# tud-amr/semantic_dsp_map

Hardware: AMD Instinct MI355X
Metric: Mvoxels updated/sec (256^3 grid, 2M particles, VKITTI2 camera; whole hot-path frame) (higher is better)
Workload: dtype f32

## Files before the change

include/sdm.h:

```cpp
#ifndef SDM_H_
#define SDM_H_

#include <stddef.h>
#include <stdint.h>

#ifdef __cplusplus
extern "C" {
#endif

typedef struct sdm_map sdm_map;

typedef enum {
  SDM_OK = 0,
  SDM_ERR_INVALID_ARGUMENT = 1,
  SDM_ERR_NO_DEVICE = 2,
  SDM_ERR_HIP = 3,
  SDM_ERR_CAPACITY = 4,
  SDM_ERR_NOT_CONVERGED = 5,
  SDM_ERR_COMM = 6
} sdm_status;

typedef struct {
  int32_t x_n, y_n, z_n;
  int32_t p_n;
// ... 282 lines not shown
  uint16_t cell_max[3];
  float    wsum_max;
  uint64_t cell_sum[3];
  uint64_t cell_sq[6];
  float    box_min[3];
  float    box_max[3];
  float    centroid[3];
  uint32_t pad;
} sdm_instance;
sdm_status sdm_instances_update(sdm_map *m, uint32_t flags);
sdm_status sdm_get_instances(sdm_map *m, sdm_instance *out, int32_t cap, int32_t *n_out, float origin[3]);
sdm_status sdm_get_label_cells(sdm_map *m, uint32_t out[256]);

#define SDM_FRONTIERS_FACE_CONNECTED 0x1u
#define SDM_FRONTIERS_BYTES_PER_CELL 169
typedef struct {
  uint32_t first_cell;
  uint32_t n_cells;
  uint32_t n_unknown_faces;
  uint32_t first_index;
  uint16_t cell_min[3];
  uint16_t cell_max[3];
  uint32_t pad0;
  uint64_t cell_sum[3];
  float    box_min[3];
  float    box_max[3];
  float    centroid[3];
  uint32_t pad1;
} sdm_frontier_cluster;
sdm_status sdm_frontiers_update(sdm_map *m, uint32_t flags, int32_t min_cells, int64_t max_cells);
sdm_status sdm_get_frontier_clusters(sdm_map *m, sdm_frontier_cluster *out, int32_t cap, int32_t *n_out, float origin[3]);
sdm_status sdm_get_frontier_cells(sdm_map *m, uint32_t *cell, uint32_t *cluster, uint8_t *unknown_faces,
                                  int64_t cap, int64_t *n_out);

#define SDM_VIEW_MAX_RAYS 65536
typedef struct {
  float pos[3];
  float q[4];
  float range;
} sdm_view;
typedef struct {
  uint32_t n_unknown;
  uint32_t n_free;
  uint32_t n_occupied;
  uint32_t rays_hit;
  uint32_t rays_in_map;
  uint32_t pad;
  uint64_t ray_cells;
  uint64_t ray_unknown;
} sdm_view_gain;
sdm_status sdm_query_views(sdm_map *m, const sdm_view *views, int64_t n_views, const float *dirs, int32_t n_rays,
                           sdm_view_gain *out, sdm_segment_hit *rays_out, int32_t *ray_unknown_out, uint32_t flags);

#define SDM_REACH_FACE_CONNECTED  0x1u
#define SDM_REACH_THROUGH_UNKNOWN 0x2u
#define SDM_REACH_COST_PER_CELL   10
typedef struct {
  uint32_t n_starts_used;
  uint32_t n_traversable, n_reached, max_cost_reached;
  uint32_t rounds;
  uint32_t flags, min_d2, max_cost;
} sdm_reach_info;
typedef struct {
  uint32_t cost;
  float    metres;
  uint32_t cell;
  uint8_t  next;
  uint8_t  status;
  uint16_t pad;
} sdm_reach_result;
sdm_status sdm_reach_update(sdm_map *m, const float *start_xyz, const uint32_t *start_cells, int64_t n_starts,
                            uint32_t min_d2, uint32_t max_cost, uint32_t flags);
sdm_status sdm_get_reach(sdm_map *m, uint32_t *cost, sdm_reach_info *info, float origin[3]);
sdm_status sdm_query_reach(sdm_map *m, const float *xyz, const uint32_t *cells, int64_t n, sdm_reach_result *out, uint32_t flags);
sdm_status sdm_reach_paths(sdm_map *m, const float *xyz, const uint32_t *cells, int64_t n, int32_t max_len,
                           uint32_t *cells_out, int32_t *len_out, uint32_t flags);

sdm_status sdm_object_particle_count(sdm_map *m, int32_t track_id, int64_t *count);
sdm_status sdm_tracks_with_particles(sdm_map *m, int32_t *out, int32_t cap, int32_t *n_out);

sdm_status sdm_get_stats(sdm_map *m, sdm_stats *out, int32_t count_live);
sdm_status sdm_set_profiling(sdm_map *m, int32_t on);
sdm_status sdm_debug_force_generic_flood(sdm_map *m, int32_t on);
sdm_status sdm_get_ring_state(sdm_map *m, sdm_ring_state *out);
sdm_status sdm_set_ring_state(sdm_map *m, const sdm_ring_state *in);
sdm_status sdm_get_stamps(sdm_map *m, uint32_t *sx, uint32_t *sy, uint32_t *sz);
sdm_status sdm_set_stamps(sdm_map *m, const uint32_t *sx, const uint32_t *sy, const uint32_t *sz);
sdm_status sdm_dump_state(sdm_map *m, float *px, float *py, float *pz, float *w, uint16_t *ts,
                          uint16_t *track, uint8_t *label, uint8_t *status, uint8_t *forget,
                          uint16_t *owner);
sdm_status sdm_load_state(sdm_map *m, const float *px, const float *py, const float *pz,
                          const float *w, const uint16_t *ts, const uint16_t *track,
                          const uint8_t *label, const uint8_t *status, const uint8_t *forget,
                          const uint16_t *owner);
sdm_status sdm_get_ck_kappa(sdm_map *m, float *out);
sdm_status sdm_get_bin_counts(sdm_map *m, uint32_t *out);
sdm_status sdm_get_bins(sdm_map *m, uint32_t *out, int64_t cap, int64_t *n_out);
sdm_status sdm_get_extrinsic(sdm_map *m, float *out16);

sdm_status sdm_time_occupancy_sweep(sdm_map *m, int32_t iters, float *avg_ms);
sdm_status sdm_debug_fill_dense(sdm_map *m);
sdm_status sdm_debug_fill_dense_ex(sdm_map *m, int32_t mode);
sdm_status sdm_debug_hinted_groups(sdm_map *m, int64_t *n_out);
sdm_status sdm_debug_sweep_lists(sdm_map *m, int32_t mode);
sdm_status sdm_debug_sweep_mode(sdm_map *m, int32_t *mode_out);
sdm_status sdm_debug_alias_cap(sdm_map *m, int32_t cap);
sdm_status sdm_debug_reach_tiles(sdm_map *m, int64_t *tiles_out);
sdm_status sdm_debug_view_batch(sdm_map *m, int32_t max_views_in_flight);

sdm_status sdm_test_scan(const uint32_t *in, uint32_t *out, int64_t n);
sdm_status sdm_test_sort_pairs(const uint32_t *keys_in, const uint32_t *vals_in, uint32_t *keys_out,
                               uint32_t *vals_out, int64_t n, int32_t nbits);
#define SDM_TEST_IN_PLACE 1u
#define SDM_TEST_COUNT_ON_DEVICE 2u
#define SDM_TEST_GUARD_WORDS 64
sdm_status sdm_test_scratch_elems(int32_t sort, int64_t n, int64_t *elems);
sdm_status sdm_test_scan_seq(int32_t n_calls, const int64_t *capacity, const int64_t *count, uint32_t flags,
                             const uint32_t *in, uint32_t *out, int32_t *guard_ok, uint32_t *scratch_out);
sdm_status sdm_test_sort_pairs_seq(int32_t n_calls, const int64_t *capacity, const int64_t *count, const int32_t *nbits,
                                   uint32_t flags, const uint32_t *keys_in, const uint32_t *vals_in, uint32_t *keys_out,
                                   uint32_t *vals_out, int32_t *which, int32_t *guard_ok, uint32_t *scratch_out);

const char *sdm_last_error(void);
const char *sdm_version(void);

#ifdef __cplusplus
}
#endif
#endif
```

semantic_dsp_map_amd/binding.py:

```python
import ctypes as C
import os

import numpy as np

_HERE = os.path.dirname(os.path.abspath(__file__))
LIB_PATH = os.environ.get("SDM_LIB_PATH") or os.path.join(_HERE, "csrc", "libsdm_hip.so")

LABELED_POINT = np.dtype([("x", "<f4"), ("y", "<f4"), ("z", "<f4"), ("sigma", "<f4"),
                          ("track_id", "<u2"), ("label_id", "u1"), ("is_valid", "u1")])
OBJECT_MOVE = np.dtype([("track_id", "<i4"), ("T", "<f4", (16,))])
VOXEL_RESULT = np.dtype([("wsum", "<f4"), ("track", "<u2"), ("label", "u1"), ("occ", "i1")])
POINT = np.dtype([("x", "<f4"), ("y", "<f4"), ("z", "<f4"), ("track", "<u2"), ("label", "u1"), ("occ", "i1")])
POINT_XYZRGB = np.dtype([("x", "<f4"), ("y", "<f4"), ("z", "<f4"), ("one", "<f4"), ("b", "u1"), ("g", "u1"), ("r", "u1"), ("a", "u1"),
                         ("pad", "<u4", (3,))])
assert LABELED_POINT.itemsize == 20 and OBJECT_MOVE.itemsize == 68 and VOXEL_RESULT.itemsize == 8 and POINT.itemsize == 16
SEGMENT_HIT = np.dtype([("t", "<f4"), ("voxel", "<u4"), ("cells", "<i4"), ("track", "<u2"), ("label", "u1"), ("occ", "i1")])
BOX_RESULT = np.dtype([("n_occupied", "<i4"), ("n_free", "<i4"), ("n_unknown", "<i4"), ("first_occupied", "<u4"), ("clipped", "<i4")])
assert SEGMENT_HIT.itemsize == 16 and BOX_RESULT.itemsize == 20
QUERY_ON_DEVICE = 0x1
QUERY_UNKNOWN_BLOCKS = 0x2
DISTANCE_RESULT = np.dtype([("distance", "<f4"), ("gradient", "<f4", (3,)), ("nearest", "<f4", (3,)), ("d2", "<u4"), ("track", "<u2"),
                            ("label", "u1"), ("occ", "i1")])
assert DISTANCE_RESULT.itemsize == 36
ESDF_UNKNOWN_IS_OBSTACLE = 0x1
# ... 103 lines not shown

def load_library():
    global _lib
    if _lib is not None:
        return _lib
    if not os.path.exists(LIB_PATH):
        raise SdmError("libsdm_hip.so is not built: run `python -c 'import __graft_entry__ as g; g.build()'` "
                       "or `make -C semantic_dsp_map_amd/csrc`.  There is no CPU path.")
    L = C.CDLL(LIB_PATH)
    vp = C.c_void_p
    i32, u32, i64 = C.c_int32, C.c_uint32, C.c_int64
    sig = {
        "sdm_create": [C.POINTER(Config), C.POINTER(vp)],
        "sdm_destroy": [vp],
        "sdm_clear": [vp],
        "sdm_set_params": [vp, C.POINTER(Params)],
        "sdm_generate_noise_table": [vp, C.c_uint64, i32, C.c_float],
        "sdm_upload_noise_table": [vp, vp, i32],
        "sdm_download_noise_table": [vp, vp, i32],
        "sdm_download_pdf_table": [vp, vp, i32],
        "sdm_update": [vp, vp, vp, vp, vp, vp, i32, vp, i32, u32, i32],
        "sdm_update_raw": [vp, vp, vp, vp, vp, i32, vp, vp, vp, i32, vp, i32, u32, i32],
        "sdm_update_raw_ex": [vp, vp, vp, vp, vp, i32, vp, vp, vp, i32, vp, i32, u32, i32, vp],
        "sdm_get_labeled_cloud": [vp, vp],
        "sdm_host_alloc": [C.c_size_t, C.POINTER(vp)],
        "sdm_host_free": [vp],
        "sdm_update_begin": [vp, vp, vp, vp, vp, vp, i32, vp, i32, u32, i32, C.POINTER(vp)],
        "sdm_update_finish": [vp, vp, i32, u32, i32],
        "sdm_frame_start": [vp, vp, vp, vp, vp, vp, i32, vp, i32, u32, i32],
        "sdm_frame_moves": [vp],
        "sdm_frame_moves_pending": [vp, C.POINTER(C.c_int32)],
        "sdm_frame_predict": [vp, C.POINTER(vp)],
        "sdm_set_halo_buffers": [vp, vp, vp, vp, vp, i32],
        "sdm_comm_unique_id": [vp],
        "sdm_comm_init": [vp, vp, i32],
        "sdm_ipc_create": [vp, i32, vp],
        "sdm_ipc_connect": [vp, vp],
        "sdm_update_sharded": [vp, vp, vp, vp, vp, vp, i32, vp, i32, u32],
        "sdm_ck_chunk_elems": [vp, C.POINTER(i64)],
        "sdm_ck_reduce": [vp, vp, vp],
        "sdm_comm_timing": [vp, i32],
        "sdm_get_comm_times": [vp, vp],
        "sdm_device_alloc": [vp, C.c_size_t, C.POINTER(vp)],
        "sdm_device_free": [vp, vp],
        "sdm_device_upload": [vp, vp, vp, C.c_size_t],
        "sdm_device_download": [vp, vp, vp, C.c_size_t],
        "sdm_device_synchronize": [vp],
        "sdm_stream": [vp, C.POINTER(vp)],
        "sdm_set_stream": [vp, vp],
        "sdm_set_ck_buffer": [vp, vp],
        "sdm_synchronize": [vp],
        "sdm_get_voxels": [vp, vp],
        "sdm_get_occupied": [vp, vp, C.c_size_t, C.POINTER(C.c_size_t), i32],
        "sdm_get_occupied_rgb": [vp, vp, C.c_size_t, C.POINTER(C.c_size_t), i32],
        "sdm_get_freespace_rgb": [vp, vp, C.c_size_t, C.POINTER(C.c_size_t), i32],
        "sdm_set_colours": [vp, vp],
        "sdm_get_freespace": [vp, vp, C.c_size_t, C.POINTER(C.c_size_t), i32],
        "sdm_voxels_device_ptr": [vp, C.POINTER(vp)],
        "sdm_query_points": [vp, vp, i64, vp, vp, u32],
        "sdm_query_segments": [vp, vp, i64, vp, u32],
        "sdm_query_boxes": [vp, vp, i64, vp, u32],
        "sdm_esdf_update": [vp, u32],
        "sdm_get_esdf": [vp, vp, vp, vp],
        "sdm_query_distance": [vp, vp, i64, vp, u32],
        "sdm_instances_update": [vp, u32],
        "sdm_get_instances": [vp, vp, i32, C.POINTER(i32), vp],
        "sdm_get_label_cells": [vp, vp],
        "sdm_frontiers_update": [vp, u32, i32, i64],
        "sdm_get_frontier_clusters": [vp, vp, i32, C.POINTER(i32), vp],
        "sdm_get_frontier_cells": [vp, vp, vp, vp, i64, C.POINTER(i64)],
        "sdm_query_views": [vp, vp, i64, vp, i32, vp, vp, vp, u32],
        "sdm_debug_view_batch": [vp, i32],
        "sdm_reach_update": [vp, vp, vp, i64, u32, u32, u32],
        "sdm_get_reach": [vp, vp, vp, vp],
        "sdm_query_reach": [vp, vp, vp, i64, vp, u32],
        "sdm_reach_paths": [vp, vp, vp, i64, i32, vp, vp, u32],
        "sdm_debug_reach_tiles": [vp, C.POINTER(i64)],
        "sdm_object_particle_count": [vp, i32, C.POINTER(i64)],
        "sdm_tracks_with_particles": [vp, vp, i32, C.POINTER(i32)],
        "sdm_comm_set_options": [vp, i32, i32],
        "sdm_get_stats": [vp, C.POINTER(Stats), i32],
        "sdm_set_profiling": [vp, i32],
        "sdm_debug_force_generic_flood": [vp, i32],
        "sdm_get_ring_state": [vp, C.POINTER(RingState)],
        "sdm_set_ring_state": [vp, C.POINTER(RingState)],
        "sdm_get_stamps": [vp, vp, vp, vp],
        "sdm_set_stamps": [vp, vp, vp, vp],
        "sdm_dump_state": [vp] + [vp] * 10,
        "sdm_load_state": [vp] + [vp] * 10,
        "sdm_get_ck_kappa": [vp, vp],
        "sdm_get_bin_counts": [vp, vp],
        "sdm_get_bins": [vp, vp, i64, C.POINTER(i64)],
        "sdm_get_extrinsic": [vp, vp],
        "sdm_time_occupancy_sweep": [vp, i32, C.POINTER(C.c_float)],
        "sdm_set_issue_mode": [vp, i32],
        "sdm_bind_host_thread": [i32],
        "sdm_host_numa_node_early": [i32],
        "sdm_debug_fill_dense": [vp],
        "sdm_debug_fill_dense_ex": [vp, i32],
        "sdm_debug_hinted_groups": [vp, C.POINTER(C.c_int64)],
        "sdm_debug_sweep_lists": [vp, i32],
        "sdm_debug_sweep_mode": [vp, C.POINTER(i32)],
        "sdm_debug_alias_cap": [vp, i32],
        "sdm_test_scan": [vp, vp, i64],
        "sdm_test_sort_pairs": [vp, vp, vp, vp, i64, i32],
        "sdm_test_scratch_elems": [i32, i64, C.POINTER(i64)],
        "sdm_test_scan_seq": [i32, vp, vp, u32, vp, vp, C.POINTER(i32), vp],
        "sdm_test_sort_pairs_seq": [i32, vp, vp, vp, u32, vp, vp, vp, vp, vp, C.POINTER(i32), vp],
    }
    for name, argtypes in sig.items():
        fn = getattr(L, name)
        fn.argtypes = argtypes
        fn.restype = C.c_int
    L.sdm_last_error.restype = C.c_char_p
    L.sdm_version.restype = C.c_char_p
    global HOST_NUMA_NODE
    HOST_NUMA_NODE = L.sdm_bind_host_thread(int(os.environ.get("LOCAL_RANK", "0")))
    _lib = L
    return L


def _ptr(a):
    if a is None:
        return None
    if isinstance(a, int):
        return C.c_void_p(a)
    return a.ctypes.data_as(C.c_void_p)


def _check(L, rc, what):
    if rc != 0:
        raise SdmError("%s failed: %s (%s)" % (what, STATUS_NAMES.get(rc, rc), L.sdm_last_error().decode()))


class SdmMap:

    def __init__(self, cfg, params=None, noise_table=None, device=0, shard_rank=0, shard_count=1, max_visible=0):
        self.L = load_library()
        c = Config()
        for k, _ in Config._fields_:
            if k in cfg:
                setattr(c, k, cfg[k])
        c.device, c.shard_rank, c.shard_count, c.max_visible = device, shard_rank, shard_count, max_visible
        self.cfg = c
        h = C.c_void_p()
        _check(self.L, self.L.sdm_create(C.byref(c), C.byref(h)), "sdm_create")
        self.h = h
        self.V = 1 << (c.x_n + c.y_n + c.z_n)
        self.S = 1 << c.p_n
        self.v_count = self.V // shard_count
        self.W, self.H = c.width, c.height
        if params is not None:
            self.set_params(params)
        if noise_table is not None:
            self.upload_noise_table(noise_table)

    def close(self):
        if getattr(self, "h", None):
            self.L.sdm_destroy(self.h)
            self.h = None

    def __del__(self):
        try:
            self.close()
        except Exception:
            pass
# ... 336 lines not shown
            return None
        p = None if xyz is None else np.ascontiguousarray(xyz, dtype=np.float32).reshape(-1, 3)
        w = None if cells is None else np.ascontiguousarray(cells, dtype=np.uint32).reshape(-1)
        n = len(p) if p is not None else len(w) if w is not None else 0
        res = np.empty(n, REACH_RESULT)
        _check(self.L, self.L.sdm_query_reach(self.h, _ptr(p), _ptr(w), n, _ptr(res), 0), "sdm_query_reach")
        return res

    def reach_paths(self, xyz=None, cells=None, max_len=0, on_device=False, n=None, cells_out=None, len_out=None, fill=REACH_NO_COST):
        if on_device:
            _check(self.L, self.L.sdm_reach_paths(self.h, _ptr(int(xyz)) if xyz else None, _ptr(int(cells)) if cells else None, int(n),
                                                  int(max_len), _ptr(int(cells_out)) if cells_out else None, _ptr(int(len_out)),
                                                  QUERY_ON_DEVICE), "sdm_reach_paths")
            return None
        p = None if xyz is None else np.ascontiguousarray(xyz, dtype=np.float32).reshape(-1, 3)
        w = None if cells is None else np.ascontiguousarray(cells, dtype=np.uint32).reshape(-1)
        n = len(p) if p is not None else len(w) if w is not None else 0
        rows, lens = np.full((n, int(max_len)), fill, np.uint32), np.zeros(n, np.int32)
        _check(self.L, self.L.sdm_reach_paths(self.h, _ptr(p), _ptr(w), n, int(max_len), _ptr(rows), _ptr(lens), 0), "sdm_reach_paths")
        return rows, lens

    def reach_tiles(self):
        n = C.c_int64(0)
        _check(self.L, self.L.sdm_debug_reach_tiles(self.h, C.byref(n)), "sdm_debug_reach_tiles")
        return n.value

    def occupied(self, cap=None, zero_center=False, free=False, mark_fov=False):
        cap = cap or self.v_count
        out = np.empty(cap, POINT)
        n = C.c_size_t()
        fn = self.L.sdm_get_freespace if free else self.L.sdm_get_occupied
        _check(self.L, fn(self.h, _ptr(out), cap, C.byref(n), (1 if zero_center else 0) | (2 if mark_fov else 0)),
               "sdm_get_occupied")
        return out[:min(n.value, cap)], n.value

    def set_colours(self, label_bgr, perm, background_label=0, colour_by_label=False, jet_axis=0, evaluation_format=False):
        c = ColourConfig()
        lb = np.ascontiguousarray(label_bgr, np.uint8).reshape(256, 3)
        pm = np.ascontiguousarray(perm, np.uint8).reshape(256)
        C.memmove(c.label_bgr, lb.ctypes.data, 768)
        C.memmove(c.perm, pm.ctypes.data, 256)
        c.background_label, c.colour_by_label = int(background_label), 1 if colour_by_label else 0
        c.jet_axis, c.evaluation_format = int(jet_axis), 1 if evaluation_format else 0
        _check(self.L, self.L.sdm_set_colours(self.h, C.byref(c)), "sdm_set_colours")

    def occupied_rgb(self, cap=None, zero_center=False, free=False):
        cap = cap or self.v_count
        out = np.empty(cap, POINT_XYZRGB)
        n = C.c_size_t()
        fn = self.L.sdm_get_freespace_rgb if free else self.L.sdm_get_occupied_rgb
        _check(self.L, fn(self.h, _ptr(out), cap, C.byref(n), 1 if zero_center else 0), "sdm_get_occupied_rgb")
        return out[:min(n.value, cap)], n.value

    def object_particle_count(self, track):
        n = C.c_int64()
        _check(self.L, self.L.sdm_object_particle_count(self.h, track, C.byref(n)), "sdm_object_particle_count")
        return n.value

    def tracks_with_particles(self):
        out = np.zeros(65536, np.int32)
        n = C.c_int32(0)
        _check(self.L, self.L.sdm_tracks_with_particles(self.h, _ptr(out), out.size, C.byref(n)), "sdm_tracks_with_particles")
        return out[:n.value].copy()

    def stats_unchecked(self):
        return self.stats(check=False)

    def stats(self, count_live=False, check=True):
        s = Stats()
        rc = self.L.sdm_get_stats(self.h, C.byref(s), 1 if count_live else 0)
        if check:
            _check(self.L, rc, "sdm_get_stats")
        d = {k: getattr(s, k) for k, _ in Stats._fields_ if k not in ("stage_ms", "restamped_slabs")}
        d["stage_ms"] = list(s.stage_ms)
        d["restamped_slabs"] = list(s.restamped_slabs)
        return d

    def set_profiling(self, on=True):
        _check(self.L, self.L.sdm_set_profiling(self.h, 1 if on else 0), "sdm_set_profiling")

    def force_generic_flood(self, on=True):
        _check(self.L, self.L.sdm_debug_force_generic_flood(self.h, 1 if on else 0), "sdm_debug_force_generic_flood")

    def ring_state(self):
        r = RingState()
        _check(self.L, self.L.sdm_get_ring_state(self.h, C.byref(r)), "sdm_get_ring_state")
        return {"global_time_stamp": r.global_time_stamp, "moved_steps": list(r.moved_steps),
                "eq_steps": list(r.eq_steps), "map_center": list(r.map_center), "last_pos": list(r.last_pos),
                "birth_cursor": r.birth_cursor, "move_cursor": r.move_cursor}

    def set_ring_state(self, d):
        r = RingState()
        r.global_time_stamp = d["global_time_stamp"]
        for i in range(3):
            r.moved_steps[i] = d["moved_steps"][i]
            r.eq_steps[i] = d["eq_steps"][i]
            r.map_center[i] = d["map_center"][i]
            r.last_pos[i] = d["last_pos"][i]
        r.birth_cursor = d["birth_cursor"]
        r.move_cursor = d["move_cursor"]
        _check(self.L, self.L.sdm_set_ring_state(self.h, C.byref(r)), "sdm_set_ring_state")

    def stamps(self):
        c = self.cfg
        sx = np.empty(1 << c.x_n, np.uint32)
        sy = np.empty(1 << c.y_n, np.uint32)
        sz = np.empty(1 << c.z_n, np.uint32)
        _check(self.L, self.L.sdm_get_stamps(self.h, _ptr(sx), _ptr(sy), _ptr(sz)), "sdm_get_stamps")
        return sx, sy, sz

    def set_stamps(self, sx, sy, sz):
        sx, sy, sz = (np.ascontiguousarray(a, dtype=np.uint32) for a in (sx, sy, sz))
        _check(self.L, self.L.sdm_set_stamps(self.h, _ptr(sx), _ptr(sy), _ptr(sz)), "sdm_set_stamps")

    def dump_state(self):
        n = self.v_count * self.S
        st = {k: np.empty(n, dt) for k, dt in STATE_FIELDS}
        _check(self.L, self.L.sdm_dump_state(self.h, *[_ptr(st[k]) for k, _ in STATE_FIELDS]), "sdm_dump_state")
        return st

    def load_state(self, st):
        arrs = [np.ascontiguousarray(st[k], dtype=dt) for k, dt in STATE_FIELDS]
        _check(self.L, self.L.sdm_load_state(self.h, *[_ptr(a) for a in arrs]), "sdm_load_state")

    def ck_kappa(self):
        out = np.empty(self.W * self.H, np.float32)
        _check(self.L, self.L.sdm_get_ck_kappa(self.h, _ptr(out)), "sdm_get_ck_kappa")
        return out.reshape(self.H, self.W)

    def bin_counts(self):
        out = np.empty(self.W * self.H, np.uint32)
        _check(self.L, self.L.sdm_get_bin_counts(self.h, _ptr(out)), "sdm_get_bin_counts")
        return out.reshape(self.H, self.W)

    def bins(self):
        n = C.c_int64()
        _check(self.L, self.L.sdm_get_bins(self.h, None, 0, C.byref(n)), "sdm_get_bins")
        out = np.empty(max(n.value, 1), np.uint32)
        _check(self.L, self.L.sdm_get_bins(self.h, _ptr(out), n.value, C.byref(n)), "sdm_get_bins")
        return out[:n.value]

    def extrinsic(self):
        out = np.empty(16, np.float32)
        _check(self.L, self.L.sdm_get_extrinsic(self.h, _ptr(out)), "sdm_get_extrinsic")
        return out.reshape(4, 4)

    def fill_dense_ex(self, mode):
        _check(self.L, self.L.sdm_debug_fill_dense_ex(self.h, mode), "sdm_debug_fill_dense_ex")

    def hinted_groups(self):
        n = C.c_int64()
        _check(self.L, self.L.sdm_debug_hinted_groups(self.h, C.byref(n)), "sdm_debug_hinted_groups")
        return n.value

    def force_sweep_lists(self, mode):
        _check(self.L, self.L.sdm_debug_sweep_lists(self.h, int(mode)), "sdm_debug_sweep_lists")

    def sweep_mode(self):
        v = C.c_int32(0)
        _check(self.L, self.L.sdm_debug_sweep_mode(self.h, C.byref(v)), "sdm_debug_sweep_mode")
        return v.value

    def set_alias_cap(self, cap):
        _check(self.L, self.L.sdm_debug_alias_cap(self.h, int(cap)), "sdm_debug_alias_cap")

    def fill_dense(self):
# ... 89 lines not shown
```

semantic_dsp_map_amd/csrc/debug.hip:

```cpp
#include "sdm_map.h"

namespace {

__global__ void k_spin(unsigned long long ticks, unsigned long long *out) {
  const unsigned long long t0 = wall_clock64();
  out[0] = t0;
  while (wall_clock64() - t0 < ticks) __builtin_amdgcn_s_sleep(8);
  out[1] = wall_clock64();
}
__global__ void k_stamp(unsigned long long *out) { *out = wall_clock64(); }

}

extern "C" {

sdm_status sdm_debug_overlap(sdm_map *m, int32_t which, double out_us[2]) {
  if (!m || which < 0 || which > 2 || !out_us) return SDM_ERR_INVALID_ARGUMENT;
  HIP_TRY(hipSetDevice(m->device));
  unsigned long long *d = nullptr, h[3] = {0, 0, 0};
  DevTemps tmp;
  HIP_TRY(tmp.alloc(&d, 3));
  if (which == 2) HIP_TRY(lazy_stream(m->device, &m->s_moves));
  hipStream_t side = which == 0 ? m->s_frustum : (which == 1 ? m->s_birth : m->s_moves);
  HIP_TRY(hipStreamSynchronize(m->stream));
  HIP_TRY(hipStreamSynchronize(side));
  hipLaunchKernelGGL(k_spin, dim3(1), dim3(1), 0, m->stream, 6000ull, d);
  hipLaunchKernelGGL(k_stamp, dim3(1), dim3(1), 0, side, d + 2);
  HIP_TRY(hipStreamSynchronize(m->stream));
  HIP_TRY(hipStreamSynchronize(side));
  HIP_TRY(hipMemcpy(h, d, sizeof(h), hipMemcpyDeviceToHost));
  out_us[0] = ((double)h[2] - (double)h[0]) / 100.0;
  out_us[1] = ((double)h[1] - (double)h[0]) / 100.0;
  return SDM_OK;
}

sdm_status sdm_debug_force_generic_flood(sdm_map *m, int32_t on) {
  if (!m) return SDM_ERR_INVALID_ARGUMENT;
  m->force_generic_flood = on ? 1 : 0;
  return SDM_OK;
}

sdm_status sdm_time_occupancy_sweep(sdm_map *m, int32_t iters, float *avg_ms) {
  if (!m || !avg_ms || iters <= 0) return SDM_ERR_INVALID_ARGUMENT;
  HIP_TRY(hipSetDevice(m->device));
  hipEvent_t a, b;
  HIP_TRY(hipEventCreate(&a));
  HIP_TRY(hipEventCreate(&b));
  launch_occupancy(m->d, m->flt, m->st, m->sc.cnt, 1, m->sc.fa, m->sweep_epoch, m->stream, sweep_mode(m));
  m->sweep_rec_pending = true;
  HIP_TRY(hipStreamSynchronize(m->stream));
  SDM_TRY(sweep_mode_latch(m));
  const int mode = sweep_mode(m);
  HIP_TRY(hipEventRecord(a, m->stream));
  for (int i = 0; i < iters; ++i) launch_occupancy(m->d, m->flt, m->st, m->sc.cnt, 1, m->sc.fa, m->sweep_epoch, m->stream, mode);
  HIP_TRY(hipEventRecord(b, m->stream));
  HIP_TRY(hipEventSynchronize(b));
  m->sweep_rec_pending = true;
  float ms = 0.f;
  HIP_TRY(hipEventElapsedTime(&ms, a, b));
  *avg_ms = ms / iters;
  (void)hipEventDestroy(a);
  (void)hipEventDestroy(b);
  return SDM_OK;
}

sdm_status sdm_debug_fill_dense_ex(sdm_map *m, int32_t mode) {
  if (!m || mode < 0 || mode > 1) return SDM_ERR_INVALID_ARGUMENT;
  HIP_TRY(hipSetDevice(m->device));
  launch_fill_dense(m->d, m->st, m->global_time_stamp ? m->global_time_stamp : 1u, mode, m->stream);
  HIP_TRY(hipStreamSynchronize(m->stream));
  return SDM_OK;
}
sdm_status sdm_debug_fill_dense(sdm_map *m) { return sdm_debug_fill_dense_ex(m, 0); }
sdm_status sdm_debug_sweep_lists(sdm_map *m, int32_t mode) {
  if (!m || mode < -1 || mode > 1) return SDM_ERR_INVALID_ARGUMENT;
  m->sweep_lists_forced = mode;
  if (mode >= 0) m->sweep_lists = mode != 0;
  return SDM_OK;
}
sdm_status sdm_debug_sweep_mode(sdm_map *m, int32_t *mode_out) {
  if (!m || !mode_out) return SDM_ERR_INVALID_ARGUMENT;
  HIP_TRY(hipSetDevice(m->device));
  HIP_TRY(hipStreamSynchronize(m->stream));
  SDM_TRY(sweep_mode_latch(m));
  *mode_out = sweep_mode(m);
  return SDM_OK;
}
sdm_status sdm_debug_alias_cap(sdm_map *m, int32_t cap) {
  if (!m || cap < 1 || (uint32_t)cap > ALIAS_CAP) return SDM_ERR_INVALID_ARGUMENT;
  if (m->n_graph_frames || m->n_direct_frames) return SDM_ERR_INVALID_ARGUMENT;
  m->st.alias_cap = (uint32_t)cap;
  return SDM_OK;
}
sdm_status sdm_debug_hinted_groups(sdm_map *m, int64_t *n_out) {
  if (!m || !n_out) return SDM_ERR_INVALID_ARGUMENT;
  HIP_TRY(hipSetDevice(m->device));
  std::vector<uint8_t> h(grp_hint_bytes(m->d.v_count));
  HIP_TRY(hipMemcpyAsync(h.data(), m->st.grp_hint, h.size(), hipMemcpyDeviceToHost, m->stream));
  HIP_TRY(hipStreamSynchronize(m->stream));
  int64_t n = 0;
  for (uint8_t b : h) n += b != 0;
  *n_out = n;
  return SDM_OK;
}

#ifdef SDM_AB_TIMERS
extern "C++" {
namespace sdm {
void debug_timers(unsigned long long *out32, int reset);
void debug_timers_moves(unsigned long long *out, int reset);
}
}
sdm_status sdm_debug_timers(sdm_map *m, unsigned long long *out32, int reset) {
  HIP_TRY(hipSetDevice(m->device));
  HIP_TRY(hipDeviceSynchronize());
  sdm::debug_timers(out32, reset);
  sdm::debug_timers_moves(out32 + 6 * 8192 * 4, reset);
  return SDM_OK;
}
#endif

// ... 164 lines not shown
```

semantic_dsp_map_amd/csrc/frame.hip:

```cpp
#include <chrono>

#include "sdm_map.h"

#pragma clang fp contract(off)

void sdm::drop_graphs(sdm_map *m) {
  if (m->graph_exec) (void)hipGraphExecDestroy(m->graph_exec);
  if (m->graph) (void)hipGraphDestroy(m->graph);
  m->graph_exec = nullptr;
  m->graph = nullptr;
  m->graph_set_node = nullptr;
  for (hipGraphExec_t &g : m->piece) {
    if (g) (void)hipGraphExecDestroy(g);
    g = nullptr;
  }
}

namespace {

inline void stage_mark(sdm_map *m, int stage) {
  if (m->profiling && !m->capturing) {
    (void)hipEventRecord(m->ev[stage], m->stream);
    m->stage_ran[stage] = true;
  }
}

sdm_status frame_host_prepare(sdm_map *m, const float cam_pos[3], const float cam_q[4], const sdm_object_move *moves, int32_t n_moves,
                              const int32_t *remove_tracks, int32_t n_remove, uint32_t flags, int32_t stop_after) {
  if ((n_moves > MAX_MOVE_OBJECTS || n_remove > MAX_REMOVE_TRACKS) && m->capturing) {
    set_error("sdm_update", __FILE__, __LINE__, "object lists beyond one frame block inside a graph capture");
    return SDM_ERR_INVALID_ARGUMENT;
  }
  m->moves_all.clear();
  m->removes_all.clear();
  m->mv_batch_next = n_moves > MAX_MOVE_OBJECTS ? (size_t)MAX_MOVE_OBJECTS : 0;
  m->mv_batch_ready = false;
  if (n_moves > MAX_MOVE_OBJECTS) m->moves_all.assign(moves, moves + n_moves);
  if (n_remove > MAX_REMOVE_TRACKS) m->removes_all.assign(remove_tracks, remove_tracks + n_remove);
  m->stop_after = stop_after;
  m->frame_flags = flags;
  for (int i = 0; i < 9; ++i) m->stage_ran[i] = false;
  m->global_time_stamp += 1;
  FrameArgs &fa = m->fa;
  fa.su.n = 0;
  fa.su.value = m->global_time_stamp;
  m->restamped[0] = m->restamped[1] = m->restamped[2] = 0;
  update_ego_center(m, cam_pos);
  sync_frame_scalars(m);
  if (m->stamps_dirty) {
    m->sweep_all = true;
    fa.su.n = 0;
  }
  refresh_filter(m);
  m->forgetting_initialized = true;
  compute_extrinsic(m, cam_pos, cam_q);
  compute_frustum_box(m);
  fa.f = m->f;
  memset(&fa.ms, 0, sizeof(fa.ms));
  const int n_first = n_moves < MAX_MOVE_OBJECTS ? n_moves : MAX_MOVE_OBJECTS;
  fa.ms.n = n_first;
  for (int k = 0; k < n_first; ++k) {
    fa.ms.track[k] = (uint16_t)moves[k].track_id;
    memcpy(fa.ms.T[k], moves[k].T, 12 * sizeof(float));
  }
  fa.n_obj = n_first;
  fa.mv_batch = 0;
  if (n_moves > 0 && !stage_done(stop_after, 1)) m->mv_seq++;
  fa.mv_seq = m->mv_seq;
  fa.n_remove = n_remove < MAX_REMOVE_TRACKS ? n_remove : MAX_REMOVE_TRACKS;
  for (int k = 0; k < fa.n_remove; ++k) fa.remove[k] = (uint16_t)remove_tracks[k];
  fa.force_generic = m->force_generic_flood;
  m->n_moves = n_moves;
  m->n_remove = n_remove;
  return SDM_OK;
}

sdm_status frame_enqueue_start(sdm_map *m) {
  hipStream_t s = m->stream;
  const Dims &d = m->d;
  const int32_t stop_after = m->stop_after;
  const bool whole = d.v_count == d.V;
  stage_mark(m, 0);
  if (m->stamps_dirty) SDM_TRY(upload_stamps(m));
  m->cur_depth = m->fa.depth;
  m->cur_cloud = m->fa.cloud;
  if (m->capturing) {
    m->fb.set(d, m->st, m->sc, m->fa, true, whole);
    launch_frame_begin(m->fb, s);
    HIP_TRY(hipEventRecord(m->cap_begin, s));
    HIP_TRY(hipStreamWaitEvent(m->s_frustum, m->cap_begin, 0));
    HIP_TRY(hipStreamWaitEvent(m->s_birth, m->cap_begin, 0));
  } else {
    const bool side_chain_now = m->n_moves > 0 && (!whole || ((m->comm || m->ipc) && m->sharded_frame));
    if (!m->state_event_valid && (!m->vis_event_valid || side_chain_now)) {
      HIP_TRY(hipEventRecord(m->ev_state, s));
      m->state_event_valid = true;
    }
    HIP_TRY(hipStreamWaitEvent(m->s_frustum, m->vis_event_valid ? m->ev_vis : m->ev_state, 0));
    launch_set_frame(m->d_fa[1], m->fa, m->s_frustum);
    HIP_TRY(hipEventRecord(m->ev_fa, m->s_frustum));
    if (whole && m->mv_pending) HIP_TRY(hipMemsetAsync(m->sc.mv_tot, 0, move_total_elems() * sizeof(uint32_t), s));
    m->fb.set(d, m->st, m->sc, m->fa, false, whole);
    launch_frame_begin(m->fb, s, !stage_done(stop_after, 5) ? m->ev_begin : nullptr);
    if (whole && m->n_moves > 0) m->mv_pending = true;
  }
  stage_mark(m, 1);
  if (stage_done(stop_after, 1)) return SDM_OK;

  const bool side_chain = !m->capturing && m->n_moves > 0 && (!whole || ((m->comm || m->ipc) && m->sharded_frame));
  if (m->capturing) {
    if (!whole) launch_moves_count(d, m->st, m->sc, m->d_counts_local, s);
  } else if (side_chain) {
    HIP_TRY(lazy_stream(m->device, &m->s_moves));
    HIP_TRY(hipStreamWaitEvent(m->s_moves, m->ev_state, 0));
    if (!whole) {
      if (m->mv_pending) HIP_TRY(hipMemsetAsync(m->sc.mv_tot, 0, move_total_elems() * sizeof(uint32_t), m->s_moves));
      launch_moves_count(d, m->st, m->sc, m->counts_local_user ? m->counts_local_user : m->d_counts_local, m->s_moves, &m->fa);
      m->mv_pending = true;
    }
    if ((m->comm || m->ipc) && m->sharded_frame) {
      if (m->comm_timing) HIP_TRY(hipEventRecord(m->ev_comm[0], m->s_moves));
      SDM_TRY(exchange_counts(m, m->s_moves));
      if (m->comm_timing) {
        HIP_TRY(hipEventRecord(m->ev_comm[1], m->s_moves));
        m->comm_timed[0] = true;
      }
    }
    HIP_TRY(hipEventRecord(m->ev_counts, m->s_moves));
  }
  if (!stage_done(stop_after, 3)) {
    launch_frustum(d, m->sc, m->s_frustum);
    HIP_TRY(hipGetLastError());
    HIP_TRY(hipEventRecord(m->capturing ? m->cap_frustum : m->ev_frustum, m->s_frustum));
  } else if (!m->capturing) {
    HIP_TRY(hipStreamWaitEvent(s, m->ev_fa, 0));
  }
  if (!stage_done(stop_after, 5)) {
    if (!m->capturing) HIP_TRY(hipStreamWaitEvent(m->s_birth, m->ev_begin, 0));
    m->birth_which = launch_birth_prepare(d, m->flt, m->bo, m->st, m->sc, m->s_birth);
    HIP_TRY(hipEventRecord(m->capturing ? m->cap_birth : m->ev_birth, m->s_birth));
  }
  if (side_chain) HIP_TRY(hipStreamWaitEvent(s, m->ev_counts, 0));
  m->state_event_valid = false;
  m->vis_event_valid = false;
  return SDM_OK;
}

sdm_status check_frame_args(sdm_map *m, const float *depth, const sdm_labeled_point *cloud, const float cam_pos[3], const float cam_q[4],
                            const sdm_object_move *moves, int32_t n_moves, const int32_t *remove_tracks, int32_t n_remove) {
  if (!m || !depth || !cloud || !cam_pos || !cam_q || n_moves < 0 || n_remove < 0 || (n_moves && !moves) || (n_remove && !remove_tracks)) {
    set_error("sdm_update", __FILE__, __LINE__, "null pointer or negative count");
    return SDM_ERR_INVALID_ARGUMENT;
  }
  return SDM_OK;
}

sdm_status stage_inputs(sdm_map *m, const float *depth, const sdm_labeled_point *cloud, uint32_t flags) {
  const size_t hw = (size_t)m->d.W * m->d.H;
  if (flags & SDM_INPUT_ON_DEVICE) {
    m->fa.depth = depth;
    m->fa.cloud = cloud;
  } else {
    HIP_TRY(hipMemcpyAsync(m->d_depth, depth, hw * sizeof(float), hipMemcpyHostToDevice, m->stream));
    HIP_TRY(hipMemcpyAsync(m->d_cloud, cloud, hw * sizeof(sdm_labeled_point), hipMemcpyHostToDevice, m->stream));
    m->fa.depth = m->d_depth;
    m->fa.cloud = m->d_cloud;
  }
  return SDM_OK;
}

}

extern "C" {

sdm_status sdm_frame_start(sdm_map *m, const float *depth, const sdm_labeled_point *cloud, const float cam_pos[3],
                           const float cam_q[4], const sdm_object_move *moves, int32_t n_moves,
                           const int32_t *remove_tracks, int32_t n_remove, uint32_t flags, int32_t stop_after) {
  sdm_status rc = check_frame_args(m, depth, cloud, cam_pos, cam_q, moves, n_moves, remove_tracks, n_remove);
  if (rc != SDM_OK) return rc;
  HIP_TRY(hipSetDevice(m->device));
  if ((rc = frame_host_prepare(m, cam_pos, cam_q, moves, n_moves, remove_tracks, n_remove, flags, stop_after)) != SDM_OK) return rc;
  if ((rc = stage_inputs(m, depth, cloud, flags)) != SDM_OK) return rc;
  m->n_direct_frames++;
  return frame_enqueue_start(m);
}

sdm_status sdm_frame_moves(sdm_map *m) {
  if (!m) return SDM_ERR_INVALID_ARGUMENT;
  if (stage_done(m->stop_after, SDM_STAGE_EGO)) return SDM_OK;
  if (!m->capturing) HIP_TRY(hipSetDevice(m->device));
  const int world = m->cfg.shard_count, rank = m->cfg.shard_rank;
  const int32_t *counts_all = m->counts_all_user;
  int w = world, r = rank;
  if (!counts_all) {
    counts_all = m->counts_local_user ? m->counts_local_user : m->d_counts_local;
    w = 1;
    r = 0;
  }
  if (m->capturing || m->n_moves > 0) {
    launch_moves_transform(m->d, m->flt, m->st, m->sc, counts_all, w, r, m->stream);
    m->mv_pending = false;
    m->mv_batch_ready = false;
    const bool shard = m->d.v_count != m->d.V;
    while (m->mv_batch_next && m->mv_batch_next < m->moves_all.size()) {
      const size_t k0 = m->mv_batch_next;
      const int nb = (int)std::min<size_t>(MAX_MOVE_OBJECTS, m->moves_all.size() - k0);
      FrameArgs &fa = m->fa;
      memset(&fa.ms, 0, sizeof(fa.ms));
      fa.ms.n = nb;
      for (int k = 0; k < nb; ++k) {
        fa.ms.track[k] = (uint16_t)m->moves_all[k0 + k].track_id;
        memcpy(fa.ms.T[k], m->moves_all[k0 + k].T, 12 * sizeof(float));
      }
      fa.n_obj = nb;
      fa.mv_seq = ++m->mv_seq;
      fa.mv_batch += 1;
      m->mv_batch_next = k0 + MAX_MOVE_OBJECTS;
      launch_moves_batch(m->d, m->st, m->sc, fa, m->counts_local_user ? m->counts_local_user : m->d_counts_local, m->stream);
      if (shard) {
        m->mv_batch_ready = true;
        return SDM_OK;
      }
      launch_moves_transform(m->d, m->flt, m->st, m->sc, counts_all, w, r, m->stream);
    }
    m->mv_batch_next = 0;
  }
  return SDM_OK;
}

sdm_status sdm_frame_moves_pending(sdm_map *m, int32_t *pending) {
  if (!m || !pending) return SDM_ERR_INVALID_ARGUMENT;
  *pending = m->mv_batch_ready ? 1 : 0;
  return SDM_OK;
}

sdm_status sdm_frame_predict(sdm_map *m, const float **ck_part_dev) {
  if (!m) return SDM_ERR_INVALID_ARGUMENT;
  if (m->mv_batch_ready) {
    set_error("sdm_frame_predict", __FILE__, __LINE__, "a batch of the frame's object list is still waiting for its counts: sdm_frame_moves_pending");
    return SDM_ERR_INVALID_ARGUMENT;
  }
  const int stop_after = m->stop_after;
  if (stage_done(stop_after, SDM_STAGE_EGO)) return SDM_OK;
  if (!m->capturing) HIP_TRY(hipSetDevice(m->device));
  hipStream_t s = m->stream;
  const Dims &d = m->d;
  if (m->capturing || m->n_moves > 0)
    launch_moves_finish(d, m->flt, m->st, m->sc, m->counts_all_user ? m->cfg.shard_count : 1, m->cfg.shard_rank, s);
  stage_mark(m, 2);
  if (stage_done(stop_after, 2)) return SDM_OK;

  if (m->capturing || m->n_remove > 0) launch_remove(d, m->st, m->sc, s);
  for (size_t k0 = MAX_REMOVE_TRACKS; k0 < m->removes_all.size(); k0 += MAX_REMOVE_TRACKS) {
    FrameArgs &fa = m->fa;
    fa.n_remove = (int)std::min<size_t>(MAX_REMOVE_TRACKS, m->removes_all.size() - k0);
    for (int k = 0; k < fa.n_remove; ++k) fa.remove[k] = (uint16_t)m->removes_all[k0 + k];
    launch_set_frame(m->d_fa[0], fa, s);
    launch_remove(d, m->st, m->sc, s);
  }
  stage_mark(m, 3);
  if (stage_done(stop_after, 3)) return SDM_OK;

  HIP_TRY(hipStreamWaitEvent(s, m->capturing ? m->cap_frustum : m->ev_frustum, 0));
  float *ck_dst = m->ck_user ? m->ck_user : m->d_ck_part;
  launch_visibility(d, m->flt, m->st, m->sc, ck_dst, m->fused_ck ? 1 : 0, s, m->capturing ? nullptr : m->ev_vis);
  if (!m->capturing) m->vis_event_valid = true;
  stage_mark(m, 4);
  if (stage_done(stop_after, 4)) return SDM_OK;

  launch_ck(d, m->flt, m->st, m->sc, ck_dst, m->fused_ck ? 1 : 0, s);
  if (ck_part_dev) *ck_part_dev = ck_dst;
  return SDM_OK;
}

sdm_status sdm_update_begin(sdm_map *m, const float *depth, const sdm_labeled_point *cloud, const float cam_pos[3],
                            const float cam_q[4], const sdm_object_move *moves, int32_t n_moves,
                            const int32_t *remove_tracks, int32_t n_remove, uint32_t flags, int32_t stop_after,
                            const float **ck_part_dev) {
  sdm_status rc = sdm_frame_start(m, depth, cloud, cam_pos, cam_q, moves, n_moves, remove_tracks, n_remove, flags, stop_after);
  if (rc != SDM_OK) return rc;
  const int32_t *keep_all = m->counts_all_user;
  m->counts_all_user = nullptr;
  rc = sdm_frame_moves(m);
  while (rc == SDM_OK && m->mv_batch_ready) rc = sdm_frame_moves(m);
  if (rc == SDM_OK) rc = sdm_frame_predict(m, ck_part_dev);
  m->counts_all_user = keep_all;
  return rc;
}

sdm_status sdm_set_halo_buffers(sdm_map *m, int32_t *counts_local, const int32_t *counts_all, void *send, const void *recv_all,
                                int32_t cap_records) {
  if (!m || cap_records < 0) return SDM_ERR_INVALID_ARGUMENT;
  m->counts_local_user = counts_local;
  m->counts_all_user = counts_all;
  m->sc.halo_send = (unsigned char *)send;
  m->sc.halo_recv = (const unsigned char *)recv_all;
  m->sc.halo_cap = (uint32_t)cap_records;
  m->sc.halo_world = (uint32_t)m->cfg.shard_count;
  return SDM_OK;
}

sdm_status sdm_update_finish(sdm_map *m, const float *ck_parts_dev, int32_t n_parts, uint32_t flags, int32_t stop_after) {
  if (!m || n_parts < 1) return SDM_ERR_INVALID_ARGUMENT;
  if (stage_done(stop_after, SDM_STAGE_VISIBILITY)) return SDM_OK;
  if (!m->capturing) HIP_TRY(hipSetDevice(m->device));
  hipStream_t s = m->stream;
  const Dims &d = m->d;
  const float *own = m->ck_user ? m->ck_user : m->d_ck_part;
  const float *ck_raw = nullptr;
  if (!m->fused_ck) {
    if (!ck_parts_dev || n_parts == 1) ck_raw = ck_parts_dev ? ck_parts_dev : own;
    else launch_ck_finish(d, m->flt, m->sc, ck_parts_dev, n_parts, m->ck_part_stride, s);
  }
  m->ck_raw_last = ck_raw;
  m->ck_part_stride = 0;
  launch_weight(d, m->flt, m->st, m->sc, s, ck_raw);
  stage_mark(m, 5);
  if (stage_done(stop_after, 5)) return SDM_OK;
  HIP_TRY(hipStreamWaitEvent(s, m->capturing ? m->cap_birth : m->ev_birth, 0));
  launch_birth_replay(d, m->flt, m->st, m->sc, m->birth_which, m->global_time_stamp > 65535u, s);
  if (!m->capturing) {
    if (d.v_count != d.V || m->comm || m->ipc) {
      HIP_TRY(hipEventRecord(m->ev_state, s));
      m->state_event_valid = true;
    } else {
      m->state_event_valid = false;
    }
  }
  stage_mark(m, 6);
  if (stage_done(stop_after, 6)) return SDM_OK;
  if (!(flags & SDM_SKIP_OCCUPANCY)) {
    launch_occupancy(d, m->flt, m->st, m->sc.cnt, m->sweep_all ? 1 : 0, m->sc.fa, next_epoch(m->f.epoch), s, sweep_mode(m));
    if (m->sweep_all) m->sweep_rec_pending = true;
    m->sweep_all = false;
    if (!m->capturing) m->sweep_epoch = next_epoch(m->f.epoch);
  }
  stage_mark(m, 7);
  return SDM_OK;
}

namespace {

sdm_status issue_frame(sdm_map *m, uint32_t flags, int32_t stop_after) {
  sdm_status rc = frame_enqueue_start(m);
  if (rc == SDM_OK) rc = sdm_frame_moves(m);
  if (rc == SDM_OK) rc = sdm_frame_predict(m, nullptr);
  if (rc == SDM_OK) rc = sdm_update_finish(m, nullptr, 1, flags, stop_after);
  return rc;
}

sdm_status capture_prepare(sdm_map *m) {
  drop_graphs(m);
  HIP_TRY(hipStreamSynchronize(m->s_frustum));
  if (m->s_moves) HIP_TRY(hipStreamSynchronize(m->s_moves));
  HIP_TRY(hipStreamSynchronize(m->s_birth));
  m->sc.fa = m->d_fa[0];
  m->sc.fa_side = m->d_fa[1];
  return SDM_OK;
}

sdm_status graph_capture(sdm_map *m) {
  SDM_TRY(capture_prepare(m));
  m->capturing = true;
  hipStream_t side[3] = {m->s_frustum, m->s_birth, m->s_moves};
  if (m->graph_shape == GRAPH_CHAIN) m->s_frustum = m->s_birth = m->stream;
  hipError_t e = hipStreamBeginCapture(m->stream, hipStreamCaptureModeThreadLocal);
  sdm_status rc = SDM_OK;
  if (e == hipSuccess) {
    rc = issue_frame(m, m->frame_flags, 0);
    hipGraph_t g = nullptr;
    e = hipStreamEndCapture(m->stream, &g);
    m->graph = g;
  }
  m->s_frustum = side[0];
  m->s_birth = side[1];
  m->s_moves = side[2];
  m->capturing = false;
  if (e != hipSuccess || rc != SDM_OK || !m->graph) {
    set_error("hipStreamCapture", __FILE__, __LINE__, e != hipSuccess ? hipGetErrorString(e) : "frame enqueue failed under capture");
    (void)hipGetLastError();
    return rc != SDM_OK ? rc : SDM_ERR_HIP;
  }
  size_t n_nodes = 0;
  HIP_TRY(hipGraphGetNodes(m->graph, nullptr, &n_nodes));
  std::vector<hipGraphNode_t> nodes(n_nodes);
  HIP_TRY(hipGraphGetNodes(m->graph, nodes.data(), &n_nodes));
  for (hipGraphNode_t nd : nodes) {
    hipGraphNodeType t;
    if (hipGraphNodeGetType(nd, &t) != hipSuccess || t != hipGraphNodeTypeKernel) continue;
    hipKernelNodeParams kp;
    if (hipGraphKernelNodeGetParams(nd, &kp) == hipSuccess && kp.func == FrameBeginLaunch::kernel()) m->graph_set_node = nd;
  }
  if (!m->graph_set_node) {
    set_error("graph_capture", __FILE__, __LINE__, "frame-block node not found in the captured graph");
    return SDM_ERR_HIP;
  }
  HIP_TRY(hipGraphInstantiate(&m->graph_exec, m->graph, nullptr, nullptr, 0));
  m->graph_flt = m->flt;
  return SDM_OK;
}

sdm_status graph_launch(sdm_map *m) {
  m->fb.set(m->d, m->st, m->sc, m->fa, true, m->d.v_count == m->d.V);
  hipKernelNodeParams kp;
  memset(&kp, 0, sizeof(kp));
  kp.func = const_cast<void *>(FrameBeginLaunch::kernel());
  kp.gridDim = dim3(FrameBeginLaunch::GRID);
  kp.blockDim = dim3(FrameBeginLaunch::BLOCK);
  kp.sharedMemBytes = 0;
  kp.kernelParams = m->fb.argv;
  kp.extra = nullptr;
  const auto t0 = std::chrono::steady_clock::now();
  HIP_TRY(hipGraphExecKernelNodeSetParams(m->graph_exec, m->graph_set_node, &kp));
  const auto t1 = std::chrono::steady_clock::now();
  HIP_TRY(hipGraphLaunch(m->graph_exec, m->stream));
  if (m->host_timing) {
    m->t_setparams_us += std::chrono::duration<double, std::micro>(t1 - t0).count();
    m->t_launch_us += std::chrono::duration<double, std::micro>(std::chrono::steady_clock::now() - t1).count();
  }
  return SDM_OK;
}

sdm_status pieces_capture(sdm_map *m) {
  SDM_TRY(capture_prepare(m));
  const Dims &d = m->d;
  auto capture = [&](hipStream_t st, int which, auto &&body) -> sdm_status {
    HIP_TRY(hipStreamBeginCapture(st, hipStreamCaptureModeThreadLocal));
    body(st);
    hipGraph_t g = nullptr;
    hipError_t e = hipStreamEndCapture(st, &g);
    if (e != hipSuccess || !g) {
      set_error("hipStreamEndCapture", __FILE__, __LINE__, e != hipSuccess ? hipGetErrorString(e) : "no graph");
      (void)hipGetLastError();
      return SDM_ERR_HIP;
    }
    e = hipGraphInstantiate(&m->piece[which], g, nullptr, nullptr, 0);
    (void)hipGraphDestroy(g);
    if (e != hipSuccess) {
      set_error("hipGraphInstantiate", __FILE__, __LINE__, hipGetErrorString(e));
      return SDM_ERR_HIP;
    }
    return SDM_OK;
  };
  sdm_status rc = capture(m->s_frustum, 0, [&](hipStream_t st) { launch_frustum(d, m->sc, st); });
  if (rc == SDM_OK)
    rc = capture(m->s_birth, 1, [&](hipStream_t st) { m->birth_which = launch_birth_prepare(d, m->flt, m->bo, m->st, m->sc, st); });
  if (rc == SDM_OK)
    rc = capture(m->stream, 2, [&](hipStream_t st) {
      if (d.v_count != d.V) launch_moves_count(d, m->st, m->sc, m->d_counts_local, st);
      launch_moves_transform(d, m->flt, m->st, m->sc, m->d_counts_local, 1, 0, st);
      launch_moves_finish(d, m->flt, m->st, m->sc, 1, m->cfg.shard_rank, st);
      launch_remove(d, m->st, m->sc, st);
    });
  if (rc == SDM_OK)
    rc = capture(m->stream, 3, [&](hipStream_t st) {
      launch_visibility(d, m->flt, m->st, m->sc, m->d_ck_part, 1, st);
      launch_ck(d, m->flt, m->st, m->sc, m->d_ck_part, 1, st);
      launch_weight(d, m->flt, m->st, m->sc, st);
    });
  if (rc == SDM_OK)
    rc = capture(m->stream, 4, [&](hipStream_t st) {
      launch_birth_replay(d, m->flt, m->st, m->sc, m->birth_which, false, st);
      launch_occupancy(d, m->flt, m->st, m->sc.cnt, 0, m->sc.fa, 0, st);
    });
  m->graph_flt = m->flt;
  return rc;
}

sdm_status pieces_launch(sdm_map *m) {
  hipStream_t s = m->stream;
  const auto t0 = std::chrono::steady_clock::now();
  m->fb.set(m->d, m->st, m->sc, m->fa, true, m->d.v_count == m->d.V);
  launch_frame_begin(m->fb, s);
  HIP_TRY(hipEventRecord(m->ev_begin, s));
  HIP_TRY(hipStreamWaitEvent(m->s_frustum, m->ev_begin, 0));
  HIP_TRY(hipGraphLaunch(m->piece[0], m->s_frustum));
  HIP_TRY(hipEventRecord(m->ev_frustum, m->s_frustum));
  HIP_TRY(hipStreamWaitEvent(m->s_birth, m->ev_begin, 0));
  HIP_TRY(hipGraphLaunch(m->piece[1], m->s_birth));
  HIP_TRY(hipEventRecord(m->ev_birth, m->s_birth));
  HIP_TRY(hipGraphLaunch(m->piece[2], s));
  HIP_TRY(hipStreamWaitEvent(s, m->ev_frustum, 0));
  HIP_TRY(hipGraphLaunch(m->piece[3], s));
  HIP_TRY(hipStreamWaitEvent(s, m->ev_birth, 0));
  HIP_TRY(hipGraphLaunch(m->piece[4], s));
  if (m->host_timing) m->t_launch_us += std::chrono::duration<double, std::micro>(std::chrono::steady_clock::now() - t0).count();
  return SDM_OK;
}

}

sdm_status sdm_set_issue_mode(sdm_map *m, int32_t mode) {
  if (!m || mode < 0 || mode > 4) return SDM_ERR_INVALID_ARGUMENT;
  HIP_TRY(hipSetDevice(m->device));
  bool use;
  int shape;
  issue_mode_for(m, mode, &use, &shape);
  if (shape != m->graph_shape) {
    HIP_TRY(hipStreamSynchronize(m->stream));
    drop_graphs(m);
  }
  m->graph_mode = mode;
  m->use_graph = use;
  m->graph_shape = shape;
  return SDM_OK;
}

sdm_status sdm_update(sdm_map *m, const float *depth, const sdm_labeled_point *cloud, const float cam_pos[3],
                      const float cam_q[4], const sdm_object_move *moves, int32_t n_moves, const int32_t *remove_tracks,
                      int32_t n_remove, uint32_t flags, int32_t stop_after) {
  sdm_status rc = check_frame_args(m, depth, cloud, cam_pos, cam_q, moves, n_moves, remove_tracks, n_remove);
  if (rc != SDM_OK) return rc;
  HIP_TRY(hipSetDevice(m->device));
  m->fused_ck = true;
  const auto tp0 = std::chrono::steady_clock::now();
  rc = frame_host_prepare(m, cam_pos, cam_q, moves, n_moves, remove_tracks, n_remove, flags, stop_after);
  if (rc == SDM_OK) rc = stage_inputs(m, depth, cloud, flags);
  if (m->host_timing) m->t_prepare_us += std::chrono::duration<double, std::micro>(std::chrono::steady_clock::now() - tp0).count();
  if (rc != SDM_OK) {
    m->fused_ck = false;
    return rc;
  }
  const bool would_be_plain = stop_after == 0 && (flags & ~(uint32_t)SDM_INPUT_ON_DEVICE) == 0 && !m->profiling &&
                              m->cfg.shard_count == 1 && !m->comm && !m->ck_user && !m->counts_local_user &&
                              m->stream == m->own_stream && !m->sweep_all && !m->stamps_dirty &&
                              n_moves <= MAX_MOVE_OBJECTS && n_remove <= MAX_REMOVE_TRACKS &&
                              m->global_time_stamp <= 65535u;
  const bool plain = m->use_graph && would_be_plain;
  if (plain) {
// ... 218 lines not shown
```

semantic_dsp_map_amd/csrc/kernels.hip:

```cpp
#include <algorithm>

#include <type_traits>

#include <hip/hip_ext.h>
#include "sdm_internal.h"
#include "sdm_scratch.h"

#pragma clang fp contract(off)

namespace sdm {

namespace {

constexpr int TPB = 256;

#ifdef SDM_AB_TIMERS
}
__device__ unsigned long long g_dbg[6][8192 * 4];
namespace {
#define DBG_T() wall_clock64()
#define DBG_PUTK(k, i, v) do { if (blockIdx.x < 8192) g_dbg[k][blockIdx.x * 4 + (i)] = (unsigned long long)(v); } while (0)
#define DBG_PUT(i, v) DBG_PUTK(0, i, v)
#define DBG_LANE0(k, i) do { if (threadIdx.x == 0 && threadIdx.y == 0) DBG_PUTK(k, i, DBG_T()); } while (0)
#else
// ... 2280 lines not shown
        const uint16_t ptrack = (uint16_t)(tf[u] & 0xffffu);
        const float ff = flt.forget[(tf[u] >> 16) & 7];
        right[u] = 0;
#pragma unroll
        for (int rd = 0; rd < ROUNDS; ++rd) {
          float t = 0.f;
          const uint16_t otrack = (uint16_t)(ot[u][rd] & 0xffffu);
          if ((ot[u][rd] >> 16) && !(flt.independent && otrack != ptrack)) {
            float gk = query_pdf_r<F>(pdf, pv[u].x, o[u][rd].x, sigma[u], rsig[u]) *
                       query_pdf_r<F>(pdf, pv[u].y, o[u][rd].y, sigma[u], rsig[u]) *
                       query_pdf_r<F>(pdf, pv[u].z, o[u][rd].z, sigma[u], rsig[u]);
            if (!flt.independent) {
              if (ptrack != otrack) {
                gk *= flt.id_transition;
              } else {
                if (gk > SDM_MIN_RIGHT_PDF) right[u] = 1;
              }
              gk *= ff;
            }
            t = gk / o[u][rd].w;
          }
          term[wv][u][rd * 64 + lane] = t;
        }
      }
    };
    if (all_fast) terms(std::true_type{}); else terms(std::false_type{});
    unsigned long long rb[U];
#pragma unroll
    for (int u = 0; u < U; ++u) rb[u] = __ballot(right[u]);
    wave_lds_sync();
    const int lu = lane / A7_ROWS, lr = lane % A7_ROWS;
    if (lu < U && lr < side) {
      float acc = 0.f;
      for (int c = 0; c < side; ++c) acc += term[wv][lu][lr * side + c];
      rowsum[wv][lu][lr] = acc;
    }
    wave_lds_sync();
    if (lu < U && lr == 0 && k0 + lu < n) {
      float a = 0.f;
      for (int m = 0; m < side; ++m) a += rowsum[wv][lu][m];
      uint32_t my_bi = bi[0], my_tf = tf[0];
      float my_w = pv[0].w;
      bool right_id = rb[0] != 0ull;
#pragma unroll
      for (int u = 1; u < U; ++u)
        if (lu == u) my_bi = bi[u], my_tf = tf[u], my_w = pv[u].w, right_id = rb[u] != 0ull;
      const size_t li = (size_t)my_bi - slot_base;
      const uint32_t fc = (my_tf >> 16) & 0xffu;
      const SlotRef sr = slot_ref_li(st, d.p_n, li);
      sr.set_w(my_w * (a * flt.p_detect + 1.f - flt.p_detect));
      sr.set_status(ST_UPDATED);
      st.vflag[li >> d.p_n] = VF_DIRTY;
      mark_tile(st, li >> d.p_n, f.epoch);
      sr.set_ts((uint16_t)f.gts);
      if (!flt.independent) {
        uint32_t nf = right_id ? 0u : (fc < 5u ? fc + 1u : fc);
        if (nf != fc) st.forget[li] = (uint8_t)nf;
      }
    }
    wave_lds_sync();
  }
  DBG_LANE0(4, 1);
}

__device__ __forceinline__ void birth_seq_to_pixel(const BirthOrder &bo, int q, int &i, int &j) {
  int p = 0;
#pragma unroll
  for (int k = 1; k < 9; ++k)
    if (q >= bo.off[k]) p = k;
  int r = q - bo.off[p];
  int cols = bo.cols[p];
  i = p / 3 + 3 * (r / cols);
  j = p % 3 + 3 * (r % cols);
}

__global__ __launch_bounds__(TPB) void k_birth_flags(Dims d, BirthOrder bo, Scratch sc) {
  int q = blockIdx.x * blockDim.x + threadIdx.x;
  if (q >= d.W * d.H) return;
  int i, j;
  birth_seq_to_pixel(bo, q, i, j);
  sc.b_valid[q] = as_global(sc.fa->cloud)[i * d.W + j].is_valid ? 1u : 0u;
}

__global__ __launch_bounds__(TPB) void k_birth_candidates(Dims d, Filter flt, BirthOrder bo, State st, Scratch sc) {
  const Frame f = sc.fa->f;
  uint32_t b = blockIdx.x * blockDim.x + threadIdx.x;
  uint32_t total = (uint32_t)(d.W * d.H) * (uint32_t)flt.nb;
  if (b >= total) return;
  int q = (int)(b / (uint32_t)flt.nb), n = (int)(b % (uint32_t)flt.nb);
  int i, j;
  birth_seq_to_pixel(bo, q, i, j);
  const sdm_labeled_point pt = load_point(sc.fa->cloud, (size_t)(i * d.W + j));
  uint32_t key = d.V;
  float x = pt.x, y = pt.y, z = pt.z;
  if (pt.is_valid) {
    if (flt.use_rng) {
      long long draw = (long long)sc.cur->birth_cursor + 3ll * ((long long)flt.nb * sc.b_rank[q] + n);
      float nx = pt.sigma * st.noise[(draw + 1) % flt.noise_n];
      float ny = pt.sigma * st.noise[(draw + 2) % flt.noise_n];
      float nz = pt.sigma * st.noise[(draw + 3) % flt.noise_n];
      x = pt.x + nx;
      y = pt.y + ny;
      z = pt.z + nz;
    }
    uint32_t rx, ry, rz;
    uint32_t v = global_pos_to_voxel(d, f, x, y, z, rx, ry, rz);
    if (v != INVALID_INDEX && rz >= d.rz_begin && rz < d.rz_begin + d.rz_count) key = v;
  }
  sc.bkey_a[b] = key;
  sc.bval_a[b] = b;
  sc.bpos[b] = make_float4(x, y, z, __uint_as_float((uint32_t)pt.track_id | ((uint32_t)pt.label_id << 16)));
}

__global__ void k_birth_cursor(Dims d, Filter flt, Scratch sc) {
  if (threadIdx.x != 0 || blockIdx.x != 0) return;
  int last = d.W * d.H - 1;
  uint32_t n_valid = sc.b_rank[last] + sc.b_valid[last];
  sc.cnt->n_valid_px = n_valid;
  sc.cnt->n_birth_attempts = n_valid * (uint32_t)flt.nb;
  if (flt.use_rng) {
    long long c = (long long)sc.cur->birth_cursor + 3ll * flt.nb * (long long)n_valid;
    sc.cur->birth_cursor = (int32_t)(c % flt.noise_n);
  }
}

__device__ __forceinline__ float resample_next_threshold(float run, float thr, float wpp) {
  if (!(run > thr)) return thr;
  if (wpp == 1.f) return ceilf(run);
  while (run > thr) thr += wpp;
  return thr;
}

template <int S>
__device__ __forceinline__ bool resample_voxel(const Dims &d, State &st, size_t base, uint8_t (&stv)[S], uint16_t (&own)[S],
                                               uint32_t n_alias, bool touched, uint32_t fbits, float (&wv)[S], const uint16_t (&trk)[S]) {
  float weight_sum = 0.f;
  uint32_t updated = 0;
#pragma unroll
  for (int i = 1; i < S; ++i)
    if (stv[i] == ST_UPDATED) {
      weight_sum += wv[i];
      ++updated;
    }
  const uint32_t trigger = S >> 1;
  if (updated <= trigger) return false;
  if (weight_sum < 0.01f) {
#pragma unroll
    for (int i = 1; i < S; ++i)
      if (stv[i] == ST_UPDATED) {
        stv[i] = ST_INVALID;
        owner_erase_local(st, base + i, trk[i], own[i], n_alias, touched, fbits, i);
      }
    return true;
  }
  float wpp = weight_sum / (float)trigger;
  if (wpp > 1.f) wpp = 1.f;
  float run = 0.f, thr = wpp;
#pragma unroll
  for (int i = 1; i < S; ++i)
    if (stv[i] == ST_UPDATED) {
      run += wv[i];
      if (run < thr) {
        stv[i] = ST_INVALID;
        owner_erase_local(st, base + i, trk[i], own[i], n_alias, touched, fbits, i);
      } else {
        wv[i] = wpp;
        thr += wpp;
        thr = resample_next_threshold(run, thr, wpp);
      }
    }
  return true;
}

template <int S>
__device__ __forceinline__ bool resample_voxel_seq(const Dims &d, State &st, size_t base, uint8_t (&stv)[S]) {
  float weight_sum = 0.f;
  uint32_t updated = 0;
  unsigned char *const rec = st.rec + base / S * rec_bytes(S);
  float wv[S];
  {
    uint16_t t1[S], t2[S];
    uint8_t l1[S], s1[S];
    rec_load<S>(rec, wv, t1, t2, l1, s1);
  }
#pragma unroll
  for (int i = 1; i < S; ++i)
    if (stv[i] == ST_UPDATED) {
      weight_sum += wv[i];
      ++updated;
    }
  const uint32_t trigger = S >> 1;
  if (updated <= trigger) return false;
  if (weight_sum < 0.01f) {
#pragma unroll
// ... 47 lines not shown
      ok[j] = u < total && skey[u] == v;
      vs[j] = ok[j] ? sval[u] : 0u;
    }
#pragma unroll
    for (int j = 0; j < 8; ++j)
      if (ok[j]) bps[j] = sc.bpos[vs[j]];
#pragma unroll
    for (int j = 0; j < 8; ++j) {
      if (done) break;
      if (!ok[j]) {
        done = true;
        break;
      }
      const float4 bp = bps[j];
      const uint32_t tl = __float_as_uint(bp.w);
      const uint16_t track = (uint16_t)(tl & 0xffffu);
      const uint8_t label = (uint8_t)((tl >> 16) & 0xffu);
      bool changed = false;
#pragma unroll
      for (int attempt = 0; attempt < 2; ++attempt) {
        int slot = -1;
#pragma unroll
        for (int i = S - 1; i >= 1; --i)
          if (stv[i] == ST_INVALID || (uint32_t)tsv[i] < smax) slot = i;
        if (slot > 0) {
          st.pos4[base + slot] = make_float4(bp.x, bp.y, bp.z, 0.f);
          st.forget[base + slot] = 0;
          const SlotRef sr{rec, S - 1, (uint32_t)slot - 1u};
          sr.set_w(SDM_OCC_INIT_WEIGHT);
          sr.set_ts((uint16_t)f.gts);
          sr.set_track(track);
          sr.set_label(label);
          sr.set_status(ST_REGULAR_BORN);
          if ((int)track <= d.max_movable) {
            if (!owner_insert(st, base + slot, track)) sc.cnt->overflow = 1;
            flag_owner_chunk(st, base + slot);
          }
#pragma unroll
          for (int i = 1; i < S; ++i)
            if (i == slot) {
              stv[i] = ST_REGULAR_BORN;
              tsv[i] = (uint16_t)f.gts;
            }
          changed = true;
          ++n_success;
          break;
        }
        if (!flt.consider_depth_noise) break;
        if (attempt == 1 || resampled || checked) break;
        if (resample_voxel_seq<S>(d, st, base, stv)) {
          resampled = true;
          changed = true;
          n_resamp++;
        } else {
          checked = true;
          break;
        }
      }
      if (!flt.consider_depth_noise && !resampled && !checked) {
        if (resample_voxel_seq<S>(d, st, base, stv)) {
          resampled = true;
          changed = true;
          n_resamp++;
        } else {
          checked = true;
        }
      }
      if (!changed && (resampled || checked)) done = true;
    }
  }
  n_success_out = n_success;
  n_resamp_out = n_resamp;
}

template <int S, bool LITERAL>
__global__ __launch_bounds__(TPB) void k_birth_replay(Dims d, Filter flt, State st, Scratch sc,
                                                      const uint32_t *__restrict__ skey, const uint32_t *__restrict__ sval,
                                                      uint32_t total) {
  const Frame f = sc.fa->f;
  uint32_t t = blockIdx.x * blockDim.x + threadIdx.x;
#ifndef SDM_TIMERS_BIRTH
  if (threadIdx.x == 0) DBG_PUT(0, DBG_T());
#endif
  __shared__ uint32_t heads[TPB], head_key[TPB];
  __shared__ uint32_t n_heads;
  if (threadIdx.x == 0) n_heads = 0;
  __syncthreads();
  if (t < total) {
    const uint32_t key = skey[t];
    const uint32_t prev = t > 0 ? skey[t - 1] : 0xffffffffu;
    if (key < d.V && prev != key) {
      const uint32_t q = atomicAdd(&n_heads, 1u);
      heads[q] = t;
      head_key[q] = key;
    }
  }
  __syncthreads();
  if (threadIdx.x >= n_heads) return;
#ifndef SDM_TIMERS_BIRTH
  if (threadIdx.x == 0) DBG_PUT(1, DBG_T());
#endif
  t = heads[threadIdx.x];
  const uint32_t v = head_key[threadIdx.x];
  constexpr int LMAX = 2 * (S - 1) + 1;
  uint32_t kb[LMAX], sv[LMAX];
  kb[0] = v;
#pragma unroll
  for (int j = 1; j < LMAX; ++j) kb[j] = t + j < total ? skey[t + j] : 0xffffffffu;
  if constexpr (!LITERAL) {
#pragma unroll
    for (int j = 0; j < LMAX; ++j) sv[j] = t + j < total ? sval[t + j] : 0u;
  }
  uint32_t rx, ry, rz;
  voxel_to_ring(d, v, rx, ry, rz);
  const uint32_t smax = stamp_max(st, rx, ry, rz);
  if constexpr (LITERAL) {
    uint32_t ns = 0, nr = 0;
    birth_replay_sequential<S>(d, f, flt, st, sc, skey, sval, total, t, v, smax, ns, nr);
    if (ns || nr) {
      st.vflag[v - d.v_begin] = VF_DIRTY;
      mark_tile(st, v - d.v_begin, f.epoch);
    }
    if (ns) atomicAdd(&sc.cnt->shard[blockIdx.x & (VIS_SHARDS - 1)].birth, ns);
    if (nr) atomicAdd(&sc.cnt->shard[blockIdx.x & (VIS_SHARDS - 1)].resample, nr);
    return;
  } else {
  const size_t base = (size_t)(v - d.v_begin) * S;
  uint8_t stv[S];
  uint16_t tsv[S];
  unsigned char *const rec = rec_ptr(st, S, v - d.v_begin);
  float wv0[S];
  uint16_t trk0[S];
  uint8_t lab0[S], fg[S];
  rec_load<S>(rec, wv0, tsv, trk0, lab0, stv);
  __builtin_memcpy(fg, st.forget + base, S);
  uint16_t own[S];
  load_vec<(2 * S < 16 ? 2 * S : 16)>(own, st.owner + base);
  const uint32_t n_alias = st.alias[0];
  bool alias_touched = false;
  uint32_t fbits = n_alias ? alias_filter_bits<S>(st, base) : 0u;
  uint32_t L = 0;
  {
    bool run = true;
#pragma unroll
    for (int j = 0; j < LMAX; ++j) {
      run = run && kb[j] == v;
      L += run ? 1u : 0u;
    }
  }
#ifdef SDM_TIMERS_BIRTH
  if (threadIdx.x == 0) DBG_PUT(0, DBG_T() + (stv[1] == 0xEE ? 1 : 0) + (own[1] == 0xEEEE ? 1 : 0) + (wv0[1] == 1234.5f ? 1 : 0) + (trk0[1] == 0xEEEE ? 1 : 0) + (kb[LMAX - 1] == 0xEEEEEEEEu ? 1 : 0) + (sv[LMAX - 1] == 0xEEEEEEEEu ? 1 : 0));
#endif
  const bool noise_flavour = flt.consider_depth_noise != 0;
  uint32_t vac0 = 0;
#pragma unroll
  for (int i = 1; i < S; ++i)
    if (stv[i] == ST_INVALID || (uint32_t)tsv[i] < smax) vac0 |= 1u << i;
  const uint32_t V0 = (uint32_t)__popc(vac0);
  const uint32_t nA = noise_flavour ? (L < V0 ? L : V0) : ((L >= 1 && V0 >= 1) ? 1u : 0u);
  int cand[S];
#pragma unroll
  for (int i = 1; i < S; ++i) {
    const uint32_t rank = (uint32_t)__popc(vac0 & ((1u << i) - 1u));
    const bool take = ((vac0 >> i) & 1u) && rank < nA;
    cand[i] = take ? (int)rank : -1;
    if (take) {
      stv[i] = ST_REGULAR_BORN;
      tsv[i] = (uint16_t)f.gts;
    }
  }
  const bool try_resample = noise_flavour ? L > V0 : L >= 1;
  uint32_t n_resamp = 0;
  if (try_resample && resample_voxel<S>(d, st, base, stv, own, n_alias, alias_touched, fbits, wv0, trk0)) n_resamp = 1;
  uint32_t nB = 0;
  if (try_resample) {
    const uint32_t consumed = noise_flavour ? V0 : 1u;
    uint32_t vac1 = 0;
#pragma unroll
    for (int i = 1; i < S; ++i)
      if (stv[i] == ST_INVALID || (uint32_t)tsv[i] < smax) vac1 |= 1u << i;
    const uint32_t V1 = (uint32_t)__popc(vac1), left = L - consumed;
    nB = left < V1 ? left : V1;
#pragma unroll
    for (int i = 1; i < S; ++i) {
      const uint32_t rank = (uint32_t)__popc(vac1 & ((1u << i) - 1u));
      if (((vac1 >> i) & 1u) && rank < nB) cand[i] = (int)(consumed + rank);
    }
  }
  const uint32_t n_success = nA + nB;
  bool any_owner = false;
#ifdef SDM_TIMERS_BIRTH
  if (threadIdx.x == 0) DBG_PUT(1, DBG_T() + (n_success == 77u ? 1 : 0) + (n_resamp == 77u ? 1 : 0) + (stv[S - 1] == 0xEE ? 1 : 0));
#endif
  uint32_t cidx[S];
  float4 bps[S];
#pragma unroll
  for (int i = 1; i < S; ++i) {
    cidx[i] = 0;
    if (cand[i] >= 0) {
#pragma unroll
      for (int j = 0; j < LMAX; ++j) cidx[i] = cand[i] == j ? sv[j] : cidx[i];
    }
  }
#pragma unroll
  for (int i = 1; i < S; ++i) bps[i] = sc.bpos[cidx[i]];
  __builtin_amdgcn_sched_barrier(0);
#ifdef SDM_TIMERS_BIRTH
  if (threadIdx.x == 0) DBG_PUT(2, DBG_T() + (bps[1].x == 1234.5f ? 1 : 0) + (bps[S - 1].x == 1234.5f ? 1 : 0));
#endif
#pragma unroll
  for (int i = 1; i < S; ++i) {
    if (cand[i] < 0) continue;
    const float4 bp = bps[i];
    const uint32_t tl = __float_as_uint(bp.w);
    const uint16_t track = (uint16_t)(tl & 0xffffu);
    const uint8_t label = (uint8_t)((tl >> 16) & 0xffu);
    st.pos4[base + i] = make_float4(bp.x, bp.y, bp.z, 0.f);
    fg[i] = 0;
    wv0[i] = SDM_OCC_INIT_WEIGHT;
    tsv[i] = (uint16_t)f.gts;
    trk0[i] = track;
    lab0[i] = label;
    stv[i] = ST_REGULAR_BORN;
    if ((int)track <= d.max_movable) {
      if (!owner_insert_local(st, base + i, track, own[i], n_alias, alias_touched, fbits, i)) sc.cnt->overflow = 1;
      any_owner = true;
    }
  }
  if (n_success || n_resamp) {
    rec_store_all<S>(rec, wv0, tsv, trk0, lab0, stv);
    __builtin_memcpy(st.owner + base, own, 2 * S);
    if (n_success) __builtin_memcpy(st.forget + base, fg, S);
    if (any_owner) flag_owner_chunk(st, base + 1);
  }
// ... 477 lines not shown
    } else {
      SDM_DISPATCH_S(k_occupancy_scan, sgrid, s, d, flt.occ_threshold, st, cnt, st.occ_need, grid.x, remark);
    }
    SDM_DISPATCH_S(k_occupancy_dense, grid, s, d, flt.occ_threshold, st, cnt, st.occ_need, remark, grid.x);
  } else {
    const uint32_t n_tiles = grid.x;
    const uint32_t seg = n_tiles <= TPB * OCC_SEG_MAX ? ((n_tiles + TPB - 1) / TPB + 15u) / 16u * 16u : 0u;
    if (seg) grid = dim3(std::min<uint32_t>(OCC_GRID, n_tiles));
    SDM_DISPATCH_S(k_occupancy, grid, s, d, flt.occ_threshold, st, cnt, fa, n_tiles, seg);
  }
}


void launch_set_frame(FrameArgs *fa_dev, const FrameArgs &fa, hipStream_t s) {
  hipLaunchKernelGGL(k_set_frame, dim3(1), dim3(TPB), 0, s, fa_dev, fa);
}
const void *set_frame_kernel() { return reinterpret_cast<const void *>(k_set_frame); }

void launch_frustum(const Dims &d, const Scratch &sc, hipStream_t s) {
  static bool lds_attr_set = false;
  if (!lds_attr_set) {
    (void)hipFuncSetAttribute(reinterpret_cast<const void *>(k_flood2d), hipFuncAttributeMaxDynamicSharedMemorySize, 152 * 1024);
    lds_attr_set = true;
  }
  const size_t max_words = (size_t)(d.NY + 1) * (d.NZ + 1) * sc.wpl;
  const unsigned g_mask = (unsigned)std::min<size_t>(blocks_for(max_words * 64), 4096);
  const unsigned g_line = (unsigned)std::min<size_t>(blocks_for((size_t)sc.wy * (d.NZ + 1) * 64), 256);
  hipLaunchKernelGGL(k_vertex_mask, dim3(g_mask), dim3(TPB), 0, s, d, sc.fa_side, sc.vmask, sc.wpl, sc.cnt);
  hipLaunchKernelGGL(k_line_info, dim3(g_line), dim3(TPB), 0, s, d, sc.fa_side, sc.vmask, sc.wpl, sc.wy, sc.line_ne, sc.line_ey, sc.line_ez,
                     sc.cnt);
  hipLaunchKernelGGL(k_flood2d, dim3(1), dim3(TPB), (size_t)(d.NZ + 1) * sc.wy * 8 * 4, s, d, sc.fa_side, sc.vmask, sc.wpl, sc.wy, sc.line_ey,
                     sc.line_ez, sc.line_reach, sc.cnt);
  hipLaunchKernelGGL(k_flood_generic, dim3(1), dim3(1024), 0, s, d, sc.fa_side, sc.vmask, sc.reach, sc.wpl, sc.cnt);
}

void launch_visibility(const Dims &d, const Filter &flt, const State &st, const Scratch &sc, float *ck_out, int finish, hipStream_t s,
                       hipEvent_t vis_done) {
  {
    const size_t max_words = (size_t)((d.NX + 63) / 64 + 1) * d.NY * d.NZ;
    dim3 grid((unsigned)std::min<size_t>(blocks_for(max_words, VIS_WORDS), 2048));
    if (vis_done) {
      switch (d.p_n) {
        case 1: hipExtLaunchKernelGGL(k_visibility<2>, grid, dim3(TPB), 0, s, nullptr, vis_done, 0, d, st, sc); break;
        case 2: hipExtLaunchKernelGGL(k_visibility<4>, grid, dim3(TPB), 0, s, nullptr, vis_done, 0, d, st, sc); break;
        case 3: hipExtLaunchKernelGGL(k_visibility<8>, grid, dim3(TPB), 0, s, nullptr, vis_done, 0, d, st, sc); break;
        default: hipExtLaunchKernelGGL(k_visibility<16>, grid, dim3(TPB), 0, s, nullptr, vis_done, 0, d, st, sc); break;
      }
    } else {
      SDM_DISPATCH_S(k_visibility, grid, s, d, st, sc);
    }
  }
  if (d.W <= 2 * BR_TPB) hipLaunchKernelGGL(k_bin_rows<2>, dim3((unsigned)d.H), dim3(BR_TPB), 0, s, d, st, sc);
  else if (d.W <= 4 * BR_TPB) hipLaunchKernelGGL(k_bin_rows<4>, dim3((unsigned)d.H), dim3(BR_TPB), 0, s, d, st, sc);
  else hipLaunchKernelGGL(k_bin_rows<8>, dim3((unsigned)d.H), dim3(BR_TPB), 0, s, d, st, sc);
  hipLaunchKernelGGL(k_ck_classify, dim3(blocks_for((size_t)d.W * d.H)), dim3(TPB), 0, s, d, flt, sc, ck_out, finish);
}

void launch_ck(const Dims &d, const Filter &flt, const State &st, const Scratch &sc, float *ck_out, int finish, hipStream_t s) {
  hipLaunchKernelGGL(k_ck, dim3(CK_HEAVY_BLOCKS + blocks_for((size_t)d.W * d.H, A7_ROWS * A7_ITEMS)), dim3(A7_ROWS, A7_ITEMS), 0, s, d, flt, st, sc,
                     ck_out, finish);
}
void launch_ck_finish(const Dims &d, const Filter &flt, const Scratch &sc, const float *parts, int n_parts, size_t part_stride, hipStream_t s) {
  hipLaunchKernelGGL(k_ck_finish, dim3(blocks_for((size_t)d.W * d.H)), dim3(TPB), 0, s, d, flt, sc, parts, n_parts,
                     part_stride ? part_stride : (size_t)d.W * d.H);
}
void launch_ck_reduce_chunk(const float *stage, const float *own_part, float *full, uint32_t chunk, int world, int rank, hipStream_t s) {
  hipLaunchKernelGGL(k_ck_reduce_chunk, dim3((chunk + TPB - 1) / TPB), dim3(TPB), 0, s, stage, own_part, full, chunk, world, rank);
}
void launch_weight(const Dims &d, const Filter &flt, const State &st, const Scratch &sc, hipStream_t s, const float *ck_raw) {
  const int side = 2 * d.window_half + 1;
#define SDM_WEIGHT(UU, RR)                                                                                              \
  if (ck_raw) hipLaunchKernelGGL((k_weight<UU, RR, true>), dim3(WT_GRID), dim3(64 * WT_WAVES), 0, s, d, flt, st, sc, ck_raw); \
  else hipLaunchKernelGGL((k_weight<UU, RR, false>), dim3(WT_GRID), dim3(64 * WT_WAVES), 0, s, d, flt, st, sc, ck_raw);
  if (side * side <= 64) {
    SDM_WEIGHT(4, 1)
  } else if (side * side <= 128) {
    SDM_WEIGHT(4, 2)
  } else {
    SDM_WEIGHT(2, 4)
  }
#undef SDM_WEIGHT
}

int launch_birth_prepare(const Dims &d, const Filter &flt, const BirthOrder &bo, const State &st,
                         const Scratch &sc, hipStream_t s) {
  const size_t hw = (size_t)d.W * d.H;
  const size_t total = hw * flt.nb;
  if (flt.use_rng) {
    hipLaunchKernelGGL(k_birth_flags, dim3(blocks_for(hw)), dim3(TPB), 0, s, d, bo, sc);
    exclusive_scan_u32(sc.b_valid, sc.b_rank, hw, sc.scan_scratch_b, s);
  }
  hipLaunchKernelGGL(k_birth_candidates, dim3(blocks_for(total)), dim3(TPB), 0, s, d, flt, bo, st, sc);
  if (flt.use_rng) hipLaunchKernelGGL(k_birth_cursor, dim3(1), dim3(64), 0, s, d, flt, sc);
  int nbits = d.x_n + d.y_n + d.z_n + 1;
  return radix_sort_pairs(sc.bkey_a, sc.bval_a, sc.bkey_b, sc.bval_b, total, nbits, sc.sort_scratch, s);
}

void launch_birth_replay(const Dims &d, const Filter &flt, const State &st, const Scratch &sc, int which, bool literal,
                         hipStream_t s) {
  const size_t total = (size_t)d.W * d.H * flt.nb;
  const uint32_t *skey = which ? sc.bkey_b : sc.bkey_a;
  const uint32_t *sval = which ? sc.bval_b : sc.bval_a;
  dim3 grid(blocks_for(total));
#define SDM_BIRTH(SS)                                                                                                  \
  if (literal) hipLaunchKernelGGL((k_birth_replay<SS, true>), grid, dim3(TPB), 0, s, d, flt, st, sc, skey, sval, (uint32_t)total); \
  else hipLaunchKernelGGL((k_birth_replay<SS, false>), grid, dim3(TPB), 0, s, d, flt, st, sc, skey, sval, (uint32_t)total);
  switch (d.p_n) {
    case 1: SDM_BIRTH(2) break;
    case 2: SDM_BIRTH(4) break;
    case 3: SDM_BIRTH(8) break;
    default: SDM_BIRTH(16) break;
  }
#undef SDM_BIRTH
}

void launch_labeled_cloud(const Dims &d, const CloudArgsHost &h, const float *depth, const uint8_t *static_mask,
                          const uint16_t *label_to_inst, const uint8_t *obj_masks, const double *bbox,
                          sdm_labeled_point *cloud, hipStream_t s) {
  CloudArgs a;
  static_assert(sizeof(CloudArgs) == sizeof(CloudArgsHost), "CloudArgs layout");
  __builtin_memcpy(&a, &h, sizeof(a));
  hipLaunchKernelGGL(k_labeled_cloud, dim3(blocks_for((size_t)d.W * d.H)), dim3(TPB), 0, s, d, a, depth, static_mask, label_to_inst,
                     obj_masks, bbox, cloud);
}

void launch_manual_resize(const Dims &d, const void *src, void *dst, int src_w, int src_h, float scale, int elem_bytes,
                          hipStream_t s) {
  const float scale_inv = 1.f / scale;
  dim3 grid(blocks_for((size_t)d.W * d.H));
  if (elem_bytes == 4)
    hipLaunchKernelGGL(k_manual_resize<float>, grid, dim3(TPB), 0, s, (const float *)src, (float *)dst, src_w, src_h, d.W, d.H, scale_inv);
  else
    hipLaunchKernelGGL(k_manual_resize<uint8_t>, grid, dim3(TPB), 0, s, (const uint8_t *)src, (uint8_t *)dst, src_w, src_h, d.W, d.H,
                       scale_inv);
}

__global__ __launch_bounds__(TPB) void k_rec_pack(Dims d, State st, const float *__restrict__ w, const uint16_t *__restrict__ ts,
                                                  const uint16_t *__restrict__ track, const uint8_t *__restrict__ label,
                                                  const uint8_t *__restrict__ status, size_t n) {
  size_t li = (size_t)blockIdx.x * blockDim.x + threadIdx.x;
  if (li >= n) return;
  if ((li & (d.S - 1)) == 0) {
    st.vts[li >> d.p_n] = ts[li];
    return;
  }
  const SlotRef sr = slot_ref_li(st, d.p_n, li);
  sr.set_status(status[li]);
  sr.set_w(w[li]);
  sr.set_ts(ts[li]);
  sr.set_track(track[li]);
  sr.set_label(label[li]);
}
__global__ __launch_bounds__(TPB) void k_rec_unpack(Dims d, State st, float *__restrict__ w, uint16_t *__restrict__ ts,
                                                    uint16_t *__restrict__ track, uint8_t *__restrict__ label,
                                                    uint8_t *__restrict__ status, size_t n) {
  size_t li = (size_t)blockIdx.x * blockDim.x + threadIdx.x;
  if (li >= n) return;
  if ((li & (d.S - 1)) == 0) {
    status[li] = ST_TIMEPTC;
    w[li] = 0.f;
    ts[li] = st.vts[li >> d.p_n];
    track[li] = 0;
    label[li] = 0;
    return;
  }
  const SlotRef sr = slot_ref_li(st, d.p_n, li);
  status[li] = sr.status();
  w[li] = sr.w();
  ts[li] = sr.ts();
  track[li] = sr.track();
  label[li] = sr.label();
}

void launch_rec_pack(const Dims &d, const State &st, const float *w, const uint16_t *ts, const uint16_t *track,
                     const uint8_t *label, const uint8_t *status, hipStream_t s) {
  const size_t n = (size_t)d.v_count * d.S;
  hipLaunchKernelGGL(k_rec_pack, dim3(blocks_for(n)), dim3(TPB), 0, s, d, st, w, ts, track, label, status, n);
}
void launch_rec_unpack(const Dims &d, const State &st, float *w, uint16_t *ts, uint16_t *track, uint8_t *label, uint8_t *status,
                       hipStream_t s) {
  const size_t n = (size_t)d.v_count * d.S;
  hipLaunchKernelGGL(k_rec_unpack, dim3(blocks_for(n)), dim3(TPB), 0, s, d, st, w, ts, track, label, status, n);
}

__global__ __launch_bounds__(TPB) void k_fill_dense(Dims d, State st, uint32_t stamp, int mode) {
  size_t li = (size_t)blockIdx.x * blockDim.x + threadIdx.x;
  const size_t n = (size_t)d.v_count * d.S;
  if (li >= n) return;
  const uint32_t i = (uint32_t)(li & (d.S - 1));
// ... 88 lines not shown
```

semantic_dsp_map_amd/csrc/lifecycle.hip:

```cpp
#include <rocrand/rocrand.h>

#include <chrono>
#include <cmath>
#include <cstdlib>
#include <mutex>

#include "sdm_map.h"

#pragma clang fp contract(off)

namespace {

thread_local std::string g_last_error;

__attribute__((constructor(101))) void sdm_runtime_defaults() {
  setenv("HIP_FORCE_DEV_KERNARG", "1", 0);
}

constexpr double GRAPH_PIECES_US = 110.0, GRAPH_CHAIN_US = 170.0;
constexpr int LAUNCHES_PER_FRAME = 50;

__global__ void k_noop() {}

}

namespace sdm {

void set_error(const char *what, const char *file, int line, const char *detail) {
  char buf[512];
  snprintf(buf, sizeof(buf), "%s (%s:%d): %s", what, file, line, detail ? detail : "");
  g_last_error = buf;
}

sdm_status map_alloc(sdm_map *m, void **p, size_t bytes, bool pinned) {
  *p = nullptr;
  HIP_TRY(pinned ? hipHostMalloc(p, bytes, hipHostMallocDefault) : hipMalloc(p, bytes));
  (pinned ? m->pinned : m->allocs).push_back(*p);
  return SDM_OK;
}
void map_release(sdm_map *m, void **p) {
  for (auto *list : {&m->allocs, &m->pinned}) {
    const auto at = std::find(list->begin(), list->end(), *p);
    if (!*p || at == list->end()) continue;
    list->erase(at);
    (void)(list == &m->pinned ? hipHostFree(*p) : hipFree(*p));
  }
  *p = nullptr;
}
sdm_status new_event(sdm_map *m, hipEvent_t *e, unsigned flags) {
  HIP_TRY(hipEventCreateWithFlags(e, flags));
  m->events.push_back(*e);
  return SDM_OK;
}

void issue_mode_for(const sdm_map *m, int mode, bool *use_graph, int *shape) {
  *use_graph = mode == 2 ? m->enqueue_us > GRAPH_PIECES_US : mode != 0;
  *shape = mode == 1 ? GRAPH_BRANCHED
           : mode == 3 ? GRAPH_CHAIN
           : mode == 2 ? (m->enqueue_us > GRAPH_CHAIN_US ? GRAPH_CHAIN : GRAPH_PIECES)
                       : GRAPH_PIECES;
}

static hipError_t new_stream(int, hipStream_t *s) { return hipStreamCreateWithFlags(s, hipStreamNonBlocking); }
static void retire_stream(int, hipStream_t s) {
  if (!s) return;
  (void)hipStreamSynchronize(s);
  (void)hipStreamDestroy(s);
}
hipError_t lazy_stream(int device, hipStream_t *s) {
  if (*s) return hipSuccess;
  return new_stream(device, s);
}

static void build_pdf_table(std::vector<float> &pdf) {
  pdf.resize(PDF_NUM);
  const float pi_2 = 1.5707964f;
  for (int i = 0; i < PDF_NUM; ++i) {
    float value = (float)(i - PDF_NUM / 2) * 0.001f;
    pdf[i] = (1.f / (sqrtf(2.f * pi_2))) * expf(-powf(value, 2) / (2));
  }
}

void refresh_filter(sdm_map *m) {
  Filter &flt = m->flt;
  const sdm_params &p = m->prm;
  if (!m->forgetting_initialized) {
    for (int i = 0; i < 5; ++i) m->forgetting_function[i] = (float)pow(2.5, -i / p.forgetting_rate);
  }
  for (int c = 0; c < 8; ++c)
    flt.forget[c] = (c < p.max_forget_count && c < 5) ? m->forgetting_function[c] : 0.f;
  flt.p_detect = p.detection_probability;
  flt.noise_number = p.noise_number;
  flt.occ_threshold = p.occupancy_threshold;
  flt.id_transition = p.id_transition_probability;
  flt.independent = p.if_use_independent_filter ? 1 : 0;
  flt.consider_depth_noise = p.if_consider_depth_noise ? 1 : 0;
  flt.nb = p.if_consider_depth_noise ? std::max(p.nb_ptc_num_per_point, 0) : 1;
  flt.use_rng = (p.if_consider_depth_noise && p.nb_ptc_num_per_point != 1) ? 1 : 0;
  flt.noise_n = m->noise_n;
}

static void build_birth_order(sdm_map *m) {
  const int W = m->d.W, H = m->d.H;
  int off = 0;
  for (int p = 0; p < 9; ++p) {
    int rs = p / 3, cs = p % 3;
    int rows = rs < H ? (H - rs + 2) / 3 : 0;
    int cols = cs < W ? (W - cs + 2) / 3 : 0;
    m->bo.off[p] = off;
    m->bo.cols[p] = cols > 0 ? cols : 1;
    off += rows * cols;
  }
  m->bo.off[9] = off;
}

static sdm_status ensure_birth_buffers(sdm_map *m) {
  const size_t hw = (size_t)m->d.W * m->d.H;
  const int nb = std::max(m->flt.nb, 1);
  if (nb <= m->nb_alloc) return SDM_OK;
  const size_t need = hw * nb;
  Scratch &sc = m->sc;
  void **const old[6] = {(void **)&sc.bkey_a, (void **)&sc.bval_a, (void **)&sc.bkey_b, (void **)&sc.bval_b, (void **)&sc.bpos, (void **)&sc.sort_scratch};
  const size_t bytes[6] = {need * 4, need * 4, need * 4, need * 4, need * sizeof(*sc.bpos), sort_scratch_elems(need) * 4};
  void *fresh[6] = {};
  sdm_status rc = SDM_OK;
  HIP_TRY(hipStreamSynchronize(m->stream));
  for (int i = 0; i < 6 && rc == SDM_OK; ++i) rc = map_alloc(m, &fresh[i], bytes[i], false);
  for (int i = 0; i < 6; ++i) {
    map_release(m, rc == SDM_OK ? old[i] : &fresh[i]);
    if (rc == SDM_OK) *old[i] = fresh[i];
  }
  SDM_TRY(rc);
  HIP_TRY(hipMemsetAsync(sc.sort_scratch, 0, sort_scratch_elems(need) * 4, m->stream));
  HIP_TRY(hipStreamSynchronize(m->stream));
  m->nb_alloc = nb;
  m->sort_cap = need;
  return SDM_OK;
}

static void update_ring_index_params(sdm_map *m) {
  const Dims &d = m->d;
  int steps[3];
  for (int a = 0; a < 3; ++a) steps[a] = static_cast<int>(m->ego_center[a] * d.recip);
  for (int a = 0; a < 3; ++a) m->map_center[a] = static_cast<float>(steps[a]) * d.voxel_size;
  const uint32_t N[3] = {d.NX, d.NY, d.NZ};
  std::vector<uint32_t> *st[3] = {&m->stamps_x, &m->stamps_y, &m->stamps_z};
  for (int a = 0; a < 3; ++a) {
    const int new_moved = steps[a] - m->moved_steps[a];
    const int n = (int)N[a];
    auto stamp = [&](uint32_t idx) {
      (*st[a])[idx] = m->global_time_stamp;
      m->restamped[a]++;
      StampUpdates &su = m->fa.su;
      if (su.n < MAX_STAMP_UPDATES) su.entry[su.n++] = (uint16_t)((a << 12) | idx);
      else m->stamps_dirty = true;
    };
    if (new_moved > 0) {
      for (int i = 0; i < new_moved; ++i) stamp(axis_correct(i + m->eq_steps[a], N[a]));
    } else if (new_moved < 0) {
      for (int i = 0; i < -new_moved; ++i) stamp(axis_correct(n - 1 - i + m->eq_steps[a], N[a]));
    }
  }
  for (int a = 0; a < 3; ++a) {
    m->moved_steps[a] = steps[a];
    const int n = (int)N[a];
    const int o = steps[a];
    m->eq_steps[a] = o > 0 ? o % n : (o < 0 ? -(-o % n) : 0);
  }
}

void update_ego_center(sdm_map *m, const float pos[3]) {
  const Dims &d = m->d;
  const float mx = (1 << (d.x_n - 2)) * d.voxel_size;
  const float my = (1 << (d.y_n - 2)) * d.voxel_size;
  const float mz = (1 << (d.z_n - 2)) * d.voxel_size;
  const float max_once = std::min(std::min(mx, my), mz);
  float mv[3] = {pos[0] - m->last_pos[0], pos[1] - m->last_pos[1], pos[2] - m->last_pos[2]};
  const float sq = (mv[0] * mv[0] + mv[1] * mv[1]) + mv[2] * mv[2];
  float dist = sqrtf(sq);
  float unit[3] = {mv[0], mv[1], mv[2]};
  if (sq > 0.f)
    for (int a = 0; a < 3; ++a) unit[a] = mv[a] / dist;
  float new_pos[3] = {m->last_pos[0], m->last_pos[1], m->last_pos[2]};
  while (dist > max_once) {
    for (int a = 0; a < 3; ++a) new_pos[a] = new_pos[a] + unit[a] * max_once;
    for (int a = 0; a < 3; ++a) m->ego_center[a] = new_pos[a];
    update_ring_index_params(m);
    for (int a = 0; a < 3; ++a) mv[a] = pos[a] - new_pos[a];
    dist = sqrtf((mv[0] * mv[0] + mv[1] * mv[1]) + mv[2] * mv[2]);
  }
  for (int a = 0; a < 3; ++a) m->ego_center[a] = pos[a];
  update_ring_index_params(m);
  for (int a = 0; a < 3; ++a) m->last_pos[a] = pos[a];
}

void compute_extrinsic(sdm_map *m, const float pos[3], const float q[4]) {
  const float w = q[0], x = q[1], y = q[2], z = q[3];
  const float tx = 2.f * x, ty = 2.f * y, tz = 2.f * z;
  const float twx = tx * w, twy = ty * w, twz = tz * w;
  const float txx = tx * x, txy = ty * x, txz = tz * x;
  const float tyy = ty * y, tyz = tz * y, tzz = tz * z;
  float *R = m->cam_R;
  R[0] = 1.f - (tyy + tzz);
  R[1] = txy - twz;
  R[2] = txz + twy;
  R[3] = txy + twz;
  R[4] = 1.f - (txx + tzz);
  R[5] = tyz - twx;
  R[6] = txz - twy;
  R[7] = tyz + twx;
  R[8] = 1.f - (txx + tyy);
  for (int a = 0; a < 3; ++a) m->cam_p[a] = pos[a];
  float *E = m->f.E;
  for (int r = 0; r < 3; ++r) {
    const float a = R[0 * 3 + r], b = R[1 * 3 + r], c = R[2 * 3 + r];
    E[r * 4 + 0] = a;
// ... 108 lines not shown
  }
  if (c.overflow && c.n_moved > m->sc.cap_move) {
    char buf[160];
    snprintf(buf, sizeof(buf), "moved-copy list overflowed: %u particles of moving objects in one frame, more than %u", c.n_moved,
             m->sc.cap_move);
    set_error("capacity", __FILE__, __LINE__, buf);
    return SDM_ERR_CAPACITY;
  }
  if (c.overflow) {
    set_error("capacity", __FILE__, __LINE__, "visible-particle or move list overflowed: more visible particles than sdm_config.max_visible, more in ONE image row than "
              "max(2 max_visible / height, 2 width slots) - raise max_visible -, or more than 2^20 in one pixel's bin");
    return SDM_ERR_CAPACITY;
  }
  if (c.vis_flood_rounds >= 256 && !c.vis_flood_complex) {
    set_error("flood", __FILE__, __LINE__, "frustum flood fill did not converge");
    return SDM_ERR_NOT_CONVERGED;
  }
  return SDM_OK;
}

}

extern "C" {

const char *sdm_last_error(void) { return g_last_error.c_str(); }
const char *sdm_version(void) { return "libsdm_hip 0.1 (gfx950)"; }

static sdm_status map_init(sdm_map *m, const sdm_config *cfg, int shard_count) {
  m->cfg = *cfg;
  m->cfg.shard_count = shard_count;
  m->device = cfg->device;
  Dims &d = m->d;
  d.x_n = cfg->x_n;
  d.y_n = cfg->y_n;
  d.z_n = cfg->z_n;
  d.p_n = cfg->p_n;
  d.NX = 1u << d.x_n;
  d.NY = 1u << d.y_n;
  d.NZ = 1u << d.z_n;
  d.S = 1u << d.p_n;
  d.V = d.NX * d.NY * d.NZ;
  d.rz_count = d.NZ / shard_count;
  d.rz_begin = d.rz_count * cfg->shard_rank;
  d.v_count = d.V / shard_count;
  d.v_begin = d.v_count * cfg->shard_rank;
  d.voxel_size = cfg->voxel_size;
  d.recip = 1.f / cfg->voxel_size;
  d.pmax[0] = (d.NX >> 1) * cfg->voxel_size;
  d.pmax[1] = (d.NY >> 1) * cfg->voxel_size;
  d.pmax[2] = (d.NZ >> 1) * cfg->voxel_size;
  for (int a = 0; a < 3; ++a) d.pmin[a] = -d.pmax[a];
  d.W = cfg->width;
  d.H = cfg->height;
  d.fx = cfg->fx;
  d.fy = cfg->fy;
  d.cx = cfg->cx;
  d.cy = cfg->cy;
  d.dmin = cfg->depth_min;
  d.dmax = cfg->depth_max;
  d.tanx = (float)tan(atan2(cfg->width / 2.0, (double)cfg->fx));
  d.tany = (float)tan(atan2(cfg->height / 2.0, (double)cfg->fy));
  d.occl_coeff = 0.1f + 1.f;
  d.window_half = cfg->window_half;
  d.max_movable = cfg->max_movable_track;
  m->stamps_x.assign(d.NX, 0);
  m->stamps_y.assign(d.NY, 0);
  m->stamps_z.assign(d.NZ, 0);
  m->prm.detection_probability = 0.95f;
  m->prm.noise_number = 0.1f;
  m->prm.nb_ptc_num_per_point = 3;
  m->prm.occupancy_threshold = 0.2f;
  m->prm.max_obersevation_lost_time = 5;
  m->prm.forgetting_rate = 1.0f;
  m->prm.max_forget_count = 5;
  m->prm.match_score_threshold = 0.3f;
  m->prm.id_transition_probability = 0.1f;
  m->prm.if_consider_depth_noise = 0;
  m->prm.if_use_independent_filter = 0;
  m->prm.depth_noise_first_order = 0.f;
  m->prm.depth_noise_zero_order = 0.1f;

  for (hipStream_t *s : {&m->own_stream, &m->s_frustum, &m->s_birth}) HIP_TRY(new_stream(cfg->device, s));
  m->stream = m->own_stream;
  for (hipEvent_t *e : {&m->ev_state, &m->ev_counts, &m->ev_begin, &m->ev_frustum, &m->ev_birth, &m->ev_fa, &m->ev_vis, &m->cap_begin,
                        &m->cap_frustum, &m->cap_birth, &m->ev_copy, &m->raw[0].ev_free, &m->raw[1].ev_free})
    SDM_TRY(new_event(m, e, hipEventDisableTiming));
  const size_t n_slots = (size_t)d.v_count * d.S;
  const size_t hw = (size_t)d.W * d.H;
#define A(ptr, n) SDM_TRY(alloc_tracked(m, &(ptr), (n)))
  A(m->st.pos4, n_slots);
  A(m->st.forget, n_slots);
  HIP_TRY(hipMemsetAsync(m->st.forget, 0, n_slots, m->stream));
  A(m->st.rec, rec_array_bytes(d.v_count, d.S));
  const size_t v_groups = ((size_t)d.v_count + 511) / 512 * 512;
  A(m->st.vts, v_groups + 64);
  A(m->st.vflag, v_groups + 64);
  m->st.tile_stride = (uint32_t)tile_mark_bytes(d);
  A(m->st.tile_dirty, 2 * (size_t)m->st.tile_stride);
  A(m->st.occ_need, ((size_t)d.v_count + 63) / 64 + 32);
  A(m->st.occ_list, occ_list_tiles(d.v_count) * OCC_LIST_CAP);
  A(m->st.occ_list_n, occ_list_tiles(d.v_count) + 64);
  m->st.occ_unit_cap = (uint32_t)((occ_list_tiles(d.v_count) + OCC_LIST_SHARDS - 1) / OCC_LIST_SHARDS * (OCC_LIST_CAP / OCC_LIST_UNIT));
  A(m->st.occ_unit, (size_t)OCC_LIST_SHARDS * m->st.occ_unit_cap);
  A(m->st.occ_shard, OCC_LIST_SHARDS + 1);
  HIP_TRY(hipMemsetAsync(m->st.occ_shard, 0, (OCC_LIST_SHARDS + 1) * sizeof(State::OccListShard), m->stream));
  A(m->st.grp_hint, grp_hint_bytes(d.v_count));
  HIP_TRY(hipMemsetAsync(m->st.grp_hint, 0, grp_hint_bytes(d.v_count), m->stream));
  A(m->st.owner, n_slots);
  A(m->st.owner_flag, owner_flag_bytes(n_slots));
  A(m->st.owner_flag2, owner_flag2_bytes(n_slots));
  A(m->st.alias, 2 + 2 * ALIAS_CAP);
  m->st.alias_cap = ALIAS_CAP;
  HIP_TRY(hipMemsetAsync(m->st.alias, 0, 8, m->stream));
  A(m->st.alias_filter, ALIAS_FILTER_WORDS);
  HIP_TRY(hipMemsetAsync(m->st.alias_filter, 0, ALIAS_FILTER_WORDS * 4, m->stream));
  A(m->st.res, d.v_count);
  A(m->st.stamps_x, d.NX);
  A(m->st.stamps_y, d.NY);
  A(m->st.stamps_z, d.NZ);
  A(m->st.pdf, PDF_NUM);
  m->noise_n = 1000000;
  A(m->st.noise, m->noise_n);
  HIP_TRY(hipMemsetAsync(m->st.noise, 0, (size_t)m->noise_n * 4, m->stream));
  {
    std::vector<float> pdf;
    build_pdf_table(pdf);
    HIP_TRY(hipMemcpyAsync(m->st.pdf, pdf.data(), PDF_NUM * 4, hipMemcpyHostToDevice, m->stream));
    HIP_TRY(hipStreamSynchronize(m->stream));
  }
  Scratch &sc = m->sc;
  sc.wpl = (int)((d.NX + 1 + 63) / 64);
  const size_t n_words = (size_t)(d.NZ + 1) * (d.NY + 1) * sc.wpl;
  A(sc.vmask, n_words);
  A(sc.reach, n_words);
  sc.wy = (int)((d.NY + 1 + 63) / 64);
  const size_t n_line_words = (size_t)(d.NZ + 1) * sc.wy;
  A(sc.line_ne, n_line_words);
  A(sc.line_ey, n_line_words);
  A(sc.line_ez, n_line_words);
  A(sc.line_reach, n_line_words);
  A(m->d_depth, hw);
  A(m->d_cloud, hw);
  A(sc.bin_count, hw + 1 + (size_t)d.H * ROW_SUBS * ROW_CNT_STRIDE);
  A(sc.row_win, hw);
  sc.row_cnt = sc.bin_count + hw + 1;
  A(sc.bin_start, (size_t)d.H * (d.W + 1));
  size_t cap_vis = cfg->max_visible > 0 ? (size_t)cfg->max_visible
                                        : std::min<size_t>(n_slots + (size_t)VIS_SHARDS * 256 * d.S, (size_t)16 << 20);
  cap_vis = (cap_vis + VIS_SHARDS - 1) / VIS_SHARDS * VIS_SHARDS;
  cap_vis = std::min<size_t>(cap_vis, 0xffffff00u);
  sc.cap_vis = (uint32_t)cap_vis;
  {
    const size_t row_total = std::min<size_t>(cap_vis, std::max<size_t>(2 * cap_vis / (size_t)d.H, (size_t)2 * d.W * d.S));
    sc.row_cap = (uint32_t)std::max<size_t>(64, (row_total + row_total / 4) / ROW_SUBS + 64);
  }
  A(sc.row_list, (size_t)d.H * ROW_SUBS * sc.row_cap);
  A(sc.bin_idx, cap_vis);
  A(sc.vpix, cap_vis);
  A(sc.vp4, cap_vis);
  A(sc.vtf, cap_vis);
  A(sc.pix4, hw);
  A(sc.pixt, hw);
  A(sc.ck_kappa, hw);
  sc.cap_heavy = (uint32_t)(((hw + 255) / 256 + VIS_SHARDS - 1) / VIS_SHARDS * 256);
  A(sc.ck_heavy, (size_t)sc.cap_heavy * VIS_SHARDS);
  A(sc.ck_class, hw);
  m->ck_chunk = (uint32_t)(((hw + shard_count - 1) / shard_count + 63) / 64 * 64);
// ... 83 lines not shown
    static double best_seen = 0.0;
    double best = burst[0];
    {
      std::lock_guard<std::mutex> g(best_mu);
      if (best_seen == 0.0 || best < best_seen) best_seen = best;
      best = best_seen;
    }
    m->enqueue_us = best / 16.0 * LAUNCHES_PER_FRAME;
    issue_mode_for(m, m->graph_mode, &m->use_graph, &m->graph_shape);
  }
  return SDM_OK;
}

sdm_status sdm_create(const sdm_config *cfg, sdm_map **out) {
  if (!cfg || !out) return SDM_ERR_INVALID_ARGUMENT;
  *out = nullptr;
  if (cfg->x_n + cfg->y_n + cfg->z_n + cfg->p_n > 31 || cfg->x_n < 2 || cfg->y_n < 2 || cfg->z_n < 2 || cfg->p_n < 1 ||
      cfg->p_n > 4 || cfg->x_n > 9 || cfg->y_n > 9 || cfg->z_n > 9 || cfg->width <= 0 || cfg->height <= 0 || !(cfg->voxel_size > 0.f) ||
      cfg->window_half < 0 || cfg->window_half > 7) {
    set_error("sdm_create", __FILE__, __LINE__, "invalid configuration");
    return SDM_ERR_INVALID_ARGUMENT;
  }
  int shard_count = cfg->shard_count > 0 ? cfg->shard_count : 1;
  if (cfg->shard_rank < 0 || cfg->shard_rank >= shard_count || ((1u << cfg->z_n) % (uint32_t)shard_count) != 0) {
    set_error("sdm_create", __FILE__, __LINE__, "invalid shard rank/count (count must divide the z axis)");
    return SDM_ERR_INVALID_ARGUMENT;
  }
  if (cfg->width >= (1 << ROW_COL_BITS)) {
    set_error("sdm_create", __FILE__, __LINE__, "image width above 4095 (the row kernel of the pixel bins holds one image row in LDS)");
    return SDM_ERR_INVALID_ARGUMENT;
  }
  int ndev = 0;
  if (hipGetDeviceCount(&ndev) != hipSuccess || ndev <= 0 || cfg->device < 0 || cfg->device >= ndev) {
    set_error("sdm_create", __FILE__, __LINE__, "no HIP device / bad device ordinal: libsdm_hip has no CPU path");
    return SDM_ERR_NO_DEVICE;
  }
  HIP_TRY(hipSetDevice(cfg->device));
  {
    const char *e = getenv("SDM_NUMA_BIND");
    if (!(e && e[0] == '0')) (void)bind_host_thread_to(cfg->device);
  }
  sdm_map *m = new sdm_map();
  const sdm_status rc = map_init(m, cfg, shard_count);
  if (rc == SDM_OK) *out = m;
  else (void)sdm_destroy(m);
  return rc;
}

sdm_status sdm_destroy(sdm_map *m) {
  if (!m) return SDM_ERR_INVALID_ARGUMENT;
  if (m->host_timing) {
    const double ng = m->n_graph_frames ? (double)m->n_graph_frames : 1.0, nd = m->n_direct_frames ? (double)m->n_direct_frames : 1.0;
    fprintf(stderr, "sdm host timing: prepare+inputs %.1f us/frame; graph frames %llu: set-params %.1f us, hipGraphLaunch %.1f us; direct frames %llu: %.1f us\n",
            m->t_prepare_us / (ng + nd - ((m->n_graph_frames && m->n_direct_frames) ? 0.0 : 1.0)), (unsigned long long)m->n_graph_frames,
            m->t_setparams_us / ng, m->t_launch_us / ng, (unsigned long long)m->n_direct_frames, m->t_direct_us / nd);
  }
  (void)hipSetDevice(m->device);
  for (hipStream_t st : {m->stream, m->s_frustum, m->s_birth, m->s_moves, m->s_copy})
    if (st) (void)hipStreamSynchronize(st);
  exchange_teardown(m);
  drop_graphs(m);
  for (hipEvent_t e : m->events) (void)hipEventDestroy(e);
  for (void *p : m->allocs) (void)hipFree(p);
  for (void *p : m->pinned) (void)hipHostFree(p);
  retire_stream(m->device, m->s_copy);
  retire_stream(m->device, m->s_moves);
  retire_stream(m->device, m->own_stream);
  retire_stream(m->device, m->s_frustum);
  retire_stream(m->device, m->s_birth);
  delete m;
  return SDM_OK;
}

sdm_status sdm_clear(sdm_map *m) {
  if (!m) return SDM_ERR_INVALID_ARGUMENT;
  HIP_TRY(hipSetDevice(m->device));
  m->state_event_valid = false;
  m->vis_event_valid = false;
  m->sweep_all = true;
  m->sweep_skip_scan = false;
  m->sweep_rec_pending = false;
  host_initialize(m);
  launch_clear(m->d, m->st, m->stream, false);
  return upload_stamps(m);
}

sdm_status sdm_set_params(sdm_map *m, const sdm_params *p) {
  if (!m || !p) return SDM_ERR_INVALID_ARGUMENT;
  if (p->nb_ptc_num_per_point < 0 || p->nb_ptc_num_per_point > 64) return SDM_ERR_INVALID_ARGUMENT;
  HIP_TRY(hipSetDevice(m->device));
  const sdm_params before = m->prm;
  m->prm = *p;
  m->sweep_all = true;
  refresh_filter(m);
  const sdm_status rc = ensure_birth_buffers(m);
  if (rc != SDM_OK) {
    m->prm = before;
    refresh_filter(m);
  }
  return rc;
}

sdm_status sdm_generate_noise_table(sdm_map *m, uint64_t seed, int32_t n, float stddev) {
  if (!m || n <= 0 || n > m->noise_n || (n & 1)) return SDM_ERR_INVALID_ARGUMENT;
  HIP_TRY(hipSetDevice(m->device));
  rocrand_generator gen;
  if (rocrand_create_generator(&gen, ROCRAND_RNG_PSEUDO_PHILOX4_32_10) != ROCRAND_STATUS_SUCCESS) {
    set_error("rocrand_create_generator", __FILE__, __LINE__, "failed");
    return SDM_ERR_HIP;
  }
  rocrand_status rs = rocrand_set_seed(gen, seed);
  if (rs == ROCRAND_STATUS_SUCCESS) rs = rocrand_set_stream(gen, m->stream);
  if (rs == ROCRAND_STATUS_SUCCESS) rs = rocrand_generate_normal(gen, m->st.noise, (size_t)n, 0.0f, stddev);
  (void)hipStreamSynchronize(m->stream);
  rocrand_destroy_generator(gen);
  if (rs != ROCRAND_STATUS_SUCCESS) {
    set_error("rocrand_generate_normal", __FILE__, __LINE__, "failed");
    return SDM_ERR_HIP;
  }
  m->flt.noise_n = n;
  return SDM_OK;
}

sdm_status sdm_upload_noise_table(sdm_map *m, const float *table, int32_t n) {
  if (!m || !table || n <= 0 || n > m->noise_n) return SDM_ERR_INVALID_ARGUMENT;
  HIP_TRY(hipSetDevice(m->device));
  HIP_TRY(hipMemcpyAsync(m->st.noise, table, (size_t)n * 4, hipMemcpyHostToDevice, m->stream));
  HIP_TRY(hipStreamSynchronize(m->stream));
  m->flt.noise_n = n;
  return SDM_OK;
}

sdm_status sdm_download_noise_table(sdm_map *m, float *table, int32_t n) {
  if (!m || !table || n <= 0 || n > m->noise_n) return SDM_ERR_INVALID_ARGUMENT;
  HIP_TRY(hipSetDevice(m->device));
  HIP_TRY(hipMemcpyAsync(table, m->st.noise, (size_t)n * 4, hipMemcpyDeviceToHost, m->stream));
  HIP_TRY(hipStreamSynchronize(m->stream));
  return SDM_OK;
}

sdm_status sdm_download_pdf_table(sdm_map *m, float *table, int32_t n) {
  if (!m || !table || n <= 0 || n > PDF_NUM) return SDM_ERR_INVALID_ARGUMENT;
  HIP_TRY(hipSetDevice(m->device));
  HIP_TRY(hipMemcpyAsync(table, m->st.pdf, (size_t)n * 4, hipMemcpyDeviceToHost, m->stream));
  HIP_TRY(hipStreamSynchronize(m->stream));
  return SDM_OK;
}

}
```

semantic_dsp_map_amd/csrc/moves.hip:

```cpp
#include <hip/hip_ext.h>
#include "sdm_internal.h"
#include "sdm_scratch.h"

#pragma clang fp contract(off)

namespace sdm {

#ifdef SDM_AB_TIMERS
__device__ unsigned long long g_dbg_m[4][4096 * 4];
void debug_timers_moves(unsigned long long *out, int reset) {
  (void)hipMemcpyFromSymbol(out, HIP_SYMBOL(g_dbg_m), sizeof(g_dbg_m));
  if (reset) {
    static unsigned long long z[4][4096 * 4];
    (void)hipMemcpyToSymbol(HIP_SYMBOL(g_dbg_m), z, sizeof(z));
  }
}
#define DBGM(k, i, v) do { if (blockIdx.x < 4096 && threadIdx.x == 0) g_dbg_m[k][blockIdx.x * 4 + (i)] = (unsigned long long)(v); } while (0)
#define DBGM_T() wall_clock64()
#define DBGM_MAX(i, v) atomicMax(&g_dbg_m[1][2048 * 4 + (i)], (unsigned long long)(v))
#define DBGM_ADD(i, v) atomicAdd(&g_dbg_m[1][2048 * 4 + (i)], (unsigned long long)(v))
#else
#define DBGM(k, i, v)
#define DBGM_T() 0ull
#define DBGM_MAX(i, v)
// ... 1022 lines not shown

void launch_tracks_with_particles(const Dims &d, const State &st, uint32_t *bitmap, hipStream_t s) {
  const size_t n_slots = (size_t)d.v_count * d.S;
  hipMemsetAsync(bitmap, 0, 2048 * sizeof(uint32_t), s);
  const size_t n_chunks = (n_slots + OWNER_CHUNK - 1) / OWNER_CHUNK;
  hipLaunchKernelGGL(k_tracks_with_particles, dim3((unsigned)((n_chunks + OWNER_GROUP - 1) / OWNER_GROUP)), dim3(TPB), 0, s, st, n_slots, bitmap);
}

size_t move_blocks(const Dims &d) { return ((size_t)d.v_count * d.S + MV_CHUNK - 1) / MV_CHUNK; }
size_t move_count_elems() { return (size_t)MAX_MOVE_OBJECTS * MV_LIST_CAP + 1; }
size_t move_member_elems(size_t n_slots) {
  const size_t n_chunks = (n_slots + MV_CHUNK - 1) / MV_CHUNK;
  return std::min<size_t>(MV_LIST_CAP, std::max<size_t>(n_chunks, 1024)) * MV_CHUNK;
}
size_t move_total_elems() { return (size_t)2 * MAX_MOVE_OBJECTS * MV_TOT_STRIDE; }

static MembersArgs members_args(const Dims &d, const Scratch &sc) {
  MembersArgs ma;
  ma.mv_cnt = sc.mv_cnt;
  ma.mv_list = sc.mv_list;
  ma.mv_nlist = sc.mv_nlist;
  ma.mv_nmem = sc.mv_nmem;
  ma.mv_mem = sc.mv_mem;
  ma.mv_tot = sc.mv_tot;
  ma.cur = sc.cur;
  ma.n_flags = (uint32_t)move_blocks(d);
  ma.n_slots = (size_t)d.v_count * d.S;
  return ma;
}
void launch_moves_count(const Dims &d, const State &st, const Scratch &sc, int32_t *counts_local, hipStream_t s, const FrameArgs *by_value) {
  const FrameArgs *fa = by_value ? sc.fa_moves : sc.fa_side;
  const MembersArgs ma = members_args(d, sc);
  if (by_value)
    hipLaunchKernelGGL(k_move_members_v, dim3(MV_GRID), dim3(TPB), 0, s, st, ma, *by_value, const_cast<FrameArgs *>(sc.fa_moves));
  else
    hipLaunchKernelGGL(k_move_members, dim3(MV_GRID), dim3(TPB), 0, s, st, ma, fa);
  if (d.v_count != d.V) hipLaunchKernelGGL(k_move_local_counts, dim3(1), dim3(HALO_OBJ), 0, s, counts_local, sc, fa, 1);
}

void launch_moves_batch(const Dims &d, const State &st, const Scratch &sc, const FrameArgs &fa_batch, int32_t *counts_local, hipStream_t s) {
  const MembersArgs ma = members_args(d, sc);
  hipLaunchKernelGGL(k_move_members_v, dim3(MV_GRID), dim3(TPB), 0, s, st, ma, fa_batch, const_cast<FrameArgs *>(sc.fa));
  if (d.v_count != d.V) hipLaunchKernelGGL(k_move_local_counts, dim3(1), dim3(HALO_OBJ), 0, s, counts_local, sc, sc.fa, 0);
}

void FrameBeginLaunch::set(const Dims &d_, const State &st_, const Scratch &sc, const FrameArgs &fa_, bool with_side, bool with_members_) {
  cnt = sc.cnt;
  bin_count = sc.bin_count;
  n_bins = (uint32_t)(d_.W * d_.H + 1 + d_.H * (int)(ROW_SUBS * ROW_CNT_STRIDE));
  st = st_;
  fa = fa_;
  dst_main = const_cast<FrameArgs *>(sc.fa);
  dst_side = with_side ? const_cast<FrameArgs *>(sc.fa_side) : nullptr;
  d = d_;
  slab_max = d_.NY * d_.NZ;
  if (d_.NX * d_.NZ > slab_max) slab_max = d_.NX * d_.NZ;
  if (d_.NX * d_.NY > slab_max) slab_max = d_.NX * d_.NY;
  ma = members_args(d_, sc);
  with_members = with_members_ ? 1 : 0;
  argv[0] = &cnt;
  argv[1] = &bin_count;
  argv[2] = &n_bins;
  argv[3] = &st;
  argv[4] = &fa;
  argv[5] = &dst_main;
  argv[6] = &dst_side;
  argv[7] = &d;
  argv[8] = &slab_max;
  argv[9] = &ma;
  argv[10] = &with_members;
}
const void *FrameBeginLaunch::kernel() { return reinterpret_cast<const void *>(k_frame_begin); }

void launch_frame_begin(FrameBeginLaunch &a, hipStream_t s, hipEvent_t done) {
  if (done) (void)hipExtLaunchKernel(FrameBeginLaunch::kernel(), dim3(FrameBeginLaunch::GRID), dim3(FrameBeginLaunch::BLOCK), a.argv, 0, s, nullptr, done, 0);
  else (void)hipLaunchKernel(FrameBeginLaunch::kernel(), dim3(FrameBeginLaunch::GRID), dim3(FrameBeginLaunch::BLOCK), a.argv, 0, s);
}

void launch_moves_transform(const Dims &d, const Filter &flt, const State &st, const Scratch &sc, const int32_t *counts_all, int world,
                            int rank, hipStream_t s) {
  hipLaunchKernelGGL(k_move_apply, dim3(1024), dim3(TPB), 0, s, d, flt, st, sc, d.v_count != d.V ? counts_all : nullptr, world, rank);
}

void launch_moves_finish(const Dims &d, const Filter &flt, const State &st, const Scratch &sc, int world, int rank, hipStream_t s) {
  if (world > 1 && sc.halo_recv) hipLaunchKernelGGL(k_move_import, dim3(64, world), dim3(TPB), 0, s, d, sc, world, rank);
  dim3 grid(RP_GRID);
  switch (d.p_n) {
    case 1: hipLaunchKernelGGL(k_move_replay<2>, grid, dim3(RP_TPB), 0, s, d, flt, st, sc); break;
    case 2: hipLaunchKernelGGL(k_move_replay<4>, grid, dim3(RP_TPB), 0, s, d, flt, st, sc); break;
    case 3: hipLaunchKernelGGL(k_move_replay<8>, grid, dim3(RP_TPB), 0, s, d, flt, st, sc); break;
    default: hipLaunchKernelGGL(k_move_replay<16>, grid, dim3(RP_TPB), 0, s, d, flt, st, sc); break;
  }
}

void launch_remove(const Dims &d, const State &st, const Scratch &sc, hipStream_t s) {
  const size_t n_slots = (size_t)d.v_count * d.S;
  const size_t n_chunks = (n_slots + OWNER_CHUNK - 1) / OWNER_CHUNK;
  hipLaunchKernelGGL(k_remove, dim3((unsigned)(n_chunks < 1024 ? n_chunks : 1024)), dim3(TPB), 0, s, st, n_slots, sc.fa, d.p_n);
}

}
```

semantic_dsp_map_amd/csrc/readback.hip:

```cpp
#include <cmath>

#include "sdm_map.h"

extern "C" {

sdm_status sdm_get_labeled_cloud(sdm_map *m, sdm_labeled_point *out) {
  if (!m || !out) return SDM_ERR_INVALID_ARGUMENT;
  HIP_TRY(hipSetDevice(m->device));
  HIP_TRY(hipMemcpyAsync(out, m->cur_cloud, (size_t)m->d.W * m->d.H * sizeof(sdm_labeled_point), hipMemcpyDeviceToHost, m->stream));
  HIP_TRY(hipStreamSynchronize(m->stream));
  return SDM_OK;
}

sdm_status sdm_device_alloc(sdm_map *m, size_t bytes, void **out) {
  if (!m || !out) return SDM_ERR_INVALID_ARGUMENT;
  HIP_TRY(hipSetDevice(m->device));
  HIP_TRY(hipMalloc(out, bytes ? bytes : 1));
  return SDM_OK;
}
sdm_status sdm_device_free(sdm_map *m, void *p) {
  if (!m) return SDM_ERR_INVALID_ARGUMENT;
  HIP_TRY(hipSetDevice(m->device));
  HIP_TRY(hipFree(p));
  return SDM_OK;
// ... 254 lines not shown
  if (!m || !sx || !sy || !sz) return SDM_ERR_INVALID_ARGUMENT;
  memcpy(sx, m->stamps_x.data(), m->d.NX * 4);
  memcpy(sy, m->stamps_y.data(), m->d.NY * 4);
  memcpy(sz, m->stamps_z.data(), m->d.NZ * 4);
  return SDM_OK;
}
sdm_status sdm_set_stamps(sdm_map *m, const uint32_t *sx, const uint32_t *sy, const uint32_t *sz) {
  if (m) m->sweep_all = true;
  if (!m || !sx || !sy || !sz) return SDM_ERR_INVALID_ARGUMENT;
  HIP_TRY(hipSetDevice(m->device));
  memcpy(m->stamps_x.data(), sx, m->d.NX * 4);
  memcpy(m->stamps_y.data(), sy, m->d.NY * 4);
  memcpy(m->stamps_z.data(), sz, m->d.NZ * 4);
  SDM_TRY(upload_stamps(m));
  HIP_TRY(hipStreamSynchronize(m->stream));
  return SDM_OK;
}

sdm_status sdm_dump_state(sdm_map *m, float *px, float *py, float *pz, float *w, uint16_t *ts, uint16_t *track,
                          uint8_t *label, uint8_t *status, uint8_t *forget, uint16_t *owner) {
  if (!m) return SDM_ERR_INVALID_ARGUMENT;
  HIP_TRY(hipSetDevice(m->device));
  hipStream_t s = m->stream;
  const size_t n = (size_t)m->d.v_count * m->d.S;
  if (px || py || pz || forget) {
    DevTemps tmp;
    float *tx, *ty, *tz;
    uint8_t *tf;
    HIP_TRY(tmp.alloc(&tx, n));
    HIP_TRY(tmp.alloc(&ty, n));
    HIP_TRY(tmp.alloc(&tz, n));
    HIP_TRY(tmp.alloc(&tf, n));
    launch_unpack_pos4(m->st.pos4, m->st.forget, tx, ty, tz, tf, n, s);
    if (px) HIP_TRY(hipMemcpyAsync(px, tx, n * 4, hipMemcpyDeviceToHost, s));
    if (py) HIP_TRY(hipMemcpyAsync(py, ty, n * 4, hipMemcpyDeviceToHost, s));
    if (pz) HIP_TRY(hipMemcpyAsync(pz, tz, n * 4, hipMemcpyDeviceToHost, s));
    if (forget) HIP_TRY(hipMemcpyAsync(forget, tf, n, hipMemcpyDeviceToHost, s));
    HIP_TRY(hipStreamSynchronize(s));
  }
  if (w || ts || track || label || status) {
    DevTemps tmp;
    float *tw;
    uint16_t *tts, *ttr;
    uint8_t *tl, *tst;
    HIP_TRY(tmp.alloc(&tw, n));
    HIP_TRY(tmp.alloc(&tts, n));
    HIP_TRY(tmp.alloc(&ttr, n));
    HIP_TRY(tmp.alloc(&tl, n));
    HIP_TRY(tmp.alloc(&tst, n));
    launch_rec_unpack(m->d, m->st, tw, tts, ttr, tl, tst, s);
    if (status) HIP_TRY(hipMemcpyAsync(status, tst, n, hipMemcpyDeviceToHost, s));
    if (w) HIP_TRY(hipMemcpyAsync(w, tw, n * 4, hipMemcpyDeviceToHost, s));
    if (ts) HIP_TRY(hipMemcpyAsync(ts, tts, n * 2, hipMemcpyDeviceToHost, s));
    if (track) HIP_TRY(hipMemcpyAsync(track, ttr, n * 2, hipMemcpyDeviceToHost, s));
    if (label) HIP_TRY(hipMemcpyAsync(label, tl, n, hipMemcpyDeviceToHost, s));
    HIP_TRY(hipStreamSynchronize(s));
  }
  if (owner) HIP_TRY(hipMemcpyAsync(owner, m->st.owner, n * 2, hipMemcpyDeviceToHost, s));
  HIP_TRY(hipStreamSynchronize(s));
  if (owner) {
    std::vector<uint32_t> al(2 + 2 * ALIAS_CAP);
    HIP_TRY(hipMemcpyAsync(al.data(), m->st.alias, al.size() * 4, hipMemcpyDeviceToHost, m->stream));
    HIP_TRY(hipStreamSynchronize(m->stream));
    const uint32_t na = std::min<uint32_t>(al[0], m->st.alias_cap);
    for (uint32_t k = 0; k < na; ++k) {
      const uint32_t idx = al[2 + 2 * k], trk = al[3 + 2 * k];
      if (trk == OWNER_NONE || idx >= n) continue;
      if (owner[idx] == OWNER_NONE || owner[idx] < trk) owner[idx] = (uint16_t)trk;
    }
  }
  return SDM_OK;
}

sdm_status sdm_load_state(sdm_map *m, const float *px, const float *py, const float *pz, const float *w,
                          const uint16_t *ts, const uint16_t *track, const uint8_t *label, const uint8_t *status,
                          const uint8_t *forget, const uint16_t *owner) {
  if (!m || !px || !py || !pz || !w || !ts || !track || !label || !status || !forget) return SDM_ERR_INVALID_ARGUMENT;
  m->sweep_all = true;
  m->state_event_valid = false;
  HIP_TRY(hipSetDevice(m->device));
  hipStream_t s = m->stream;
  const size_t n = (size_t)m->d.v_count * m->d.S;
  HIP_TRY(hipMemsetAsync(m->st.grp_hint, 0, grp_hint_bytes(m->d.v_count), s));
  m->sweep_skip_scan = false;
  m->sweep_rec_pending = false;
  DevTemps tmp;
  float *tx, *ty, *tz;
  uint8_t *tf;
  HIP_TRY(tmp.alloc(&tx, n));
  HIP_TRY(tmp.alloc(&ty, n));
  HIP_TRY(tmp.alloc(&tz, n));
  HIP_TRY(tmp.alloc(&tf, n));
  HIP_TRY(hipMemcpyAsync(tx, px, n * 4, hipMemcpyHostToDevice, s));
  HIP_TRY(hipMemcpyAsync(ty, py, n * 4, hipMemcpyHostToDevice, s));
  HIP_TRY(hipMemcpyAsync(tz, pz, n * 4, hipMemcpyHostToDevice, s));
  HIP_TRY(hipMemcpyAsync(tf, forget, n, hipMemcpyHostToDevice, s));
  launch_pack_pos4(m->st.pos4, m->st.forget, tx, ty, tz, tf, n, s);
  {
    float *tw;
    uint16_t *tts, *ttr;
    uint8_t *tl, *tst;
    HIP_TRY(tmp.alloc(&tw, n));
    HIP_TRY(tmp.alloc(&tts, n));
    HIP_TRY(tmp.alloc(&ttr, n));
    HIP_TRY(tmp.alloc(&tl, n));
    HIP_TRY(tmp.alloc(&tst, n));
    HIP_TRY(hipMemcpyAsync(tst, status, n, hipMemcpyHostToDevice, s));
    HIP_TRY(hipMemcpyAsync(tw, w, n * 4, hipMemcpyHostToDevice, s));
    HIP_TRY(hipMemcpyAsync(tts, ts, n * 2, hipMemcpyHostToDevice, s));
    HIP_TRY(hipMemcpyAsync(ttr, track, n * 2, hipMemcpyHostToDevice, s));
    HIP_TRY(hipMemcpyAsync(tl, label, n, hipMemcpyHostToDevice, s));
    launch_rec_pack(m->d, m->st, tw, tts, ttr, tl, tst, s);
    HIP_TRY(hipStreamSynchronize(s));
  }
  if (owner) HIP_TRY(hipMemcpyAsync(m->st.owner, owner, n * 2, hipMemcpyHostToDevice, s));
  else HIP_TRY(hipMemsetAsync(m->st.owner, 0xFF, n * 2, s));
  launch_owner_flags(m->d, m->st, s);
  HIP_TRY(hipMemsetAsync(m->st.alias, 0, 8, s));
  HIP_TRY(hipMemsetAsync(m->st.alias_filter, 0, ALIAS_FILTER_WORDS * 4, s));
  launch_vflag_from_records(m->d, m->st, s);
  HIP_TRY(hipStreamSynchronize(s));
  return SDM_OK;
}

sdm_status sdm_get_ck_kappa(sdm_map *m, float *out) {
  if (!m || !out) return SDM_ERR_INVALID_ARGUMENT;
  HIP_TRY(hipSetDevice(m->device));
  if (m->ck_raw_last) launch_ck_finish(m->d, m->flt, m->sc, m->ck_raw_last, 1, 0, m->stream);
  HIP_TRY(hipMemcpyAsync(out, m->sc.ck_kappa, (size_t)m->d.W * m->d.H * 4, hipMemcpyDeviceToHost, m->stream));
  HIP_TRY(hipStreamSynchronize(m->stream));
  return SDM_OK;
}
sdm_status sdm_get_bin_counts(sdm_map *m, uint32_t *out) {
  if (!m || !out) return SDM_ERR_INVALID_ARGUMENT;
  HIP_TRY(hipSetDevice(m->device));
  HIP_TRY(hipMemcpyAsync(out, m->sc.bin_count, (size_t)m->d.W * m->d.H * 4, hipMemcpyDeviceToHost, m->stream));
  HIP_TRY(hipStreamSynchronize(m->stream));
  return SDM_OK;
}
sdm_status sdm_get_bins(sdm_map *m, uint32_t *out, int64_t cap, int64_t *n_out) {
  if (!m || !n_out) return SDM_ERR_INVALID_ARGUMENT;
  HIP_TRY(hipSetDevice(m->device));
  Counters c;
  HIP_TRY(hipMemcpyAsync(&c, m->sc.cnt, sizeof(c), hipMemcpyDeviceToHost, m->stream));
  HIP_TRY(hipStreamSynchronize(m->stream));
  *n_out = c.n_vis;
  const int64_t n_vis = std::min<int64_t>(c.n_vis, m->sc.cap_vis);
  if (n_vis > 0 && out && cap > 0) {
    const int W = m->d.W, H = m->d.H;
    std::vector<uint32_t> idx((size_t)n_vis), bs((size_t)H * (W + 1));
    HIP_TRY(hipMemcpyAsync(idx.data(), m->sc.bin_idx, idx.size() * 4, hipMemcpyDeviceToHost, m->stream));
    HIP_TRY(hipMemcpyAsync(bs.data(), m->sc.bin_start, bs.size() * 4, hipMemcpyDeviceToHost, m->stream));
    HIP_TRY(hipStreamSynchronize(m->stream));
    int64_t at = 0;
    for (int r = 0; r < H && at < cap; ++r) {
      const uint32_t a = bs[(size_t)r * (W + 1)], b = bs[(size_t)r * (W + 1) + W];
      for (uint32_t k = a; k < b && at < cap && k < (uint32_t)n_vis; ++k) out[at++] = idx[k];
    }
  }
  return SDM_OK;
}
sdm_status sdm_get_extrinsic(sdm_map *m, float *out16) {
  if (!m || !out16) return SDM_ERR_INVALID_ARGUMENT;
  memcpy(out16, m->f.E, 64);
  return SDM_OK;
}
// ... 13 lines not shown
```

semantic_dsp_map_amd/csrc/sdm_internal.h:

```cpp
#pragma once
#include <hip/hip_runtime.h>
#include <stdint.h>

#include "../../include/sdm.h"

#pragma clang fp contract(off)

namespace sdm {

constexpr uint32_t INVALID_INDEX = 0xffffffffu;
constexpr uint16_t OWNER_NONE = 0xFFFF;
constexpr int PDF_NUM = 20000;
#define SDM_OCC_INIT_WEIGHT 0.05f
#define SDM_MIN_RIGHT_PDF 0.1f

enum : uint8_t { ST_INVALID = 0, ST_UPDATED = 1, ST_REGULAR_BORN = 2, ST_GUESSED_BORN = 3, ST_COPIED = 4, ST_TIMEPTC = 5 };

struct Dims {
  int x_n, y_n, z_n, p_n;
  uint32_t NX, NY, NZ, S;
  uint32_t V;
  uint32_t v_begin;
  uint32_t v_count;
  uint32_t rz_begin, rz_count;
  float voxel_size, recip;
  float pmin[3], pmax[3];
  int W, H;
  float fx, fy, cx, cy;
  float dmin, dmax;
  float tanx, tany;
  float occl_coeff;
  int window_half;
  int max_movable;
};

struct Frame {
  int eq[3];
  float center[3];
  uint32_t gts;
  uint32_t epoch;
  float E[16];
  int bb0[3], bb1[3];
  int start_v[3];
  int start_ok;
};

struct Filter {
  float p_detect, noise_number, occ_threshold, id_transition;
  float forget[8];
  int independent;
  int consider_depth_noise;
  int nb;
  int use_rng;
  int noise_n;
};

struct Counters {
  uint32_t n_vis;
  uint32_t n_birth_success;
  uint32_t n_birth_attempts;
  uint32_t n_resampled;
  uint32_t n_moved;
  uint32_t n_move_reinserted;
  uint32_t n_frustum_voxels;
  uint32_t n_occupied;
  uint32_t n_free;
  uint32_t overflow;
  uint32_t n_valid_px;
  uint32_t n_halo_dropped;
  uint32_t vis_flood_complex, vis_flood_rounds, vis_start_in_frustum;
  uint32_t n_moved_b[2];
  uint32_t pad[2];
  struct alignas(128) ShardLine {
    uint32_t vis;
    uint32_t fv;
    uint32_t heavy;
    uint32_t birth;
    uint32_t resample;
    uint32_t sweep;
    uint32_t sweep_tiles;
    uint32_t heavy_ticket;
    uint32_t pad[24];
  };
  ShardLine shard[64];
  uint32_t flood_complex;
  uint32_t flood_rounds;
  uint32_t start_in_frustum;
  uint32_t flood_pad[29];
};
static_assert(sizeof(Counters::ShardLine) == 128, "one cache line per shard");
constexpr uint32_t VIS_SHARDS = 64;
constexpr uint32_t ROW_SUBS = 8;
constexpr int ROW_COL_BITS = 12, ROW_PIB_BITS = 32 - ROW_COL_BITS;
constexpr uint32_t ROW_CNT_STRIDE = 32;
constexpr uint32_t OWNER_CHUNK = 4096;
constexpr uint32_t OWNER_GROUP = 64;
__host__ __device__ constexpr size_t owner_flag_bytes(size_t n_slots) {
  return ((n_slots + OWNER_CHUNK - 1) / OWNER_CHUNK + OWNER_GROUP - 1) / OWNER_GROUP * OWNER_GROUP;
}
__host__ __device__ constexpr size_t owner_flag2_bytes(size_t n_slots) { return (owner_flag_bytes(n_slots) / OWNER_GROUP + 4095) / 4096 * 4096; }
constexpr int MAX_STAMP_UPDATES = 96;
struct StampUpdates {
  int n;
  uint32_t value;
  uint16_t entry[MAX_STAMP_UPDATES];
};
struct Cursors {
  int32_t birth_cursor;
  int32_t move_cursor;
  uint32_t move_list_overflow;
};

constexpr size_t REC_BYTES_PER_SLOT = 10;
__host__ __device__ constexpr uint32_t rec_bytes(uint32_t S) { return (uint32_t)REC_BYTES_PER_SLOT * (S - 1u); }
__host__ __device__ constexpr size_t rec_array_bytes(size_t v_count, uint32_t S) { return (v_count + 64) * rec_bytes(S) + 64; }
typedef float rec_f32 __attribute__((aligned(2)));
typedef uint32_t rec_v4u __attribute__((ext_vector_type(4), aligned(2)));
typedef uint32_t rec_v2u __attribute__((ext_vector_type(2), aligned(2)));

struct SlotRef {
  unsigned char *r;
  uint32_t L, k;
  __host__ __device__ __forceinline__ float w() const { return *reinterpret_cast<const rec_f32 *>(r + 4u * k); }
  __host__ __device__ __forceinline__ uint16_t ts() const { return *reinterpret_cast<const uint16_t *>(r + 4u * L + 2u * k); }
  __host__ __device__ __forceinline__ uint16_t track() const { return *reinterpret_cast<const uint16_t *>(r + 6u * L + 2u * k); }
  __host__ __device__ __forceinline__ uint8_t label() const { return r[8u * L + k]; }
  __host__ __device__ __forceinline__ uint8_t status() const { return r[9u * L + k]; }
  __host__ __device__ __forceinline__ void set_w(float v) const { *reinterpret_cast<rec_f32 *>(r + 4u * k) = v; }
  __host__ __device__ __forceinline__ void set_ts(uint16_t v) const { *reinterpret_cast<uint16_t *>(r + 4u * L + 2u * k) = v; }
  __host__ __device__ __forceinline__ void set_track(uint16_t v) const { *reinterpret_cast<uint16_t *>(r + 6u * L + 2u * k) = v; }
  __host__ __device__ __forceinline__ void set_label(uint8_t v) const { r[8u * L + k] = v; }
  __host__ __device__ __forceinline__ void set_status(uint8_t v) const { r[9u * L + k] = v; }
};

struct State {
  float4 *pos4 = nullptr;
  uint8_t *forget = nullptr;
  unsigned char *rec = nullptr;
  uint16_t *vts = nullptr;
  uint8_t *vflag = nullptr;
  uint8_t *tile_dirty = nullptr;
  uint32_t tile_stride = 0;
  unsigned long long *occ_need = nullptr;
  uint16_t *occ_list = nullptr;
  uint32_t *occ_list_n = nullptr;
  uint2 *occ_unit = nullptr;
  uint32_t occ_unit_cap = 0;
  struct alignas(128) OccListShard {
    unsigned long long word;
    uint32_t aux[30];
  };
  OccListShard *occ_shard = nullptr;
  uint8_t *grp_hint = nullptr;
  uint16_t *owner = nullptr;
  uint8_t *owner_flag = nullptr;
  uint8_t *owner_flag2 = nullptr;
  uint32_t *alias = nullptr;
  uint32_t alias_cap = 0;
  uint32_t *alias_filter = nullptr;
  sdm_voxel_result *res = nullptr;
  uint32_t *stamps_x = nullptr, *stamps_y = nullptr, *stamps_z = nullptr;
  float *pdf = nullptr;
  float *noise = nullptr;
};

// ... 335 lines not shown
```

semantic_dsp_map_amd/csrc/sdm_map.h:

```cpp
#pragma once
#include <algorithm>
#include <cstdio>
#include <cstring>
#include <functional>
#include <string>
#include <vector>

#include "sdm_internal.h"
#include "sdm_scratch.h"

typedef struct ncclComm *ncclComm_t;

namespace sdm {
void set_error(const char *what, const char *file, int line, const char *detail);
}

#define HIP_TRY(expr)                                                        \
  do {                                                                       \
    hipError_t e_ = (expr);                                                  \
    if (e_ != hipSuccess) {                                                  \
      sdm::set_error(#expr, __FILE__, __LINE__, hipGetErrorString(e_));      \
      return SDM_ERR_HIP;                                                    \
    }                                                                        \
  } while (0)
#define NCCL_TRY(expr)                                                       \
  do {                                                                       \
    ncclResult_t r_ = (expr);                                                \
    if (r_ != ncclSuccess) {                                                 \
      sdm::set_error(#expr, __FILE__, __LINE__, ncclGetErrorString(r_));     \
      return SDM_ERR_COMM;                                                   \
    }                                                                        \
  } while (0)
#define SDM_TRY(expr) do { const sdm_status rc_ = (expr); if (rc_ != SDM_OK) return rc_; } while (0)

using namespace sdm;

struct Derived {
  Frame f{};
  uint32_t flags = 0;
  bool valid = false;
  void built(const Frame &from, uint32_t with) { f = from, flags = with, valid = true; }
};
struct QueryStage {
  unsigned char *d = nullptr, *h = nullptr;
  size_t bytes = 0;
};
struct EsdfLayer : Derived {
  uint32_t *site = nullptr, *snap = nullptr;
};
struct InstLayer : Derived {
  unsigned char *acc = nullptr;
  sdm_instance *out = nullptr;
  uint32_t *meta = nullptr;
};
struct FrontLayer : Derived {
  unsigned char *bits = nullptr, *cells = nullptr;
  uint32_t *meta = nullptr, *scan = nullptr;
  size_t alloc = 0;
  int64_t cap = 0;
};
struct ViewPool {
  uint32_t *pool = nullptr;
  uint32_t masks = 0;
  int32_t batch = 0;
  bool clear_rewalk = false;
};
struct ReachLayer : Derived {
  uint32_t *cost = nullptr, *trav = nullptr, *act = nullptr, *list = nullptr;
  uint32_t *meta = nullptr, *h_meta = nullptr;
  uint32_t min_d2 = 0, max_cost = 0;
};

struct sdm_map {
  sdm_config cfg{};
  sdm_params prm{};
  Dims d{};
  Frame f{};
  Filter flt{};
  BirthOrder bo{};
  State st{};
  Scratch sc{};
  hipStream_t stream = nullptr;
  hipStream_t own_stream = nullptr;
  hipStream_t s_frustum = nullptr, s_birth = nullptr, s_moves = nullptr;
  hipEvent_t ev_state = nullptr, ev_counts = nullptr;
  hipEvent_t ev_vis = nullptr;
  bool vis_event_valid = false;
  bool mv_pending = false;
  bool state_event_valid = false;
  hipEvent_t ev_begin = nullptr, ev_frustum = nullptr, ev_birth = nullptr;
  int birth_which = 0;
  float *ck_user = nullptr;
  bool fused_ck = false;
  const float *ck_raw_last = nullptr;
  int32_t stop_after = 0;
  uint32_t frame_flags = 0;
  int n_moves = 0, n_remove = 0;
  std::vector<sdm_object_move> moves_all;
  std::vector<int32_t> removes_all;
  size_t mv_batch_next = 0;
  bool mv_batch_ready = false;
  uint32_t mv_seq = 0;
  uint32_t *d_track_bits = nullptr;
  int32_t *d_counts_local = nullptr;
  ncclComm_t comm = nullptr;
  bool ipc = false;
  unsigned char *ipc_arena = nullptr;
  void *ipc_peer[16] = {};
  uint32_t ipc_seq[4] = {0, 0, 0, 0};
  size_t ipc_off_counts = 0, ipc_off_halo = 0, ipc_off_stage = 0, ipc_off_full = 0, ipc_bytes = 0;
  int ipc_fine_grained = 0;
  float *d_ck_full_local = nullptr;
  int32_t *d_counts_all_local = nullptr;
  uint32_t *d_ipc_sync = nullptr;
  int32_t *d_counts_all = nullptr;
  unsigned char *d_halo_send = nullptr, *d_halo_recv = nullptr;
  float *d_ck_stage = nullptr, *d_ck_full = nullptr;
  uint32_t halo_cap_own = 0;
  size_t ck_part_stride = 0;
  int ck_exchange = 0;
  float *d_ck_all = nullptr;
  int comm_timeout_ms = 30000;
  uint32_t ck_chunk = 0;
  hipEvent_t ev_comm[8]{};
  bool comm_timing = false, comm_timed[4]{};
  bool sharded_frame = false;
  int32_t *counts_local_user = nullptr;
  const int32_t *counts_all_user = nullptr;
  int device = 0;

  std::vector<uint32_t> stamps_x, stamps_y, stamps_z;
  int moved_steps[3]{}, eq_steps[3]{};
  float map_center[3]{}, ego_center[3]{}, last_pos[3]{};
  uint32_t global_time_stamp = 0;
  float forgetting_function[5]{};
  bool forgetting_initialized = false;
  float cam_R[9]{}, cam_p[3]{};
  FrameArgs fa{};
  FrameArgs *d_fa[3]{};
  FrameBeginLaunch fb{};
  hipEvent_t ev_fa = nullptr;
  const float *cur_depth = nullptr;
  const sdm_labeled_point *cur_cloud = nullptr;
  int graph_mode = 2;
  bool use_graph = false;
  int graph_shape = 0;
  hipGraphExec_t piece[5] = {};
  double enqueue_us = 0.0;
  double t_prepare_us = 0, t_setparams_us = 0, t_launch_us = 0, t_direct_us = 0;
  bool host_timing = false;
  bool capturing = false;
  hipGraph_t graph = nullptr;
  hipGraphExec_t graph_exec = nullptr;
  hipGraphNode_t graph_set_node = nullptr;
  Filter graph_flt{};
  hipEvent_t cap_begin = nullptr, cap_frustum = nullptr, cap_birth = nullptr;
  uint64_t n_graph_frames = 0, n_direct_frames = 0;
  int restamped[3]{};
  bool stamps_dirty = true;
  bool sweep_all = true;
  bool sweep_lists = true;
  bool sweep_skip_scan = false;
  bool sweep_skip_allowed = true;
  bool sweep_rec_pending = false;
  int sweep_lists_forced = -1;
  uint32_t sweep_epoch = 1;

  float *d_depth = nullptr;
  sdm_labeled_point *d_cloud = nullptr;
  float *d_ck_part = nullptr;
  struct RawInputs {
    float *depth = nullptr;
    uint8_t *static_mask = nullptr, *obj_masks = nullptr;
    uint16_t *label_to_inst = nullptr;
    uint16_t label_host[256];
    bool label_valid = false;
    double *bbox = nullptr;
    size_t obj_masks_cap = 0;
    hipEvent_t ev_free = nullptr;
  } raw[2];
  int raw_next = 0;
  hipStream_t s_copy = nullptr;
  hipEvent_t ev_copy = nullptr;
  unsigned char *d_src_stage = nullptr;
  size_t src_stage_bytes = 0;
  unsigned long long *d_u64 = nullptr;
  EmitScratch emit;
  unsigned char *h_emit = nullptr;
  size_t h_emit_bytes = 0;
  uint32_t *h_track_bits = nullptr;
  size_t emit_guess = 1024;
  sdm_point *d_points = nullptr;
  size_t points_cap = 0;
  QueryStage stage;
  EsdfLayer esdf;
  InstLayer inst;
  FrontLayer front;
  ViewPool views;
  ReachLayer reach;
  sdm_point_xyzrgb *d_points_rgb = nullptr;
  size_t points_rgb_cap = 0;
  ColourTables *d_colours = nullptr;
  bool colours_set = false;
  int nb_alloc = 0;
  size_t sort_cap = 0;
  int noise_n = 0;
  int force_generic_flood = 0;

  bool profiling = false;
  hipEvent_t ev[9]{};
  bool stage_ran[9]{};
  std::vector<void *> allocs, pinned;
  std::vector<hipEvent_t> events;
};

namespace sdm {

sdm_status map_alloc(sdm_map *m, void **p, size_t bytes, bool pinned);
void map_release(sdm_map *m, void **p);
sdm_status new_event(sdm_map *m, hipEvent_t *e, unsigned flags);
template <typename T>
sdm_status alloc_tracked(sdm_map *m, T **p, size_t n, bool pinned = false) {
  return map_alloc(m, (void **)p, std::max<size_t>(n, 1) * sizeof(T), pinned);
}
template <typename T>
void release(sdm_map *m, T **p) {
  map_release(m, (void **)p);
}
template <typename T>
sdm_status regrow(sdm_map *m, T **p, size_t *cap, size_t n, hipStream_t quiet = nullptr, bool pinned = false) {
  if (quiet) HIP_TRY(hipStreamSynchronize(quiet));
  *cap = 0;
  release(m, p);
  SDM_TRY(alloc_tracked(m, p, n, pinned));
  *cap = n;
  return SDM_OK;
}
struct DevTemps {
  std::vector<void *> v;
  template <typename T>
  hipError_t alloc(T **p, size_t n) {
    const hipError_t e = hipMalloc((void **)p, std::max<size_t>(n, 1) * sizeof(T));
    if (e == hipSuccess) v.push_back((void *)*p);
    return e;
  }
  ~DevTemps() { for (void *p : v) (void)hipFree(p); }
};

inline bool stage_done(int32_t stop_after, int stage) { return stop_after != 0 && stop_after <= stage; }
enum { GRAPH_PIECES = 0, GRAPH_BRANCHED = 1, GRAPH_CHAIN = 2 };
void issue_mode_for(const sdm_map *m, int mode, bool *use_graph, int *shape);
hipError_t lazy_stream(int device, hipStream_t *s);
void refresh_filter(sdm_map *m);
void update_ego_center(sdm_map *m, const float pos[3]);
void compute_extrinsic(sdm_map *m, const float pos[3], const float q[4]);
void compute_frustum_box(sdm_map *m);
void sync_frame_scalars(sdm_map *m);
sdm_status upload_stamps(sdm_map *m);
int sweep_mode(const sdm_map *m);
sdm_status sweep_mode_latch(sdm_map *m);
sdm_status check_counters(sdm_map *m, Counters *out);
int bind_host_thread_to(int device);
void drop_graphs(sdm_map *m);
sdm_status exchange_counts(sdm_map *m, hipStream_t s);
sdm_status exchange_check(sdm_map *m);
sdm_status exchange_wait(sdm_map *m);
void exchange_teardown(sdm_map *m);
sdm_status query_check(sdm_map *m, const void *in, int64_t n, const void *out, uint32_t flags, uint32_t allowed, const char *what);
struct LayerName {
  const char *the_layer, *build, *update;
  bool plural;
};
sdm_status layer_check(sdm_map *m, const char *what, const Derived *need, const LayerName &name);
void layer_origin(const sdm_map *m, const Derived &l, float origin[3]);
struct StageCol {
  enum Kind { IN, OUT, OUT_RAW } kind;
  void *host;
  size_t elem;
};
using StageLaunch = std::function<sdm_status(const unsigned char *pre, unsigned char *const *col, size_t count)>;
using StageCopyOut = std::function<void(const unsigned char *const *col, size_t off, size_t count)>;
sdm_status run_staged(sdm_map *m, size_t n, size_t chunk, const void *pre, size_t pre_bytes, const std::vector<StageCol> &cols,
                      const StageLaunch &launch, const StageCopyOut &copy_out = nullptr);
using QueryLaunch = std::function<void(const void *, void *, void *, uint32_t, hipStream_t)>;
sdm_status run_query(sdm_map *m, const void *in_v, size_t in_elem, void *out_v, size_t out_elem, void *out2_v, size_t out2_elem, int64_t n,
                     uint32_t flags, const QueryLaunch &launch);

}
```

semantic_dsp_map_amd/csrc/sdm_scratch.h:

```cpp
#pragma once
#include "sdm_internal.h"

namespace sdm {

struct BirthOrder {
  int off[10];
  int cols[9];
};

struct MoveCopy {
  float x, y, z;
  uint32_t forget_bits;
  float w;
  uint16_t ts, track, owner;
  uint8_t label, status;
  uint32_t voxel;
};
static_assert(sizeof(MoveCopy) == 32, "MoveCopy layout");

constexpr int MAX_MOVE_OBJECTS = 48;
constexpr int MAX_REMOVE_TRACKS = 128;
constexpr int HALO_OBJ = 64;
constexpr int HALO_RECORD_BYTES = 36;
constexpr int HALO_HEADER_BYTES = 16;
__host__ __device__ constexpr size_t halo_segment_bytes(uint32_t cap) { return HALO_HEADER_BYTES + (size_t)cap * HALO_RECORD_BYTES; }
struct MoveSet {
  int n;
  float T[MAX_MOVE_OBJECTS][12];
  uint16_t track[MAX_MOVE_OBJECTS];
};

struct FrameArgs {
  Frame f;
  StampUpdates su;
  MoveSet ms;
  int n_obj;
  int n_remove;
  uint32_t mv_seq;
  uint32_t mv_batch;
  int force_generic;
  const float *depth;
  const sdm_labeled_point *cloud;
  uint16_t remove[MAX_REMOVE_TRACKS];
};
static_assert(sizeof(FrameArgs) <= 3400, "FrameArgs travels as a kernel argument (4 KB limit, with the launch's other arguments)");

constexpr int MV_ROW = 16;
constexpr int MV_DIRECT = MV_ROW - 2;
constexpr uint32_t MV_FIRST = 0x100u;
struct Scratch {
  const FrameArgs *fa = nullptr;
  const FrameArgs *fa_side = nullptr;
  const FrameArgs *fa_moves = nullptr;
  uint64_t *vmask = nullptr, *reach = nullptr;
  int wpl = 0;
  uint64_t *line_ne = nullptr, *line_ey = nullptr, *line_ez = nullptr, *line_reach = nullptr;
  int wy = 0;
  uint32_t *bin_count = nullptr, *bin_start = nullptr;
  uint32_t *row_cnt = nullptr;
  uint8_t *row_win = nullptr;
  uint2 *row_list = nullptr;
  uint32_t row_cap = 0;
  uint32_t cap_vis = 0;
  uint32_t *bin_idx = nullptr, *vpix = nullptr;
  float4 *vp4 = nullptr;
  uint32_t *vtf = nullptr;
  float4 *pix4 = nullptr;
  uint32_t *pixt = nullptr;
  float *ck_kappa = nullptr;
  uint8_t *ck_class = nullptr;
  uint32_t *ck_heavy = nullptr;
  uint32_t cap_heavy = 0;
  uint32_t *b_valid = nullptr, *b_rank = nullptr;
  uint32_t *bkey_a = nullptr, *bval_a = nullptr, *bkey_b = nullptr, *bval_b = nullptr;
  float4 *bpos = nullptr;
  uint32_t *mv_cnt = nullptr;
  uint32_t *mv_list = nullptr, *mv_nlist = nullptr;
  uint32_t *mv_nmem = nullptr, *mv_mem = nullptr, *mv_tot = nullptr;
  MoveCopy *mv_copy = nullptr;
  uint32_t cap_move = 0;
  unsigned char *halo_send = nullptr;
  const unsigned char *halo_recv = nullptr;
  uint32_t halo_cap = 0;
  uint32_t halo_world = 1;
  uint8_t *track_to_obj = nullptr;
  uint32_t *scan_scratch = nullptr, *sort_scratch = nullptr;
  uint32_t *scan_scratch_b = nullptr;
  uint32_t *mv_row = nullptr, *mv_next = nullptr;
  Counters *cnt = nullptr;
  Cursors *cur = nullptr;
};

constexpr int MAX_CLOUD_OBJECTS = 64;
struct CloudArgsHost {
  double R[9], t[3];
  double ifx, icx, ify, icy;
  double dmin, dmax;
  float sigma0, sigma1;
  int consider_depth_noise, consider_instance, n_objects, has_static;
  int sky_instance, has_bbox;
  int track[MAX_CLOUD_OBJECTS], label[MAX_CLOUD_OBJECTS];
};
void launch_labeled_cloud(const Dims &d, const CloudArgsHost &h, const float *depth, const uint8_t *static_mask,
                          const uint16_t *label_to_inst, const uint8_t *obj_masks, const double *bbox,
                          sdm_labeled_point *cloud, hipStream_t s);
void launch_manual_resize(const Dims &d, const void *src, void *dst, int src_w, int src_h, float scale, int elem_bytes,
                          hipStream_t s);

void launch_set_frame(FrameArgs *fa_dev, const FrameArgs &fa, hipStream_t s);
const void *set_frame_kernel();
struct MembersArgs {
  uint32_t *mv_cnt, *mv_list, *mv_nlist, *mv_nmem, *mv_mem, *mv_tot;
  Cursors *cur;
  uint32_t n_flags;
  size_t n_slots;
};
struct FrameBeginLaunch {
#ifndef SDM_FB_GRID
#define SDM_FB_GRID 1024
#endif
  static constexpr unsigned GRID = SDM_FB_GRID, BLOCK = 256;
  Counters *cnt;
  uint32_t *bin_count;
  uint32_t n_bins;
  State st;
  FrameArgs fa;
  FrameArgs *dst_main, *dst_side;
  Dims d;
  uint32_t slab_max;
  MembersArgs ma;
  int with_members;
  void *argv[11];
  void set(const Dims &d, const State &st, const Scratch &sc, const FrameArgs &fa, bool with_side, bool with_members);
  static const void *kernel();
};
void launch_frame_begin(FrameBeginLaunch &a, hipStream_t s, hipEvent_t done = nullptr);
void launch_moves_batch(const Dims &d, const State &st, const Scratch &sc, const FrameArgs &fa_batch, int32_t *counts_local, hipStream_t s);
constexpr int OCC_LISTS = 1, OCC_SKIP_SCAN = 2;
void launch_occupancy(const Dims &d, const Filter &flt, const State &st, Counters *cnt, int all_dirty, const FrameArgs *fa, uint32_t remark,
                      hipStream_t s, int mode = 0);
size_t tile_mark_bytes(const Dims &d);
void launch_frustum(const Dims &d, const Scratch &sc, hipStream_t s);
void launch_visibility(const Dims &d, const Filter &flt, const State &st, const Scratch &sc, float *ck_out, int finish, hipStream_t s,
                       hipEvent_t vis_done = nullptr);
void launch_ck(const Dims &d, const Filter &flt, const State &st, const Scratch &sc, float *ck_out, int finish, hipStream_t s);
void launch_ck_finish(const Dims &d, const Filter &flt, const Scratch &sc, const float *parts, int n_parts, size_t part_stride, hipStream_t s);
void launch_ck_reduce_chunk(const float *stage, const float *own_part, float *full, uint32_t chunk, int world, int rank, hipStream_t s);
void launch_weight(const Dims &d, const Filter &flt, const State &st, const Scratch &sc, hipStream_t s, const float *ck_raw = nullptr);
int launch_birth_prepare(const Dims &d, const Filter &flt, const BirthOrder &bo, const State &st,
                         const Scratch &sc, hipStream_t s);
void launch_birth_replay(const Dims &d, const Filter &flt, const State &st, const Scratch &sc, int which, bool literal,
                         hipStream_t s);
void launch_count_live(const Dims &d, const State &st, unsigned long long *out, hipStream_t s);
void launch_count_owner(const Dims &d, const State &st, uint16_t track, unsigned long long *out, hipStream_t s);
void launch_pack_pos4(float4 *pos4, uint8_t *forget_plane, const float *px, const float *py, const float *pz, const uint8_t *forget, size_t n,
                      hipStream_t s);
void launch_unpack_pos4(const float4 *pos4, const uint8_t *forget_plane, float *px, float *py, float *pz, uint8_t *forget, size_t n, hipStream_t s);
void launch_rec_pack(const Dims &d, const State &st, const float *w, const uint16_t *ts, const uint16_t *track,
                     const uint8_t *label, const uint8_t *status, hipStream_t s);
void launch_rec_unpack(const Dims &d, const State &st, float *w, uint16_t *ts, uint16_t *track, uint8_t *label, uint8_t *status,
                       hipStream_t s);
void launch_fill_dense(const Dims &d, const State &st, uint32_t stamp, int mode, hipStream_t s);
void launch_vflag_from_records(const Dims &d, const State &st, hipStream_t s);
struct ColourTables {
  sdm_colour_config cfg;
  int32_t sdiv[256], hdiv180[256];
};
struct EmitScratch {
  uint8_t *mask = nullptr;
  uint32_t *blk_cnt = nullptr;
  uint32_t *total = nullptr;
};
size_t emit_mask_bytes(const Dims &d);
size_t emit_block_elems(const Dims &d);
void launch_emit_count(const Dims &d, const State &st, const EmitScratch &e, int want_free, hipStream_t s);
void launch_emit_points_rgb(const Dims &d, const Frame &f, const State &st, const ColourTables *ct, const EmitScratch &e,
                            sdm_point_xyzrgb *out, uint32_t cap, int want_free, const float sub[3], hipStream_t s);
void launch_emit_points(const Dims &d, const Frame &f, const State &st, const EmitScratch &e, sdm_point *out, uint32_t cap, int want_free,
                        const float sub[3], int mark_fov, hipStream_t s);

size_t move_blocks(const Dims &d);
size_t move_count_elems();
size_t move_member_elems(size_t n_slots);
size_t move_total_elems();
void launch_tracks_with_particles(const Dims &d, const State &st, uint32_t *bitmap, hipStream_t s);
void launch_owner_flags(const Dims &d, const State &st, hipStream_t s);
void launch_moves_count(const Dims &d, const State &st, const Scratch &sc, int32_t *counts_local, hipStream_t s,
                        const FrameArgs *by_value = nullptr);
void launch_moves_transform(const Dims &d, const Filter &flt, const State &st, const Scratch &sc, const int32_t *counts_all, int world,
                            int rank, hipStream_t s);
void launch_moves_finish(const Dims &d, const Filter &flt, const State &st, const Scratch &sc, int world, int rank, hipStream_t s);
void launch_remove(const Dims &d, const State &st, const Scratch &sc, hipStream_t s);

}
```

Before: 95860.

## Replace birth radix sort with wavefront-aggregated hash table selecting earliest candidates per voxel

In the common non-literal case, birth preparation no longer sorts all candidate keys. A new select kernel groups candidates by voxel within each wavefront using ballots and has one leader claim a slot in an open-addressed hash table. It keeps the K smallest candidate indices per voxel with atomicMin insertion and records claimed buckets in per-shard head lists. Birth replay then iterates those heads, reads and resets each bucket, and never scans the sorted arrays. The change also adds configurable points for starting birth preparation, including after move replay or visibility, plus debug knobs for table size and hash mask. The cost is extra scratch memory, atomic contention, and table reset bookkeeping.

```diff
diff --git a/include/sdm.h b/include/sdm.h
--- a/include/sdm.h
+++ b/include/sdm.h
@@ -388,6 +388,7 @@
 sdm_status sdm_get_stats(sdm_map *m, sdm_stats *out, int32_t count_live);
 sdm_status sdm_set_profiling(sdm_map *m, int32_t on);
 sdm_status sdm_debug_force_generic_flood(sdm_map *m, int32_t on);
+sdm_status sdm_debug_birth_table(sdm_map *m, int32_t min_size, uint32_t hash_mask);
 sdm_status sdm_get_ring_state(sdm_map *m, sdm_ring_state *out);
 sdm_status sdm_set_ring_state(sdm_map *m, const sdm_ring_state *in);
 sdm_status sdm_get_stamps(sdm_map *m, uint32_t *sx, uint32_t *sy, uint32_t *sz);
diff --git a/semantic_dsp_map_amd/binding.py b/semantic_dsp_map_amd/binding.py
--- a/semantic_dsp_map_amd/binding.py
+++ b/semantic_dsp_map_amd/binding.py
@@ -209,6 +209,7 @@
         "sdm_get_stats": [vp, C.POINTER(Stats), i32],
         "sdm_set_profiling": [vp, i32],
         "sdm_debug_force_generic_flood": [vp, i32],
+        "sdm_debug_birth_table": [vp, i32, C.c_uint32],
         "sdm_get_ring_state": [vp, C.POINTER(RingState)],
         "sdm_set_ring_state": [vp, C.POINTER(RingState)],
         "sdm_get_stamps": [vp, vp, vp, vp],
@@ -711,6 +712,9 @@
     def force_generic_flood(self, on=True):
         _check(self.L, self.L.sdm_debug_force_generic_flood(self.h, 1 if on else 0), "sdm_debug_force_generic_flood")
 
+    def debug_birth_table(self, min_size=False, hash_mask=0xffffffff):
+        _check(self.L, self.L.sdm_debug_birth_table(self.h, 1 if min_size else 0, hash_mask), "sdm_debug_birth_table")
+
     def ring_state(self):
         r = RingState()
         _check(self.L, self.L.sdm_get_ring_state(self.h, C.byref(r)), "sdm_get_ring_state")
diff --git a/semantic_dsp_map_amd/csrc/debug.hip b/semantic_dsp_map_amd/csrc/debug.hip
--- a/semantic_dsp_map_amd/csrc/debug.hip
+++ b/semantic_dsp_map_amd/csrc/debug.hip
@@ -37,6 +37,14 @@
 sdm_status sdm_debug_force_generic_flood(sdm_map *m, int32_t on) {
   if (!m) return SDM_ERR_INVALID_ARGUMENT;
   m->force_generic_flood = on ? 1 : 0;
+  return SDM_OK;
+}
+
+sdm_status sdm_debug_birth_table(sdm_map *m, int32_t min_size, uint32_t hash_mask) {
+  if (!m) return SDM_ERR_INVALID_ARGUMENT;
+  if (m->n_graph_frames || m->n_direct_frames) return SDM_ERR_INVALID_ARGUMENT;
+  m->sc.bt_min = min_size ? 1u : 0u;
+  m->sc.bt_hash_mask = hash_mask;
   return SDM_OK;
 }
 
diff --git a/semantic_dsp_map_amd/csrc/frame.hip b/semantic_dsp_map_amd/csrc/frame.hip
--- a/semantic_dsp_map_amd/csrc/frame.hip
+++ b/semantic_dsp_map_amd/csrc/frame.hip
@@ -72,6 +72,23 @@
   fa.force_generic = m->force_generic_flood;
   m->n_moves = n_moves;
   m->n_remove = n_remove;
+  return SDM_OK;
+}
+
+#ifndef SDM_BIRTH_START
+#define SDM_BIRTH_START 0
+#endif
+int birth_start(const sdm_map *m) {
+  if (m->capturing) return 0;
+  if (SDM_BIRTH_START == 1) return m->n_moves > 0 ? 1 : 0;
+  return SDM_BIRTH_START;
+}
+
+sdm_status enqueue_birth_prepare(sdm_map *m, hipEvent_t behind) {
+  if (!m->capturing) HIP_TRY(hipStreamWaitEvent(m->s_birth, behind, 0));
+  m->birth_literal = !m->capturing && m->global_time_stamp > 65535u;
+  m->birth_which = launch_birth_prepare(m->d, m->flt, m->bo, m->st, m->sc, m->birth_literal, m->s_birth);
+  HIP_TRY(hipEventRecord(m->capturing ? m->cap_birth : m->ev_birth, m->s_birth));
   return SDM_OK;
 }
 
@@ -101,7 +118,7 @@
     HIP_TRY(hipEventRecord(m->ev_fa, m->s_frustum));
     if (whole && m->mv_pending) HIP_TRY(hipMemsetAsync(m->sc.mv_tot, 0, move_total_elems() * sizeof(uint32_t), s));
     m->fb.set(d, m->st, m->sc, m->fa, false, whole);
-    launch_frame_begin(m->fb, s, !stage_done(stop_after, 5) ? m->ev_begin : nullptr);
+    launch_frame_begin(m->fb, s, !stage_done(stop_after, 5) && birth_start(m) == 0 ? m->ev_begin : nullptr);
     if (whole && m->n_moves > 0) m->mv_pending = true;
   }
   stage_mark(m, 1);
@@ -135,11 +152,7 @@
   } else if (!m->capturing) {
     HIP_TRY(hipStreamWaitEvent(s, m->ev_fa, 0));
   }
-  if (!stage_done(stop_after, 5)) {
-    if (!m->capturing) HIP_TRY(hipStreamWaitEvent(m->s_birth, m->ev_begin, 0));
-    m->birth_which = launch_birth_prepare(d, m->flt, m->bo, m->st, m->sc, m->s_birth);
-    HIP_TRY(hipEventRecord(m->capturing ? m->cap_birth : m->ev_birth, m->s_birth));
-  }
+  if (!stage_done(stop_after, 5) && birth_start(m) == 0) SDM_TRY(enqueue_birth_prepare(m, m->ev_begin));
   if (side_chain) HIP_TRY(hipStreamWaitEvent(s, m->ev_counts, 0));
   m->state_event_valid = false;
   m->vis_event_valid = false;
@@ -246,7 +259,9 @@
   hipStream_t s = m->stream;
   const Dims &d = m->d;
   if (m->capturing || m->n_moves > 0)
-    launch_moves_finish(d, m->flt, m->st, m->sc, m->counts_all_user ? m->cfg.shard_count : 1, m->cfg.shard_rank, s);
+    launch_moves_finish(d, m->flt, m->st, m->sc, m->counts_all_user ? m->cfg.shard_count : 1, m->cfg.shard_rank, s,
+                        !stage_done(stop_after, 5) && birth_start(m) == 1 ? m->ev_moved : nullptr);
+  if (!stage_done(stop_after, 5) && birth_start(m) == 1) SDM_TRY(enqueue_birth_prepare(m, m->ev_moved));
   stage_mark(m, 2);
   if (stage_done(stop_after, 2)) return SDM_OK;
 
@@ -265,6 +280,7 @@
   float *ck_dst = m->ck_user ? m->ck_user : m->d_ck_part;
   launch_visibility(d, m->flt, m->st, m->sc, ck_dst, m->fused_ck ? 1 : 0, s, m->capturing ? nullptr : m->ev_vis);
   if (!m->capturing) m->vis_event_valid = true;
+  if (!stage_done(stop_after, 5) && birth_start(m) == 2) SDM_TRY(enqueue_birth_prepare(m, m->ev_vis));
   stage_mark(m, 4);
   if (stage_done(stop_after, 4)) return SDM_OK;
 
@@ -318,7 +334,7 @@
   stage_mark(m, 5);
   if (stage_done(stop_after, 5)) return SDM_OK;
   HIP_TRY(hipStreamWaitEvent(s, m->capturing ? m->cap_birth : m->ev_birth, 0));
-  launch_birth_replay(d, m->flt, m->st, m->sc, m->birth_which, m->global_time_stamp > 65535u, s);
+  launch_birth_replay(d, m->flt, m->st, m->sc, m->birth_which, m->birth_literal, s);
   if (!m->capturing) {
     if (d.v_count != d.V || m->comm || m->ipc) {
       HIP_TRY(hipEventRecord(m->ev_state, s));
@@ -444,7 +460,7 @@
   };
   sdm_status rc = capture(m->s_frustum, 0, [&](hipStream_t st) { launch_frustum(d, m->sc, st); });
   if (rc == SDM_OK)
-    rc = capture(m->s_birth, 1, [&](hipStream_t st) { m->birth_which = launch_birth_prepare(d, m->flt, m->bo, m->st, m->sc, st); });
+    rc = capture(m->s_birth, 1, [&](hipStream_t st) { m->birth_which = launch_birth_prepare(d, m->flt, m->bo, m->st, m->sc, false, st); });
   if (rc == SDM_OK)
     rc = capture(m->stream, 2, [&](hipStream_t st) {
       if (d.v_count != d.V) launch_moves_count(d, m->st, m->sc, m->d_counts_local, st);
diff --git a/semantic_dsp_map_amd/csrc/kernels.hip b/semantic_dsp_map_amd/csrc/kernels.hip
--- a/semantic_dsp_map_amd/csrc/kernels.hip
+++ b/semantic_dsp_map_amd/csrc/kernels.hip
@@ -2386,11 +2386,8 @@
   sc.b_valid[q] = as_global(sc.fa->cloud)[i * d.W + j].is_valid ? 1u : 0u;
 }
 
-__global__ __launch_bounds__(TPB) void k_birth_candidates(Dims d, Filter flt, BirthOrder bo, State st, Scratch sc) {
-  const Frame f = sc.fa->f;
-  uint32_t b = blockIdx.x * blockDim.x + threadIdx.x;
-  uint32_t total = (uint32_t)(d.W * d.H) * (uint32_t)flt.nb;
-  if (b >= total) return;
+__device__ __forceinline__ uint32_t birth_candidate(const Dims &d, const Frame &f, const Filter &flt, const BirthOrder &bo, const State &st,
+                                                    const Scratch &sc, uint32_t b) {
   int q = (int)(b / (uint32_t)flt.nb), n = (int)(b % (uint32_t)flt.nb);
   int i, j;
   birth_seq_to_pixel(bo, q, i, j);
@@ -2411,9 +2408,90 @@
     uint32_t v = global_pos_to_voxel(d, f, x, y, z, rx, ry, rz);
     if (v != INVALID_INDEX && rz >= d.rz_begin && rz < d.rz_begin + d.rz_count) key = v;
   }
-  sc.bkey_a[b] = key;
+  sc.bpos[b] = make_float4(x, y, z, __uint_as_float((uint32_t)pt.track_id | ((uint32_t)pt.label_id << 16)));
+  return key;
+}
+
+__global__ __launch_bounds__(TPB) void k_birth_candidates(Dims d, Filter flt, BirthOrder bo, State st, Scratch sc) {
+  const Frame f = sc.fa->f;
+  uint32_t b = blockIdx.x * blockDim.x + threadIdx.x;
+  uint32_t total = (uint32_t)(d.W * d.H) * (uint32_t)flt.nb;
+  if (b >= total) return;
+  sc.bkey_a[b] = birth_candidate(d, f, flt, bo, st, sc, b);
   sc.bval_a[b] = b;
-  sc.bpos[b] = make_float4(x, y, z, __uint_as_float((uint32_t)pt.track_id | ((uint32_t)pt.label_id << 16)));
+}
+
+constexpr uint32_t BT_IDLE = 0xffffffffu;
+__device__ __forceinline__ uint32_t bt_load(const uint32_t *p) { return __hip_atomic_load(p, __ATOMIC_RELAXED, __HIP_MEMORY_SCOPE_AGENT); }
+__host__ __device__ constexpr uint32_t birth_head_cap(size_t candidates) {
+  return (uint32_t)(((candidates + TPB - 1) / TPB + VIS_SHARDS - 1) / VIS_SHARDS) * TPB;
+}
+
+template <int S>
+__global__ __launch_bounds__(TPB) void k_birth_select(Dims d, Filter flt, BirthOrder bo, State st, Scratch sc, uint32_t n_buckets) {
+  constexpr int K = 2 * (S - 1) + 1, BW = 2 * S;
+  const Frame f = sc.fa->f;
+  const uint32_t b = blockIdx.x * blockDim.x + threadIdx.x;
+  const uint32_t total = (uint32_t)(d.W * d.H) * (uint32_t)flt.nb;
+  uint32_t key = d.V;
+  if (b < total) key = birth_candidate(d, f, flt, bo, st, sc, b);
+  const bool has = key < d.V;
+  uint64_t peers = __ballot(has);
+  if (peers == 0ull) return;
+  const int nbits = d.x_n + d.y_n + d.z_n;
+  for (int bit = 0; bit < nbits; ++bit) {
+    const bool one = (key >> bit) & 1u;
+    const uint64_t m = __ballot(one);
+    peers &= one ? m : ~m;
+  }
+  const uint32_t lane = threadIdx.x & 63u;
+  const uint64_t lt_mask = (lane == 0) ? 0ull : (~0ull >> (64 - lane));
+  const uint32_t rank = (uint32_t)__popcll(peers & lt_mask);
+  uint32_t bucket = BT_IDLE, tail = BT_IDLE;
+  bool claimed = false;
+  if (has && rank == 0u) {
+    const uint32_t h = (key * 0x9E3779B1u) & sc.bt_hash_mask;
+    uint32_t idx = (uint32_t)(((uint64_t)h * n_buckets) >> 32);
+    for (uint32_t n = 0; n < n_buckets; ++n) {
+      uint32_t *const kp = sc.btab + (size_t)idx * BW;
+      uint32_t k = bt_load(kp);
+      if (k == BT_IDLE) {
+        k = atomicCAS(kp, BT_IDLE, key);
+        if (k == BT_IDLE) {
+          claimed = true;
+          k = key;
+        }
+      }
+      if (k == key) {
+        bucket = idx;
+        if (!claimed) tail = bt_load(kp + K);
+        break;
+      }
+      idx = idx + 1u == n_buckets ? 0u : idx + 1u;
+    }
+    if (bucket == BT_IDLE) sc.cnt->overflow = 1;
+  }
+  const uint64_t cm = __ballot(claimed);
+  if (cm != 0ull) {
+    const int first = __ffsll((unsigned long long)cm) - 1;
+    const uint32_t shard = blockIdx.x & (VIS_SHARDS - 1);
+    uint32_t base = 0;
+    if ((int)lane == first) base = atomicAdd(&sc.cnt->shard[shard].bheads, (uint32_t)__popcll(cm));
+    base = (uint32_t)__shfl((int)base, first, 64);
+    if (claimed) sc.bheads[(size_t)shard * birth_head_cap(total) + base + (uint32_t)__popcll(cm & lt_mask)] = bucket;
+  }
+  const int src = has ? __ffsll((unsigned long long)peers) - 1 : (int)lane;
+  bucket = (uint32_t)__shfl((int)bucket, src, 64);
+  tail = (uint32_t)__shfl((int)tail, src, 64);
+  if (!has || rank >= (uint32_t)K || bucket == BT_IDLE || tail < b) return;
+  uint32_t *const row = sc.btab + (size_t)bucket * BW + 1;
+  uint32_t x = b;
+  for (int i = (int)rank; i < K; ++i) {
+    if (i > (int)rank && bt_load(row + K - 1) < x) break;
+    const uint32_t old = atomicMin(row + i, x);
+    x = old > x ? old : x;
+    if (x == BT_IDLE) break;
+  }
 }
 
 __global__ void k_birth_cursor(Dims d, Filter flt, Scratch sc) {
@@ -2627,39 +2705,27 @@
 #ifndef SDM_TIMERS_BIRTH
   if (threadIdx.x == 0) DBG_PUT(0, DBG_T());
 #endif
-  __shared__ uint32_t heads[TPB], head_key[TPB];
-  __shared__ uint32_t n_heads;
-  if (threadIdx.x == 0) n_heads = 0;
-  __syncthreads();
-  if (t < total) {
-    const uint32_t key = skey[t];
-    const uint32_t prev = t > 0 ? skey[t - 1] : 0xffffffffu;
-    if (key < d.V && prev != key) {
-      const uint32_t q = atomicAdd(&n_heads, 1u);
-      heads[q] = t;
-      head_key[q] = key;
-    }
-  }
-  __syncthreads();
-  if (threadIdx.x >= n_heads) return;
-#ifndef SDM_TIMERS_BIRTH
-  if (threadIdx.x == 0) DBG_PUT(1, DBG_T());
-#endif
-  t = heads[threadIdx.x];
-  const uint32_t v = head_key[threadIdx.x];
-  constexpr int LMAX = 2 * (S - 1) + 1;
-  uint32_t kb[LMAX], sv[LMAX];
-  kb[0] = v;
-#pragma unroll
-  for (int j = 1; j < LMAX; ++j) kb[j] = t + j < total ? skey[t + j] : 0xffffffffu;
-  if constexpr (!LITERAL) {
-#pragma unroll
-    for (int j = 0; j < LMAX; ++j) sv[j] = t + j < total ? sval[t + j] : 0u;
-  }
-  uint32_t rx, ry, rz;
-  voxel_to_ring(d, v, rx, ry, rz);
-  const uint32_t smax = stamp_max(st, rx, ry, rz);
   if constexpr (LITERAL) {
+    __shared__ uint32_t heads[TPB], head_key[TPB];
+    __shared__ uint32_t n_heads;
+    if (threadIdx.x == 0) n_heads = 0;
+    __syncthreads();
+    if (t < total) {
+      const uint32_t key = skey[t];
+      const uint32_t prev = t > 0 ? skey[t - 1] : 0xffffffffu;
+      if (key < d.V && prev != key) {
+        const uint32_t q = atomicAdd(&n_heads, 1u);
+        heads[q] = t;
+        head_key[q] = key;
+      }
+    }
+    __syncthreads();
+    if (threadIdx.x >= n_heads) return;
+    t = heads[threadIdx.x];
+    const uint32_t v = head_key[threadIdx.x];
+    uint32_t rx, ry, rz;
+    voxel_to_ring(d, v, rx, ry, rz);
+    const uint32_t smax = stamp_max(st, rx, ry, rz);
     uint32_t ns = 0, nr = 0;
     birth_replay_sequential<S>(d, f, flt, st, sc, skey, sval, total, t, v, smax, ns, nr);
     if (ns || nr) {
@@ -2670,6 +2736,30 @@
     if (nr) atomicAdd(&sc.cnt->shard[blockIdx.x & (VIS_SHARDS - 1)].resample, nr);
     return;
   } else {
+  constexpr int LMAX = 2 * (S - 1) + 1;
+  const uint32_t shard = t / total, place = t - shard * total;
+  if (place >= sc.cnt->shard[shard].bheads) return;
+#ifndef SDM_TIMERS_BIRTH
+  if (threadIdx.x == 0) DBG_PUT(1, DBG_T());
+#endif
+  uint32_t *const bucket = sc.btab + (size_t)sc.bheads[(size_t)shard * total + place] * (2 * S);
+  uint32_t bw[2 * S], sv[LMAX];
+  load_vec<(8 * S < 16 ? 8 * S : 16)>(bw, bucket);
+  {
+    v4u idle = {BT_IDLE, BT_IDLE, BT_IDLE, BT_IDLE};
+#pragma unroll
+    for (int j = 0; j < 2 * S / 4; ++j) reinterpret_cast<v4u *>(bucket)[j] = idle;
+  }
+  const uint32_t v = bw[0];
+  uint32_t L = 0;
+#pragma unroll
+  for (int j = 0; j < LMAX; ++j) {
+    sv[j] = bw[1 + j];
+    L += sv[j] != BT_IDLE ? 1u : 0u;
+  }
+  uint32_t rx, ry, rz;
+  voxel_to_ring(d, v, rx, ry, rz);
+  const uint32_t smax = stamp_max(st, rx, ry, rz);
   const size_t base = (size_t)(v - d.v_begin) * S;
   uint8_t stv[S];
   uint16_t tsv[S];
@@ -2684,17 +2774,8 @@
   const uint32_t n_alias = st.alias[0];
   bool alias_touched = false;
   uint32_t fbits = n_alias ? alias_filter_bits<S>(st, base) : 0u;
-  uint32_t L = 0;
-  {
-    bool run = true;
-#pragma unroll
-    for (int j = 0; j < LMAX; ++j) {
-      run = run && kb[j] == v;
-      L += run ? 1u : 0u;
-    }
-  }
 #ifdef SDM_TIMERS_BIRTH
-  if (threadIdx.x == 0) DBG_PUT(0, DBG_T() + (stv[1] == 0xEE ? 1 : 0) + (own[1] == 0xEEEE ? 1 : 0) + (wv0[1] == 1234.5f ? 1 : 0) + (trk0[1] == 0xEEEE ? 1 : 0) + (kb[LMAX - 1] == 0xEEEEEEEEu ? 1 : 0) + (sv[LMAX - 1] == 0xEEEEEEEEu ? 1 : 0));
+  if (threadIdx.x == 0) DBG_PUT(0, DBG_T() + (stv[1] == 0xEE ? 1 : 0) + (own[1] == 0xEEEE ? 1 : 0) + (wv0[1] == 1234.5f ? 1 : 0) + (trk0[1] == 0xEEEE ? 1 : 0) + (sv[LMAX - 1] == 0xEEEEEEEEu ? 1 : 0));
 #endif
   const bool noise_flavour = flt.consider_depth_noise != 0;
   uint32_t vac0 = 0;
@@ -3338,14 +3419,25 @@
 #undef SDM_WEIGHT
 }
 
+size_t birth_table_words(const Dims &d, size_t candidates) { return 2 * candidates * (2 * (size_t)d.S); }
+size_t birth_head_words(size_t candidates) { return (size_t)VIS_SHARDS * birth_head_cap(candidates); }
+
 int launch_birth_prepare(const Dims &d, const Filter &flt, const BirthOrder &bo, const State &st,
-                         const Scratch &sc, hipStream_t s) {
+                         const Scratch &sc, bool literal, hipStream_t s) {
   const size_t hw = (size_t)d.W * d.H;
   const size_t total = hw * flt.nb;
   if (flt.use_rng) {
     hipLaunchKernelGGL(k_birth_flags, dim3(blocks_for(hw)), dim3(TPB), 0, s, d, bo, sc);
     exclusive_scan_u32(sc.b_valid, sc.b_rank, hw, sc.scan_scratch_b, s);
   }
+  if (!literal) {
+    if (total) {
+      const uint32_t n_buckets = (uint32_t)(sc.bt_min ? total : 2 * total);
+      SDM_DISPATCH_S(k_birth_select, dim3(blocks_for(total)), s, d, flt, bo, st, sc, n_buckets);
+    }
+    if (flt.use_rng) hipLaunchKernelGGL(k_birth_cursor, dim3(1), dim3(64), 0, s, d, flt, sc);
+    return 0;
+  }
   hipLaunchKernelGGL(k_birth_candidates, dim3(blocks_for(total)), dim3(TPB), 0, s, d, flt, bo, st, sc);
   if (flt.use_rng) hipLaunchKernelGGL(k_birth_cursor, dim3(1), dim3(64), 0, s, d, flt, sc);
   int nbits = d.x_n + d.y_n + d.z_n + 1;
@@ -3357,10 +3449,12 @@
   const size_t total = (size_t)d.W * d.H * flt.nb;
   const uint32_t *skey = which ? sc.bkey_b : sc.bkey_a;
   const uint32_t *sval = which ? sc.bval_b : sc.bval_a;
-  dim3 grid(blocks_for(total));
+  const uint32_t cap = birth_head_cap(total);
+  dim3 grid(literal ? blocks_for(total) : VIS_SHARDS * (cap / TPB));
+  if (grid.x == 0) return;
 #define SDM_BIRTH(SS)                                                                                                  \
   if (literal) hipLaunchKernelGGL((k_birth_replay<SS, true>), grid, dim3(TPB), 0, s, d, flt, st, sc, skey, sval, (uint32_t)total); \
-  else hipLaunchKernelGGL((k_birth_replay<SS, false>), grid, dim3(TPB), 0, s, d, flt, st, sc, skey, sval, (uint32_t)total);
+  else hipLaunchKernelGGL((k_birth_replay<SS, false>), grid, dim3(TPB), 0, s, d, flt, st, sc, skey, sval, cap);
   switch (d.p_n) {
     case 1: SDM_BIRTH(2) break;
     case 2: SDM_BIRTH(4) break;
diff --git a/semantic_dsp_map_amd/csrc/lifecycle.hip b/semantic_dsp_map_amd/csrc/lifecycle.hip
--- a/semantic_dsp_map_amd/csrc/lifecycle.hip
+++ b/semantic_dsp_map_amd/csrc/lifecycle.hip
@@ -100,6 +100,11 @@
   flt.noise_n = m->noise_n;
 }
 
+sdm_status birth_table_idle(sdm_map *m) {
+  if (m->sc.btab) HIP_TRY(hipMemsetAsync(m->sc.btab, 0xff, m->btab_bytes, m->stream));
+  return SDM_OK;
+}
+
 static void build_birth_order(sdm_map *m) {
   const int W = m->d.W, H = m->d.H;
   int off = 0;
@@ -120,18 +125,23 @@
   if (nb <= m->nb_alloc) return SDM_OK;
   const size_t need = hw * nb;
   Scratch &sc = m->sc;
-  void **const old[6] = {(void **)&sc.bkey_a, (void **)&sc.bval_a, (void **)&sc.bkey_b, (void **)&sc.bval_b, (void **)&sc.bpos, (void **)&sc.sort_scratch};
-  const size_t bytes[6] = {need * 4, need * 4, need * 4, need * 4, need * sizeof(*sc.bpos), sort_scratch_elems(need) * 4};
-  void *fresh[6] = {};
+  constexpr int N = 8;
+  void **const old[N] = {(void **)&sc.bkey_a, (void **)&sc.bval_a, (void **)&sc.bkey_b, (void **)&sc.bval_b, (void **)&sc.bpos, (void **)&sc.sort_scratch,
+                         (void **)&sc.btab, (void **)&sc.bheads};
+  const size_t bytes[N] = {need * 4, need * 4, need * 4, need * 4, need * sizeof(*sc.bpos), sort_scratch_elems(need) * 4,
+                           birth_table_words(m->d, need) * 4, birth_head_words(need) * 4};
+  void *fresh[N] = {};
   sdm_status rc = SDM_OK;
   HIP_TRY(hipStreamSynchronize(m->stream));
-  for (int i = 0; i < 6 && rc == SDM_OK; ++i) rc = map_alloc(m, &fresh[i], bytes[i], false);
-  for (int i = 0; i < 6; ++i) {
+  for (int i = 0; i < N && rc == SDM_OK; ++i) rc = map_alloc(m, &fresh[i], bytes[i], false);
+  for (int i = 0; i < N; ++i) {
     map_release(m, rc == SDM_OK ? old[i] : &fresh[i]);
     if (rc == SDM_OK) *old[i] = fresh[i];
   }
   SDM_TRY(rc);
   HIP_TRY(hipMemsetAsync(sc.sort_scratch, 0, sort_scratch_elems(need) * 4, m->stream));
+  m->btab_bytes = bytes[6];
+  SDM_TRY(birth_table_idle(m));
   HIP_TRY(hipStreamSynchronize(m->stream));
   m->nb_alloc = nb;
   m->sort_cap = need;
@@ -406,7 +416,7 @@
 
   for (hipStream_t *s : {&m->own_stream, &m->s_frustum, &m->s_birth}) HIP_TRY(new_stream(cfg->device, s));
   m->stream = m->own_stream;
-  for (hipEvent_t *e : {&m->ev_state, &m->ev_counts, &m->ev_begin, &m->ev_frustum, &m->ev_birth, &m->ev_fa, &m->ev_vis, &m->cap_begin,
+  for (hipEvent_t *e : {&m->ev_state, &m->ev_counts, &m->ev_begin, &m->ev_frustum, &m->ev_birth, &m->ev_fa, &m->ev_vis, &m->ev_moved, &m->cap_begin,
                         &m->cap_frustum, &m->cap_birth, &m->ev_copy, &m->raw[0].ev_free, &m->raw[1].ev_free})
     SDM_TRY(new_event(m, e, hipEventDisableTiming));
   const size_t n_slots = (size_t)d.v_count * d.S;
@@ -656,6 +666,7 @@
   m->sweep_rec_pending = false;
   host_initialize(m);
   launch_clear(m->d, m->st, m->stream, false);
+  SDM_TRY(birth_table_idle(m));
   return upload_stamps(m);
 }
 
diff --git a/semantic_dsp_map_amd/csrc/moves.hip b/semantic_dsp_map_amd/csrc/moves.hip
--- a/semantic_dsp_map_amd/csrc/moves.hip
+++ b/semantic_dsp_map_amd/csrc/moves.hip
@@ -1128,15 +1128,20 @@
   hipLaunchKernelGGL(k_move_apply, dim3(1024), dim3(TPB), 0, s, d, flt, st, sc, d.v_count != d.V ? counts_all : nullptr, world, rank);
 }
 
-void launch_moves_finish(const Dims &d, const Filter &flt, const State &st, const Scratch &sc, int world, int rank, hipStream_t s) {
+void launch_moves_finish(const Dims &d, const Filter &flt, const State &st, const Scratch &sc, int world, int rank, hipStream_t s,
+                         hipEvent_t replay_done) {
   if (world > 1 && sc.halo_recv) hipLaunchKernelGGL(k_move_import, dim3(64, world), dim3(TPB), 0, s, d, sc, world, rank);
   dim3 grid(RP_GRID);
+#define SDM_MOVE_REPLAY(SS)                                                                                             \
+  if (replay_done) hipExtLaunchKernelGGL(k_move_replay<SS>, grid, dim3(RP_TPB), 0, s, nullptr, replay_done, 0, d, flt, st, sc); \
+  else hipLaunchKernelGGL(k_move_replay<SS>, grid, dim3(RP_TPB), 0, s, d, flt, st, sc);
   switch (d.p_n) {
-    case 1: hipLaunchKernelGGL(k_move_replay<2>, grid, dim3(RP_TPB), 0, s, d, flt, st, sc); break;
-    case 2: hipLaunchKernelGGL(k_move_replay<4>, grid, dim3(RP_TPB), 0, s, d, flt, st, sc); break;
-    case 3: hipLaunchKernelGGL(k_move_replay<8>, grid, dim3(RP_TPB), 0, s, d, flt, st, sc); break;
-    default: hipLaunchKernelGGL(k_move_replay<16>, grid, dim3(RP_TPB), 0, s, d, flt, st, sc); break;
-  }
+    case 1: SDM_MOVE_REPLAY(2) break;
+    case 2: SDM_MOVE_REPLAY(4) break;
+    case 3: SDM_MOVE_REPLAY(8) break;
+    default: SDM_MOVE_REPLAY(16) break;
+  }
+#undef SDM_MOVE_REPLAY
 }
 
 void launch_remove(const Dims &d, const State &st, const Scratch &sc, hipStream_t s) {
diff --git a/semantic_dsp_map_amd/csrc/readback.hip b/semantic_dsp_map_amd/csrc/readback.hip
--- a/semantic_dsp_map_amd/csrc/readback.hip
+++ b/semantic_dsp_map_amd/csrc/readback.hip
@@ -360,6 +360,7 @@
   hipStream_t s = m->stream;
   const size_t n = (size_t)m->d.v_count * m->d.S;
   HIP_TRY(hipMemsetAsync(m->st.grp_hint, 0, grp_hint_bytes(m->d.v_count), s));
+  SDM_TRY(birth_table_idle(m));
   m->sweep_skip_scan = false;
   m->sweep_rec_pending = false;
   DevTemps tmp;
diff --git a/semantic_dsp_map_amd/csrc/sdm_internal.h b/semantic_dsp_map_amd/csrc/sdm_internal.h
--- a/semantic_dsp_map_amd/csrc/sdm_internal.h
+++ b/semantic_dsp_map_amd/csrc/sdm_internal.h
@@ -80,7 +80,8 @@
     uint32_t sweep;
     uint32_t sweep_tiles;
     uint32_t heavy_ticket;
-    uint32_t pad[24];
+    uint32_t bheads;
+    uint32_t pad[23];
   };
   ShardLine shard[64];
   uint32_t flood_complex;
diff --git a/semantic_dsp_map_amd/csrc/sdm_map.h b/semantic_dsp_map_amd/csrc/sdm_map.h
--- a/semantic_dsp_map_amd/csrc/sdm_map.h
+++ b/semantic_dsp_map_amd/csrc/sdm_map.h
@@ -84,6 +84,7 @@
   hipStream_t own_stream = nullptr;
   hipStream_t s_frustum = nullptr, s_birth = nullptr, s_moves = nullptr;
   hipEvent_t ev_state = nullptr, ev_counts = nullptr;
+  hipEvent_t ev_moved = nullptr;
   hipEvent_t ev_vis = nullptr;
   bool vis_event_valid = false;
   bool mv_pending = false;
@@ -204,6 +205,8 @@
   bool colours_set = false;
   int nb_alloc = 0;
   size_t sort_cap = 0;
+  size_t btab_bytes = 0;
+  bool birth_literal = false;
   int noise_n = 0;
   int force_generic_flood = 0;
 
@@ -252,6 +255,7 @@
 void issue_mode_for(const sdm_map *m, int mode, bool *use_graph, int *shape);
 hipError_t lazy_stream(int device, hipStream_t *s);
 void refresh_filter(sdm_map *m);
+sdm_status birth_table_idle(sdm_map *m);
 void update_ego_center(sdm_map *m, const float pos[3]);
 void compute_extrinsic(sdm_map *m, const float pos[3], const float q[4]);
 void compute_frustum_box(sdm_map *m);
diff --git a/semantic_dsp_map_amd/csrc/sdm_scratch.h b/semantic_dsp_map_amd/csrc/sdm_scratch.h
--- a/semantic_dsp_map_amd/csrc/sdm_scratch.h
+++ b/semantic_dsp_map_amd/csrc/sdm_scratch.h
@@ -74,6 +74,9 @@
   uint32_t *b_valid = nullptr, *b_rank = nullptr;
   uint32_t *bkey_a = nullptr, *bval_a = nullptr, *bkey_b = nullptr, *bval_b = nullptr;
   float4 *bpos = nullptr;
+  uint32_t *btab = nullptr, *bheads = nullptr;
+  uint32_t bt_min = 0;
+  uint32_t bt_hash_mask = 0xffffffffu;
   uint32_t *mv_cnt = nullptr;
   uint32_t *mv_list = nullptr, *mv_nlist = nullptr;
   uint32_t *mv_nmem = nullptr, *mv_mem = nullptr, *mv_tot = nullptr;
@@ -147,8 +150,10 @@
 void launch_ck_finish(const Dims &d, const Filter &flt, const Scratch &sc, const float *parts, int n_parts, size_t part_stride, hipStream_t s);
 void launch_ck_reduce_chunk(const float *stage, const float *own_part, float *full, uint32_t chunk, int world, int rank, hipStream_t s);
 void launch_weight(const Dims &d, const Filter &flt, const State &st, const Scratch &sc, hipStream_t s, const float *ck_raw = nullptr);
+size_t birth_table_words(const Dims &d, size_t candidates);
+size_t birth_head_words(size_t candidates);
 int launch_birth_prepare(const Dims &d, const Filter &flt, const BirthOrder &bo, const State &st,
-                         const Scratch &sc, hipStream_t s);
+                         const Scratch &sc, bool literal, hipStream_t s);
 void launch_birth_replay(const Dims &d, const Filter &flt, const State &st, const Scratch &sc, int which, bool literal,
                          hipStream_t s);
 void launch_count_live(const Dims &d, const State &st, unsigned long long *out, hipStream_t s);
@@ -189,7 +194,8 @@
                         const FrameArgs *by_value = nullptr);
 void launch_moves_transform(const Dims &d, const Filter &flt, const State &st, const Scratch &sc, const int32_t *counts_all, int world,
                             int rank, hipStream_t s);
-void launch_moves_finish(const Dims &d, const Filter &flt, const State &st, const Scratch &sc, int world, int rank, hipStream_t s);
+void launch_moves_finish(const Dims &d, const Filter &flt, const State &st, const Scratch &sc, int world, int rank, hipStream_t s,
+                         hipEvent_t replay_done = nullptr);
 void launch_remove(const Dims &d, const State &st, const Scratch &sc, hipStream_t s);
 
 }
```

New measurement: 47430. 0.495x the previous value.
